# zhangrengang/SubPhaser

Measured on AMD Instinct MI355X. Metric: genome Gbases/s k-mer+enrichment, wheat k=15 1Mb windows, higher is better.
Workload: dtype u32

## Files before the change

include/subphaser_hip.h:

```cpp
#ifndef SUBPHASER_HIP_H
#define SUBPHASER_HIP_H
#include <stdint.h>
#ifdef __cplusplus
extern "C" {
#endif

#define SP_OK 0
#define SP_EINVAL (-1)
#define SP_EUNSUP (-2)
#define SP_ENOMEM (-3)
#define SP_EHIP (-4)
#define SP_ENODEV (-5)
#define SP_ESTATE (-6)
#define SP_EIO (-7)

typedef struct sp_ctx sp_ctx;

int sp_version(void);
const char *sp_last_error(const sp_ctx *ctx);

int sp_ctx_create(int device, void *stream, sp_ctx **out);
int sp_ctx_destroy(sp_ctx *ctx);
int sp_sync(sp_ctx *ctx);
void *sp_stream(sp_ctx *ctx);

int sp_genome_reset(sp_ctx *ctx, int n_chrom);
int sp_genome_add(sp_ctx *ctx, int chrom, const uint8_t *ascii, int64_t len);
int sp_genome_add_device(sp_ctx *ctx, int chrom, const uint8_t *d_ascii, int64_t len);
int sp_genome_len(sp_ctx *ctx, int chrom, int64_t *len);
int sp_genome_unpack(sp_ctx *ctx, int chrom, uint8_t *ascii_out, int64_t len);

int sp_count(sp_ctx *ctx, int k, int lower_count, int engine);
int sp_count_range(sp_ctx *ctx, int k, int lower_count, int engine, int first, int last);
int sp_count_recounts(sp_ctx *ctx, int64_t *recounts);
int sp_nslots(sp_ctx *ctx, int k, int64_t *nslots);
int sp_tables_bind(sp_ctx *ctx, int chrom, void *d_table);
int sp_table_overflow(sp_ctx *ctx, int chrom, void *d_pairs, int64_t cap, int64_t *n_pairs);
int sp_table_merge(sp_ctx *ctx, void *d_dst_u8, const void *d_dst_ovf, int64_t n_dst_ovf, const void *d_src_u8,
                   const void *d_src_ovf, int64_t n_src_ovf, int64_t slot_base, int64_t n, void *d_out_ovf, int64_t cap,
                   int64_t *n_out);
int sp_table_lengths(sp_ctx *ctx, const void *d_tab_u8, const void *d_ovf, int64_t n_ovf, int64_t slot_base, int64_t n,
                     int lower_count, int64_t *sum, int64_t *n_dump);
int sp_lengths(sp_ctx *ctx, int64_t *lengths );
int sp_dump_size(sp_ctx *ctx, int chrom, int64_t *n);
int sp_dump(sp_ctx *ctx, int chrom, uint64_t *keys, uint32_t *counts, int64_t cap, int64_t *n);

int sp_filter_view(sp_ctx *ctx, int C, const void *const *d_tabs, int64_t slot_base,
                   int64_t nslots_view, const int64_t *lengths, int k, int lower_count,
                   const void *const *d_ovf, const int64_t *n_ovf);
int sp_filter(sp_ctx *ctx, int n_sets, const int32_t *set_off, const int32_t *unit_off,
              const int32_t *unit_chrom, double min_fold, int baseline, double min_freq,
              double max_freq, double ratio, int64_t *n_union, int64_t *n_rows, int64_t *n_hist);
int sp_filter_fetch(sp_ctx *ctx, uint64_t *keys, uint32_t *counts, double *freqs, uint64_t *tot,
                    int64_t cap_rows);
int sp_filter_fetch_async(sp_ctx *ctx, uint64_t *keys, uint32_t *counts, uint64_t *tot, int64_t cap_rows);
int sp_filter_fetch_wait(sp_ctx *ctx);
int sp_filter_fetch_device(sp_ctx *ctx, void *d_keys, void *d_counts, void *d_tot, int64_t cap_rows);
int sp_filter_hist(sp_ctx *ctx, uint64_t *tot, int64_t cap);

int sp_labels_set(sp_ctx *ctx, const uint64_t *keys, const uint8_t *sg, int64_t n, int n_sg);
int sp_labels_set_device(sp_ctx *ctx, const uint64_t *d_keys, const uint8_t *d_sg, int64_t n, int n_sg);
int sp_map_nslots(sp_ctx *ctx, int chrom, int64_t bin_size, int64_t chunk_size, int64_t *nslots);
int sp_map_bins(sp_ctx *ctx, int chrom, int64_t bin_size, int64_t chunk_size, int32_t *slot_counts,
                int64_t nslots, int64_t *n_mapped);
int sp_map_bins_all(sp_ctx *ctx, int64_t bin_size, int64_t chunk_size, const int64_t *slot_off,
                    int32_t *slot_counts, int64_t *n_mapped);
int sp_stack_windows(sp_ctx *ctx, int64_t bin_size, int64_t chunk_size, int64_t window_size,
                     const int64_t *slot_off, const int64_t *win_off, int64_t *win_counts);
int sp_stack_windows_dev(sp_ctx *ctx, int64_t bin_size, int64_t chunk_size, int64_t window_size,
                         const int64_t *slot_off, const int64_t *win_off, const int64_t *seg_start, void *d_win);
int sp_map_features(sp_ctx *ctx, const uint8_t *ascii, const int64_t *off, int64_t n_feat,
                    int64_t *counts);
int sp_map_intervals(sp_ctx *ctx, const int32_t *chrom, const int64_t *start, const int64_t *end, int64_t n,
                     int64_t *counts);
int sp_labels_hit(sp_ctx *ctx, int64_t *n_hit);

int sp_enrich(sp_ctx *ctx, const int64_t *counts, int64_t W, int S, double max_pval,
              double min_ratio, double *pvals, int32_t *argmin, uint8_t *sig, double *ratios);
int sp_enrich_dev(sp_ctx *ctx, const void *d_counts, int64_t W, int S, double max_pval, double min_ratio,
                  double *pvals, int32_t *argmin, uint8_t *sig, double *ratios);
int sp_stack_enrich(sp_ctx *ctx, int64_t bin_size, int64_t chunk_size, int64_t window_size, const int64_t *slot_off,
                    const int64_t *win_off, double max_pval, double min_ratio, int64_t *win_counts, double *pvals,
                    int32_t *argmin, uint8_t *sig, double *ratios);

int sp_kmer_ttest(sp_ctx *ctx, const uint32_t *counts, int64_t M, int C, const int64_t *lengths, int n_groups,
                  const int32_t *group_off, const int32_t *group_chrom, int32_t *top, int32_t *second,
                  double *pvals, double *means);
int sp_kmer_ttest_wide(sp_ctx *ctx, const uint32_t *counts, int64_t M, int C, const int64_t *lengths, int n_groups,
                       const int32_t *group_off, const int32_t *group_chrom, int32_t *top, int32_t *second,
                       double *pvals, double *means);
int sp_kmer_ranktest(sp_ctx *ctx, const uint32_t *counts , int64_t M, int C, const int64_t *lengths,
                     int n_groups, const int32_t *group_off, const int32_t *group_chrom,
                     int method , int32_t *top, int32_t *second, double *pvals,
                     double *means , double *stat );
int sp_kmer_wilcoxon(sp_ctx *ctx, const uint32_t *counts , int64_t M, int C, const int64_t *lengths,
                     int n_groups, const int32_t *group_off, const int32_t *group_chrom, int32_t *top, int32_t *second,
                     double *pvals, double *means , double *stat );

int sp_kmeans_bootstrap(sp_ctx *ctx, const double *z , int C, int64_t M, const int64_t *cols , int R,
                        int n, int K, uint64_t seed, int32_t *labels , int32_t *iters ,
                        double *gram );

int sp_kmer_pca_gram(sp_ctx *ctx, const uint32_t *counts , int64_t M, int C,
                     const int64_t *lengths, double *gram , int64_t *n_bad, double *stats );
int sp_kmer_pca_signs(sp_ctx *ctx, const uint32_t *counts, int64_t M, int C, const int64_t *lengths,
                      const double *U , int n_comp, int64_t *rows , double *vals );

int sp_hclust_complete(sp_ctx *ctx, const double *pts , int P, int D, double *merges ,
                       double *dist );

int sp_sparse_sizes(sp_ctx *ctx, int64_t *n);
int sp_sparse_sample(sp_ctx *ctx, int chrom, int64_t n_samples, uint64_t *keys, int64_t *n_out);
int sp_sparse_split(sp_ctx *ctx, int chrom, const uint64_t *splitters, int n_split, int64_t *bounds);
int sp_sparse_export(sp_ctx *ctx, int chrom, int64_t first, int64_t count, void *d_keys, void *d_counts);
int sp_sparse_view(sp_ctx *ctx, int C, const void *const *d_keys, const void *const *d_counts, const int64_t *n,
                   const int64_t *lengths, int k, int lower_count);

int sp_prof_enable(sp_ctx *ctx, int on);
int sp_prof_reset(sp_ctx *ctx);
int sp_prof_report(sp_ctx *ctx, char *buf, int64_t cap);

int sp_synth_chrom(sp_ctx *ctx, uint8_t *d_out, int64_t len, uint64_t seed, int set_id,
                   int sg_id, int n_sg, int chrom_id, int exchange);
int sp_synth_chrom_range(sp_ctx *ctx, uint8_t *d_out, int64_t len, int64_t start, int64_t n, uint64_t seed, int set_id,
                         int sg_id, int n_sg, int chrom_id, int exchange);
int sp_host_alloc(sp_ctx *ctx, int64_t bytes, void **h_ptr);
int sp_host_free(sp_ctx *ctx, void *h_ptr);
int sp_host_register(sp_ctx *ctx, void *h_ptr, int64_t bytes);
int sp_host_unregister(sp_ctx *ctx, void *h_ptr);
int sp_dev_alloc(sp_ctx *ctx, int64_t bytes, void **d_ptr);
int sp_dev_free(sp_ctx *ctx, void *d_ptr);
int sp_dev_copy_to_host(sp_ctx *ctx, void *dst, const void *d_src, int64_t bytes);
int sp_dev_copy_from_host(sp_ctx *ctx, void *d_dst, const void *src, int64_t bytes);


typedef struct sp_fasta sp_fasta;
int sp_fasta_open(const void *data, int64_t n, int threads, sp_fasta **out);
int sp_fasta_counts(const sp_fasta *h, int64_t *n_records, int64_t *n_bases);
int sp_fasta_fetch(const sp_fasta *h, int64_t *hdr_start, int64_t *hdr_end, int64_t *seq_off, void *cat);
void sp_fasta_close(sp_fasta *h);

// ... 27 lines not shown
```

subphaser_amd/_native.py:

```python
import ctypes as C
import json
import os

import numpy as np

_HERE = os.path.dirname(os.path.abspath(__file__))
LIB_PATH = os.environ.get("SUBPHASER_HIP_LIB") or os.path.join(_HERE, "lib", "libsubphaser_hip.so")

SP_OK, SP_EINVAL, SP_EUNSUP, SP_ENOMEM, SP_EHIP, SP_ENODEV, SP_ESTATE, SP_EIO = 0, -1, -2, -3, -4, -5, -6, -7
KBOOT_MAX_POINTS, KBOOT_MAX_CLUSTERS = 128, 32
KPCA_MAX_CHROM, KPCA_MAX_COMP = 1024, 32
HCLUST_MAX_POINTS = 16384
RANKTEST_MAX_GROUP = 64
RANKTEST_METHODS = ("kruskal", "mannwhitneyu")
WILCOXON_MAX_GROUP = 64

SYMBOLS = [
    "sp_version", "sp_last_error", "sp_ctx_create", "sp_ctx_destroy", "sp_sync", "sp_stream",
    "sp_genome_reset", "sp_genome_add", "sp_genome_add_device", "sp_genome_len", "sp_genome_unpack",
    "sp_count", "sp_count_range", "sp_count_recounts", "sp_nslots", "sp_tables_bind", "sp_table_overflow", "sp_table_merge", "sp_table_lengths", "sp_lengths", "sp_dump_size", "sp_dump",
    "sp_filter_view", "sp_filter", "sp_filter_fetch", "sp_filter_fetch_async", "sp_filter_fetch_wait", "sp_filter_fetch_device", "sp_filter_hist",
    "sp_labels_set", "sp_labels_set_device", "sp_map_nslots", "sp_map_bins", "sp_map_bins_all", "sp_stack_windows", "sp_stack_windows_dev", "sp_stack_enrich", "sp_map_features", "sp_map_intervals", "sp_labels_hit",
    "sp_enrich", "sp_enrich_dev", "sp_kmer_ttest", "sp_kmer_ttest_wide", "sp_kmer_ranktest", "sp_kmer_wilcoxon", "sp_kmeans_bootstrap", "sp_kmer_pca_gram", "sp_kmer_pca_signs", "sp_hclust_complete",
    "sp_sparse_sizes", "sp_sparse_sample", "sp_sparse_split", "sp_sparse_export", "sp_sparse_view",
    "sp_prof_enable", "sp_prof_reset", "sp_prof_report",
    "sp_synth_chrom", "sp_synth_chrom_range", "sp_host_alloc", "sp_host_free", "sp_host_register", "sp_host_unregister", "sp_dev_alloc", "sp_dev_free", "sp_dev_copy_to_host", "sp_dev_copy_from_host",
    "sp_fasta_open", "sp_fasta_counts", "sp_fasta_fetch", "sp_fasta_close",
    "sp_text_kmer_matrix", "sp_text_sig_kmers", "sp_text_repr", "sp_text_table",
]


def csrc_fingerprint():
    import glob
    import hashlib
    h = hashlib.sha256()
    files = sorted(glob.glob(os.path.join(_HERE, "csrc", "*.hip")) + glob.glob(os.path.join(_HERE, "csrc", "*.h")))
    for f in files:
        h.update(os.path.basename(f).encode())
        h.update(open(f, "rb").read())
    return h.hexdigest()[:16]


class NativeError(RuntimeError):
    """HIP/runtime failure inside libsubphaser_hip.so."""


_lib = None


def load():
    global _lib
    if _lib is not None:
        return _lib
    if not os.path.exists(LIB_PATH):
        raise NativeError(
            "libsubphaser_hip.so is not built (%s). Run `python -c 'import __graft_entry__ as g; g.build()'` "
            "or `make -C subphaser_amd/csrc`. There is no CPU fallback." % LIB_PATH)
    L = C.CDLL(LIB_PATH)
    vp, i64, i32, dbl, ci = C.c_void_p, C.c_int64, C.c_int32, C.c_double, C.c_int
    P = C.POINTER
    L.sp_version.restype = ci
    L.sp_last_error.restype = C.c_char_p
    L.sp_last_error.argtypes = [vp]
    L.sp_ctx_create.argtypes = [ci, vp, P(vp)]
    L.sp_ctx_destroy.argtypes = [vp]
    L.sp_sync.argtypes = [vp]
    L.sp_stream.restype = vp
    L.sp_stream.argtypes = [vp]
    L.sp_genome_reset.argtypes = [vp, ci]
    L.sp_genome_add.argtypes = [vp, ci, vp, i64]
    L.sp_genome_add_device.argtypes = [vp, ci, vp, i64]
    L.sp_genome_len.argtypes = [vp, ci, P(i64)]
    L.sp_genome_unpack.argtypes = [vp, ci, vp, i64]
    L.sp_count.argtypes = [vp, ci, ci, ci]
    L.sp_count_range.argtypes = [vp, ci, ci, ci, ci, ci]
    L.sp_nslots.argtypes = [vp, ci, P(i64)]
    L.sp_count_recounts.argtypes = [vp, P(i64)]
    L.sp_tables_bind.argtypes = [vp, ci, vp]
    L.sp_table_overflow.argtypes = [vp, ci, vp, i64, P(i64)]
    L.sp_table_merge.argtypes = [vp, vp, vp, i64, vp, vp, i64, i64, i64, vp, i64, P(i64)]
    L.sp_table_lengths.argtypes = [vp, vp, vp, i64, i64, i64, ci, P(i64), P(i64)]
    L.sp_filter_view.argtypes = [vp, ci, vp, i64, i64, vp, ci, ci, vp, vp]
    L.sp_lengths.argtypes = [vp, vp]
    L.sp_dump_size.argtypes = [vp, ci, P(i64)]
    L.sp_dump.argtypes = [vp, ci, vp, vp, i64, P(i64)]
    L.sp_filter.argtypes = [vp, ci, vp, vp, vp, dbl, ci, dbl, dbl, dbl, P(i64), P(i64), P(i64)]
    L.sp_filter_fetch.argtypes = [vp, vp, vp, vp, vp, i64]
    L.sp_filter_fetch_device.argtypes = [vp, vp, vp, vp, i64]
    L.sp_filter_fetch_async.argtypes = [vp, vp, vp, vp, i64]
    L.sp_filter_fetch_wait.argtypes = [vp]
    L.sp_filter_hist.argtypes = [vp, vp, i64]
    L.sp_labels_set.argtypes = [vp, vp, vp, i64, ci]
    L.sp_labels_set_device.argtypes = [vp, vp, vp, i64, ci]
    L.sp_map_nslots.argtypes = [vp, ci, i64, i64, P(i64)]
    L.sp_map_bins.argtypes = [vp, ci, i64, i64, vp, i64, P(i64)]
    L.sp_map_bins_all.argtypes = [vp, i64, i64, vp, vp, vp]
    L.sp_stack_windows.argtypes = [vp, i64, i64, i64, vp, vp, vp]
    L.sp_stack_windows_dev.argtypes = [vp, i64, i64, i64, vp, vp, vp, vp]
    L.sp_stack_enrich.argtypes = [vp, i64, i64, i64, vp, vp, dbl, dbl, vp, vp, vp, vp, vp]
    L.sp_map_features.argtypes = [vp, vp, vp, i64, vp]
    L.sp_map_intervals.argtypes = [vp, vp, vp, vp, i64, vp]
    L.sp_host_alloc.argtypes = [vp, i64, P(vp)]
    L.sp_host_free.argtypes = [vp, vp]
    L.sp_labels_hit.argtypes = [vp, P(i64)]
    L.sp_enrich.argtypes = [vp, vp, i64, ci, dbl, dbl, vp, vp, vp, vp]
    L.sp_enrich_dev.argtypes = [vp, vp, i64, ci, dbl, dbl, vp, vp, vp, vp]
    L.sp_kmer_ttest.argtypes = [vp, vp, i64, ci, vp, ci, vp, vp, vp, vp, vp, vp]
    L.sp_kmer_ttest_wide.argtypes = [vp, vp, i64, ci, vp, ci, vp, vp, vp, vp, vp, vp]
    L.sp_kmer_ranktest.argtypes = [vp, vp, i64, ci, vp, ci, vp, vp, ci, vp, vp, vp, vp, vp]
    L.sp_kmer_wilcoxon.argtypes = [vp, vp, i64, ci, vp, ci, vp, vp, vp, vp, vp, vp, vp]
    L.sp_kmeans_bootstrap.argtypes = [vp, vp, ci, i64, vp, ci, ci, ci, C.c_uint64, vp, vp, vp]
    L.sp_kmer_pca_gram.argtypes = [vp, vp, i64, ci, vp, vp, P(i64), vp]
    L.sp_kmer_pca_signs.argtypes = [vp, vp, i64, ci, vp, vp, ci, vp, vp]
    L.sp_hclust_complete.argtypes = [vp, vp, ci, ci, vp, vp]
    L.sp_sparse_sizes.argtypes = [vp, vp]
    L.sp_sparse_sample.argtypes = [vp, ci, i64, vp, P(i64)]
    L.sp_sparse_split.argtypes = [vp, ci, vp, ci, vp]
    L.sp_sparse_export.argtypes = [vp, ci, i64, i64, vp, vp]
    L.sp_sparse_view.argtypes = [vp, ci, vp, vp, vp, vp, ci, ci]
    L.sp_prof_enable.argtypes = [vp, ci]
    L.sp_prof_reset.argtypes = [vp]
    L.sp_prof_report.argtypes = [vp, C.c_char_p, i64]
    L.sp_synth_chrom.argtypes = [vp, vp, i64, C.c_uint64, ci, ci, ci, ci, ci]
    L.sp_synth_chrom_range.argtypes = [vp, vp, i64, i64, i64, C.c_uint64, ci, ci, ci, ci, ci]
    L.sp_dev_alloc.argtypes = [vp, i64, P(vp)]
    L.sp_dev_free.argtypes = [vp, vp]
    L.sp_dev_copy_to_host.argtypes = [vp, vp, vp, i64]
    L.sp_host_register.argtypes = [vp, vp, i64]
    L.sp_host_unregister.argtypes = [vp, vp]
    L.sp_dev_copy_from_host.argtypes = [vp, vp, vp, i64]
    L.sp_fasta_open.argtypes = [vp, i64, ci, P(vp)]
    L.sp_fasta_counts.argtypes = [vp, P(i64), P(i64)]
    L.sp_fasta_fetch.argtypes = [vp, vp, vp, vp, vp]
    L.sp_fasta_close.argtypes = [vp]
    L.sp_fasta_close.restype = None
    L.sp_text_kmer_matrix.argtypes = [vp, ci, vp, i64, ci, ci, ci, P(i64)]
    L.sp_text_sig_kmers.argtypes = [vp, ci, vp, C.c_char_p, ci, vp, vp, ci, i64, ci, ci, P(i64)]
    L.sp_text_repr.argtypes = [vp, i64, vp, vp]
    L.sp_text_table.argtypes = [vp, ci, i64, ci, ci, P(i64)]
    for name in SYMBOLS:
        if name not in ("sp_last_error", "sp_stream", "sp_fasta_close"):
            getattr(L, name).restype = ci
    _lib = L
    return L


def _p(a):
    return a.ctypes.data_as(C.c_void_p) if a is not None else None


def fasta_scan(data, threads=None, out=None):
    L = load()
    data = np.frombuffer(data, np.uint8) if isinstance(data, (bytes, bytearray, memoryview)) else data
    if data.dtype != np.uint8 or not data.flags.c_contiguous:
        data = np.ascontiguousarray(data, np.uint8)
    n = int(data.size)
    if threads is None:
        threads = min(32, len(os.sched_getaffinity(0)))
    h = C.c_void_p()
    rc = L.sp_fasta_open(C.c_void_p(data.ctypes.data) if n else None, n, int(threads), C.byref(h))
    if rc == SP_ENOMEM:
        raise MemoryError("sp_fasta_open")
    if rc:
        raise ValueError("sp_fasta_open: bad arguments")
    try:
        nr, nb = C.c_int64(), C.c_int64()
        L.sp_fasta_counts(h, C.byref(nr), C.byref(nb))
        nr, nb = nr.value, nb.value
        hs, he, off = np.empty(nr, np.int64), np.empty(nr, np.int64), np.empty(nr + 1, np.int64)
        cat = out(nb) if out is not None else np.empty(nb, np.uint8)
        if L.sp_fasta_fetch(h, _p(hs), _p(he), _p(off), _p(cat) if nb else None):
            raise ValueError("sp_fasta_fetch: bad arguments")
    finally:
        L.sp_fasta_close(h)
    ids = []
    for a, b in zip(hs.tolist(), he.tolist()):
        t = bytes(data[a:b]).split()
        ids.append(t[0].decode() if t else "")
    return ids, cat, off


def _fd_of(fout):
    try:
        fd = fout.fileno()
        fout.flush()
        return fd
    except Exception:
        return None


def _text_threads():
    return min(64, len(os.sched_getaffinity(0)))


def _text_fail(name, rc):
    msg = load().sp_last_error(None).decode(errors="replace")
    if rc == SP_ENOMEM:
        raise MemoryError("%s: %s" % (name, msg or "out of memory"))
    raise OSError("%s failed (%d): %s" % (name, rc, msg))


def text_kmer_matrix(fout, keys, k, freqs):
    fd = _fd_of(fout)
    if fd is None:
        return False
    keys = np.ascontiguousarray(keys, np.uint64)
    freqs = np.ascontiguousarray(freqs, np.float64)
    M, Cn = freqs.shape
    rc = load().sp_text_kmer_matrix(_p(keys), int(k), _p(freqs), M, Cn, _text_threads(), fd, None)
    if rc:
        _text_fail("sp_text_kmer_matrix", rc)
    return True


def text_sig_kmers(fout, keys, k, top, names, pvals, means):
    fd = _fd_of(fout)
    if fd is None:
        return False
    keys = np.ascontiguousarray(keys, np.uint64)
    top = np.ascontiguousarray(top, np.int32)
    pvals = np.ascontiguousarray(pvals, np.float64)
    means = np.ascontiguousarray(means, np.float64)
    blob = b"".join(n.encode() + b"\0" for n in names)
# ... 248 lines not shown
    def sparse_view(self, d_keys, d_counts, n, lengths, k, lower_count):
        if d_keys is None:
            self._ck(self.L.sp_sparse_view(self.h, 0, None, None, None, None, 0, 0))
            self._view_C = None
            return
        ka = (C.c_void_p * len(d_keys))(*[int(p) for p in d_keys])
        ca = (C.c_void_p * len(d_counts))(*[int(p) for p in d_counts])
        n = np.ascontiguousarray(n, np.int64)
        lengths = np.ascontiguousarray(lengths, np.int64)
        self._ck(self.L.sp_sparse_view(self.h, len(d_keys), ka, ca, _p(n), _p(lengths), int(k), int(lower_count)))
        self._view_C = len(d_keys)
        self.k = int(k)

    def lengths(self):
        out = np.zeros(self.n_chrom, np.int64)
        self._ck(self.L.sp_lengths(self.h, _p(out)))
        return out

    def dump_size(self, chrom):
        n = C.c_int64()
        self._ck(self.L.sp_dump_size(self.h, int(chrom), C.byref(n)))
        return n.value

    def dump(self, chrom, sort=True):
        n = C.c_int64()
        self._ck(self.L.sp_dump_size(self.h, int(chrom), C.byref(n)))
        keys = np.empty(n.value, np.uint64)
        cnts = np.empty(n.value, np.uint32)
        self._ck(self.L.sp_dump(self.h, int(chrom), _p(keys), _p(cnts), n.value, C.byref(n)))
        if sort and keys.size:
            o = np.argsort(keys, kind="stable")
            keys, cnts = keys[o], cnts[o]
        return keys, cnts

    def filter(self, set_off, unit_off, unit_chrom, min_fold, baseline, min_freq, max_freq, ratio):
        set_off = np.ascontiguousarray(set_off, np.int32)
        unit_off = np.ascontiguousarray(unit_off, np.int32)
        unit_chrom = np.ascontiguousarray(unit_chrom, np.int32)
        nu, nr, nh = C.c_int64(), C.c_int64(), C.c_int64()
        self._ck(self.L.sp_filter(self.h, len(set_off) - 1, _p(set_off), _p(unit_off), _p(unit_chrom),
                                  float(min_fold), int(baseline), float(min_freq), float(max_freq),
                                  float(ratio), C.byref(nu), C.byref(nr), C.byref(nh)))
        return nu.value, nr.value, nh.value

    def filter_fetch(self, n_rows, want_freqs=True, sort=True, pinned=False):
        Cn = getattr(self, "_view_C", None) or self.n_chrom
        if pinned and not sort:
            keys = self.pinned_empty("ff_keys", (n_rows,), np.uint64)
            counts = self.pinned_empty("ff_counts", (n_rows, Cn), np.uint32)
            tot = self.pinned_empty("ff_tot", (n_rows,), np.uint64)
            freqs = self.pinned_empty("ff_freqs", (n_rows, Cn), np.float64) if want_freqs else None
        else:
            keys = np.empty(n_rows, np.uint64)
            counts = np.empty((n_rows, Cn), np.uint32)
            tot = np.empty(n_rows, np.uint64)
            freqs = np.empty((n_rows, Cn), np.float64) if want_freqs else None
        self._ck(self.L.sp_filter_fetch(self.h, _p(keys), _p(counts), _p(freqs), _p(tot), n_rows))
        if sort and n_rows:
            o = np.argsort(keys, kind="stable")
            keys, counts, tot = keys[o], counts[o], tot[o]
            if freqs is not None:
                freqs = freqs[o]
        return keys, counts, freqs, tot

    def filter_fetch_async(self, n_rows):
        Cn = getattr(self, "_view_C", None) or self.n_chrom
        keys = self.pinned_empty("ff_keys", (n_rows,), np.uint64)
        counts = self.pinned_empty("ff_counts", (n_rows, Cn), np.uint32)
        tot = self.pinned_empty("ff_tot", (n_rows,), np.uint64)
        self._ck(self.L.sp_filter_fetch_async(self.h, _p(keys), _p(counts), _p(tot), n_rows))
        return keys, counts, tot

    def filter_fetch_async_ptr(self, h_keys, h_counts, n_rows):
        tot = self.pinned_empty("ff_tot", (max(int(n_rows), 1),), np.uint64)
        self._ck(self.L.sp_filter_fetch_async(self.h, C.c_void_p(int(h_keys)), C.c_void_p(int(h_counts)), _p(tot), int(n_rows)))

    def filter_fetch_wait(self):
        self._ck(self.L.sp_filter_fetch_wait(self.h))

    def filter_fetch_device(self, d_keys, d_counts, d_tot, n_rows):
        v = lambda p: C.c_void_p(int(p)) if p else None
        self._ck(self.L.sp_filter_fetch_device(self.h, v(d_keys), v(d_counts), v(d_tot), int(n_rows)))

    def filter_hist(self, n_hist):
        tot = np.empty(n_hist, np.uint64)
        self._ck(self.L.sp_filter_hist(self.h, _p(tot), n_hist))
        return tot

    def labels_set(self, keys, sg, n_sg):
        keys = np.ascontiguousarray(keys, np.uint64)
        sg = np.ascontiguousarray(sg, np.uint8)
        assert keys.size == sg.size
        self._ck(self.L.sp_labels_set(self.h, _p(keys), _p(sg), keys.size, int(n_sg)))
        self.n_sg = int(n_sg)

    def labels_set_device(self, d_keys, d_sg, n, n_sg):
        self._ck(self.L.sp_labels_set_device(self.h, C.c_void_p(int(d_keys)), C.c_void_p(int(d_sg)), int(n), int(n_sg)))
        self.n_sg = int(n_sg)

    def labels_set_from(self, labels, n_sg):
        if hasattr(labels, "on_device"):
            d_keys, d_sg = labels.on_device(self)
            self.labels_set_device(d_keys, d_sg, len(labels.keys), n_sg)
        else:
            self.labels_set(labels.keys, labels.sg_idx, n_sg)

    def map_nslots(self, chrom, bin_size, chunk_size):
        n = C.c_int64()
        self._ck(self.L.sp_map_nslots(self.h, int(chrom), int(bin_size), int(chunk_size), C.byref(n)))
        return n.value

    def map_bins(self, chrom, bin_size=10000, chunk_size=10_000_000):
        ns = self.map_nslots(chrom, bin_size, chunk_size)
        out = np.empty((ns, self.n_sg), np.int32)
        n = C.c_int64()
        self._ck(self.L.sp_map_bins(self.h, int(chrom), int(bin_size), int(chunk_size), _p(out), ns,
                                    C.byref(n)))
        return out, n.value

    def map_bins_all(self, bin_size=10000, chunk_size=10_000_000):
        off = np.zeros(self.n_chrom + 1, np.int64)
        for i in range(self.n_chrom):
            off[i + 1] = off[i] + self.map_nslots(i, bin_size, chunk_size)
        out = self.pinned_empty("map_all", (int(off[-1]), self.n_sg), np.int32)
        nm = np.zeros(self.n_chrom, np.int64)
        self._ck(self.L.sp_map_bins_all(self.h, int(bin_size), int(chunk_size), _p(off), _p(out), _p(nm)))
        self.last_map = (out, off)
        return [out[off[i]:off[i + 1]] for i in range(self.n_chrom)], nm

    def stack_windows(self, bin_size, chunk_size, window_size, lengths):
        out, off = self.last_map
        woff = np.zeros(self.n_chrom + 1, np.int64)
        for i, n in enumerate(lengths):
            woff[i + 1] = woff[i] + (int(n) + int(window_size) - 1) // int(window_size) + 1
        win = self.pinned_empty("win_all", (int(woff[-1]), self.n_sg), np.int64)
        self._ck(self.L.sp_stack_windows(self.h, int(bin_size), int(chunk_size), int(window_size), _p(off),
                                         _p(woff), _p(win)))
        return win, woff

    def stack_windows_dev(self, bin_size, chunk_size, window_size, win_off, seg_start, d_win):
        out, off = self.last_map
        win_off = np.ascontiguousarray(win_off, np.int64)
        seg = np.ascontiguousarray(seg_start, np.int64) if seg_start is not None else None
        self._ck(self.L.sp_stack_windows_dev(self.h, int(bin_size), int(chunk_size), int(window_size), _p(off),
                                             _p(win_off), _p(seg) if seg is not None else None, C.c_void_p(int(d_win))))

    def stack_enrich(self, bin_size, chunk_size, window_size, lengths, max_pval=0.05, min_ratio=0.5):
        out, off = self.last_map
        woff = np.zeros(self.n_chrom + 1, np.int64)
        for i, n in enumerate(lengths):
            woff[i + 1] = woff[i] + (int(n) + int(window_size) - 1) // int(window_size) + 1
        W, S = int(woff[-1]), self.n_sg
        win = self.pinned_empty("win_all", (W, S), np.int64)
        pvals = self.pinned_empty("enr_p", (W, S), np.float64)
        ratios = self.pinned_empty("enr_q", (W, S), np.float64)
        argmin = self.pinned_empty("enr_a", (W,), np.int32)
        sig = self.pinned_empty("enr_s", (W,), np.uint8)
        self._ck(self.L.sp_stack_enrich(self.h, int(bin_size), int(chunk_size), int(window_size), _p(off), _p(woff),
                                        float(max_pval), float(min_ratio), _p(win), _p(pvals), _p(argmin), _p(sig),
                                        _p(ratios)))
        return win, woff, pvals, argmin, sig, ratios

    def enrich_dev(self, d_counts, W, S, max_pval=0.05, min_ratio=0.5):
        pvals = np.empty((W, S), np.float64)
        ratios = np.empty((W, S), np.float64)
        argmin = np.empty(W, np.int32)
# ... 211 lines not shown
```

subphaser_amd/csrc/sp_common.h:

```cpp
#pragma once
#include <hip/hip_runtime.h>
#include <stdint.h>
#include <stdio.h>
#include <string.h>

#include <map>
#include <string>
#include <vector>

#include "../../include/subphaser_hip.h"
#include "sp_carve.h"

#define SP_WAVE 64

struct sp_chrom {
    bool tab_external = false;
    int64_t len = 0;
    int64_t nw = 0;
    int64_t cap_mw = 0;
    uint32_t *d_pk = nullptr;
    uint32_t *d_pm = nullptr;
    uint32_t *d_nm = nullptr;
    uint8_t *d_tab = nullptr;
    uint2 *d_ovf = nullptr;
    int64_t n_ovf = 0, cap_ovf = 0;
    uint32_t *d_ovf_idx = nullptr;
    int64_t ovf_idx_n = 0, ovf_idx_cap = 0;
    int64_t length_sum = 0;
    int64_t n_dump = 0;
    hipEvent_t ev_packed = nullptr;
};
#define SP_PAD_WORDS 8
#define SP_LIST_MAXC 1024
#define SP_TABLE_LDS (140 * 1024)
#define SP_TABLE_MIN_TILE 256
#define SP_TABLE_MAXC (SP_TABLE_LDS / SP_TABLE_MIN_TILE)
#ifndef SP_DERIVE_PM
#define SP_DERIVE_PM 1
#endif

struct sp_buf {
    void *p = nullptr;
    int64_t cap = 0;
};

template <typename T>
struct sp_tmp {
    T *p = nullptr;
    sp_tmp() = default;
    sp_tmp(const sp_tmp &) = delete;
    sp_tmp &operator=(const sp_tmp &) = delete;
    ~sp_tmp() {
        if (p) hipFree(p);
    }
    hipError_t alloc(size_t n_elems) { return hipMalloc((void **)&p, (n_elems ? n_elems : 1) * sizeof(T)); }
    operator T *() const { return p; }
};

struct sp_sparse_chrom {
    uint64_t *d_keys = nullptr;
    uint32_t *d_cnts = nullptr;
    int64_t n = 0, cap = 0, length_sum = 0;
};

struct sp_tabref {
    const uint8_t *tab;
    const uint2 *ovf;
    int64_t n_ovf;
    const uint32_t *ovf_idx = nullptr;
};

struct sp_prof_entry {
    std::string name;
    hipEvent_t e0, e1;
};

struct sp_ctx {
    int device = 0;
    hipStream_t stream = nullptr;
    hipStream_t copy_stream = nullptr;
    hipEvent_t copy_event = nullptr;
    bool own_stream = false;
    int n_cu = 256;
    std::string err;
    std::vector<sp_chrom> chroms;
    int k = 0;
    int lower = 0;
    int64_t nslots = 0;
    bool counted = false;
    int64_t c2_recounts = 0;
    bool fv_on = false;
    std::vector<sp_tabref> fv_tabs;
    std::vector<int64_t> fv_lengths;
    int64_t fv_slot_base = 0, fv_nslots = 0;
    bool sv_on = false;
    std::vector<const uint64_t *> sv_keys;
    std::vector<const uint32_t *> sv_cnts;
    std::vector<int64_t> sv_n;
    bool filtered = false;
    int64_t n_union = 0, n_rows = 0, n_hist = 0;
    uint32_t *d_flag_row = nullptr;
    uint32_t *d_flag_hist = nullptr;
    uint64_t *d_blk_row = nullptr;
    uint64_t *d_blk_hist = nullptr;
    int64_t n_fblocks = 0;
    uint8_t *d_label = nullptr;
    sp_buf b_ptab, b_labkeys;
    int ptab_k = 0;
    int64_t ptab_n = 0;
    unsigned long long *h_lflags = nullptr;
    sp_buf b_lflags;
    int64_t bloom_last_n = -1;
    int bloom_last_bits = 0, bloom_last_k = 0;
    sp_buf b_ctab, b_covf;
    int ct_bb = 0;
    uint32_t ct_ovf_mask = 0;
    int sq_bb = 0;
    uint64_t sq_ovf_mask = 0;
    int map_engine = 0;
    bool labels_ready = false;
    uint32_t *d_bloom = nullptr;
    int bloom_bits = 0;
    int n_sg = 0;
    int64_t n_labels = 0;
    void *d_scratch = nullptr;
    int64_t scratch_bytes = 0;
    void *d_ws2 = nullptr;
    int64_t ws2_bytes = 0;
    sp_buf b_cntlen;
    sp_buf b_tab32, b_ovfw;
    struct lane_t {
        hipStream_t stream = nullptr;
        hipEvent_t done = nullptr;
        void *d_ws2 = nullptr;
        int64_t ws2_bytes = 0;
        sp_buf b_ovfw;
        void *h_desc = nullptr;
        int64_t h_desc_cap = 0;
        sp_buf b_sp_a, b_sp_b, b_sp_c, b_sp_tmp, b_s3_small;
        hipEvent_t ev_a = nullptr, ev_b = nullptr;
    };
#define SP_MAX_LANES 7
    lane_t lanes[SP_MAX_LANES];
    lane_t *lane = nullptr;
    void *h_desc = nullptr;
    int64_t h_desc_cap = 0;
    hipEvent_t lane_go = nullptr;
    struct lane_scope {
        sp_ctx *ctx;
        hipStream_t saved;
        lane_scope(sp_ctx *c, lane_t *ln) : ctx(c), saved(c->stream) {
            if (ln) {
                ctx->lane = ln;
                ctx->stream = ln->stream;
            }
        }
        lane_scope(const lane_scope &) = delete;
        lane_scope &operator=(const lane_scope &) = delete;
        ~lane_scope() {
            ctx->lane = nullptr;
            ctx->stream = saved;
        }
    };
    bool sparse_mode = false;
    bool list_mode = false;
    std::vector<sp_sparse_chrom> sparse;
    sp_buf b_sp_a, b_sp_b, b_sp_c, b_sp_tmp, b_sf_keys, b_sf_counts, b_sf_tot, b_sf_hist, b_s3_small, b_slots;
    unsigned long long *h_s3 = nullptr;
    hipEvent_t s3_ev[2] = {nullptr, nullptr};
    int64_t sf_n = 0;
    uint64_t *d_hkeys = nullptr;
    int64_t hcap = 0;
    sp_buf b_tt;
    sp_buf b_kb;
    sp_buf b_kp;
    sp_buf b_hc;
    sp_buf b_wtab, b_enr;
    sp_buf b_fq;
    sp_buf b_fflat;
    sp_buf b_map, b_mapdesc, b_ival, b_emit, b_fpar, b_win;
    bool map_all_valid = false;
    bool prof = false;
    std::vector<sp_prof_entry> prof_pending;
    std::map<std::string, std::pair<int64_t, double>> prof_acc;
};

extern thread_local std::string g_sp_err;

int sp_fail(sp_ctx *ctx, int code, const char *fmt, ...);
int sp_scratch(sp_ctx *ctx, int64_t bytes, void **out);
struct sp_ctx;
int sp_buf_ensure(sp_ctx *ctx, sp_buf &b, int64_t bytes);
void sp_buf_free(sp_buf &b);
bool sp_on_device(sp_ctx *ctx, const void *p);
void sp_prof_begin(sp_ctx *ctx, const char *name);
void sp_prof_end(sp_ctx *ctx);
void sp_prof_flush(sp_ctx *ctx);

#define SP_HIP(ctx, call)                                                                  \
    do {                                                                                   \
        hipError_t e__ = (call);                                                           \
        if (e__ != hipSuccess)                                                             \
            return sp_fail(ctx, e__ == hipErrorOutOfMemory ? SP_ENOMEM : SP_EHIP,          \
                           "%s failed: %s (%s:%d)", #call, hipGetErrorString(e__), __FILE__, \
                           __LINE__);                                                      \
    } while (0)

#define SP_LAUNCH(ctx, name, kernel, grid, block, shmem, ...)                       \
    do {                                                                            \
        sp_prof_begin(ctx, name);                                                   \
        hipLaunchKernelGGL(kernel, grid, block, shmem, (ctx)->stream, __VA_ARGS__); \
        sp_prof_end(ctx);                                                           \
        SP_HIP(ctx, hipGetLastError());                                             \
    } while (0)

struct sp_kparams {
    int k;
    int odd;
    uint64_t kmask;
    int rcshift;
};

__host__ __device__ inline sp_kparams sp_make_kparams(int k) {
    sp_kparams p;
    p.k = k;
    p.odd = k & 1;
    p.kmask = (k == 32) ? ~0ULL : ((1ULL << (2 * k)) - 1ULL);
    p.rcshift = 2 * (k - 1);
    return p;
}

__host__ __device__ inline int64_t sp_dense_slots(int k) {
    return (k & 1) ? (1LL << (2 * k - 1)) : (1LL << (2 * k));
}

__host__ __device__ inline uint64_t sp_slot_of(uint64_t fwd, uint64_t rc, const sp_kparams &p) {
    if (p.odd) {
        uint64_t rep = ((fwd >> p.k) & 1ULL) ? rc : fwd;
        uint64_t lowmask = (1ULL << p.k) - 1ULL;
        return (rep & lowmask) | ((rep >> (p.k + 1)) << p.k);
    }
    return fwd < rc ? fwd : rc;
}

__host__ __device__ inline uint64_t sp_revcomp(uint64_t x, int k) {
    x = ~x;
    x = ((x >> 2) & 0x3333333333333333ULL) | ((x & 0x3333333333333333ULL) << 2);
    x = ((x >> 4) & 0x0F0F0F0F0F0F0F0FULL) | ((x & 0x0F0F0F0F0F0F0F0FULL) << 4);
    x = ((x >> 8) & 0x00FF00FF00FF00FFULL) | ((x & 0x00FF00FF00FF00FFULL) << 8);
    x = ((x >> 16) & 0x0000FFFF0000FFFFULL) | ((x & 0x0000FFFF0000FFFFULL) << 16);
    x = (x >> 32) | (x << 32);
    return x >> (64 - 2 * k);
}

__host__ __device__ inline uint64_t sp_key_of_slot(uint64_t slot, const sp_kparams &p) {
    if (p.odd) {
        uint64_t lowmask = (1ULL << p.k) - 1ULL;
        uint64_t rep = (slot & lowmask) | ((slot >> p.k) << (p.k + 1));
        uint64_t r = sp_revcomp(rep, p.k);
        return rep < r ? rep : r;
    }
    return slot;
}

__host__ __device__ inline uint64_t sp_slot_of_key(uint64_t key, const sp_kparams &p) {
    return sp_slot_of(key, sp_revcomp(key, p.k), p);
}
```

subphaser_amd/csrc/sp_count.hip:

```cpp
#include "sp_device.h"
#include "sp_c2batch.h"
#include "sp_c2plan.h"
#include "sp_internal.h"

__global__ void __launch_bounds__(256)
k1_count_atomic(const uint32_t *__restrict__ pk, const uint32_t *__restrict__ nm, int64_t n_units,
                sp_kparams32 kp, uint32_t *__restrict__ tab) {
    int64_t u = (int64_t)blockIdx.x * blockDim.x + threadIdx.x;
    const int64_t stride = (int64_t)gridDim.x * blockDim.x;
    for (; u < n_units; u += stride) {
        uint32_t last = 0xFFFFFFFFu;
        uint32_t acc = 0;
        sp_scan_unit32<SP_UNIT>(pk, nm, u * SP_UNIT, kp, [&](int64_t, uint32_t fwd, uint32_t rc) {
            const uint32_t slot = sp_slot_of32(fwd, rc, kp);
            if (slot == last) {
                acc++;
            } else {
                if (acc) atomicAdd(&tab[last], acc);
                last = slot;
                acc = 1;
            }
        });
        if (acc) atomicAdd(&tab[last], acc);
    }
// ... 377 lines not shown
    if (hipMemGetInfo(&free_b, &total_b) == hipSuccess) {
        int64_t need[SP_MAX_LANES];
        for (int l = 0; l < n_lanes; l++) need[l] = ctx->lanes[l].ws2_bytes >= per_lane ? 0 : per_lane;
        const int fit = sp_lanes_fit(need, n_lanes, (int64_t)free_b, (int64_t)total_b);
        if (fit < n_lanes) {
            if (getenv("SP_DEBUG_COUNT")) fprintf(stderr, "[sp] count: %d of %d lanes fit the free device memory\n", fit, n_lanes);
            n_lanes = (dense_lanes && fit == 1) ? 0 : fit;
        }
    }
    const int rc = sp_lanes_open(ctx, n_lanes);
    if (rc) return rc;
    if (n_lanes && J.list_mode) {
        SP_HIP(ctx, hipEventRecord(ctx->lane_go, ctx->stream));
        for (int l = 0; l < n_lanes; l++) SP_HIP(ctx, hipStreamWaitEvent(ctx->lanes[l].stream, ctx->lane_go, 0));
    }
    J.n_lanes = n_lanes;
    return SP_OK;
}

static int list_reserve(sp_ctx *ctx, sp_sparse_chrom &o, int64_t need) {
    if (need <= o.cap) return SP_OK;
    SP_HIP(ctx, hipStreamSynchronize(ctx->stream));
    if (o.d_keys) hipFree(o.d_keys);
    if (o.d_cnts) hipFree(o.d_cnts);
    o = sp_sparse_chrom();
    SP_HIP(ctx, hipMalloc(&o.d_keys, (size_t)(need + 1) * 8));
    SP_HIP(ctx, hipMalloc(&o.d_cnts, (size_t)(need + 1) * 4));
    o.cap = need;
    return SP_OK;
}
static int list_begin(sp_ctx *ctx, const count_job &J, size_t ci) {
    sp_sparse_chrom &o = ctx->sparse[ci];
    o.n = 0;
    o.length_sum = 0;
    int64_t need = ctx->chroms[ci].len / J.lower + 16;
    if (need > J.nslots) need = J.nslots;
    return list_reserve(ctx, o, need);
}

static int count_batch(sp_ctx *ctx, count_job &J) {
    for (size_t ci = (size_t)J.first; ci < (size_t)J.last; ci++) {
        if (!ctx->chroms[ci].d_pk && ctx->chroms[ci].len > 0) return sp_fail(ctx, SP_EINVAL, "chromosome %zu not loaded", ci);
        const int rc = list_begin(ctx, J, ci);
        if (rc) return rc;
        J.by_engine2[ci] = 1;
    }
    SP_HIP(ctx, hipMemsetAsync(J.d_len + 4 * (size_t)J.first, 0, 4 * (size_t)(J.last - J.first) * sizeof(unsigned long long), ctx->stream));
    const int G = J.n_lanes + 1;
    if (J.n_lanes) {
        SP_HIP(ctx, hipEventRecord(ctx->lane_go, ctx->stream));
        for (int l = 0; l < J.n_lanes; l++) SP_HIP(ctx, hipStreamWaitEvent(ctx->lanes[l].stream, ctx->lane_go, 0));
    }
    for (int g = 0; g < G; g++) {
        std::vector<int> idx;
        for (int ci = J.first + g; ci < J.last; ci += G) idx.push_back(ci);
        if (idx.empty()) continue;
        sp_ctx::lane_scope on(ctx, g ? &ctx->lanes[g - 1] : nullptr);
        const int rc = sp_count_engine3_batch(ctx, idx.data(), (int)idx.size(), J.kp, J.lower, J.d_len);
        if (rc) return rc;
    }
    return SP_OK;
}

static int count_chrom_chain(sp_ctx *ctx, count_job &J, size_t ci, sp_ctx::lane_t *ln) {
    SP_HIP(ctx, hipMemsetAsync(J.d_len + 4 * ci, 0, 4 * sizeof(unsigned long long), ln ? ln->stream : ctx->stream));
    sp_ctx::lane_scope on(ctx, ln);
    const int rc = sp_count_engine2(ctx, ctx->chroms[ci], J.kp, J.lower, J.d_len + 4 * ci, !J.sized_by_sample,
                                    J.list_mode ? &ctx->sparse[ci] : nullptr);
    if (!rc) J.by_engine2[ci] = 1;
    return rc;
}

static int count_chrom_list(sp_ctx *ctx, count_job &J, size_t ci) {
    const int rc = list_begin(ctx, J, ci);
    if (rc) return rc;
    const size_t G = (size_t)(J.n_lanes + 1);
    return count_chrom_chain(ctx, J, ci, (J.n_lanes > 0 && ci % G) ? &ctx->lanes[ci % G - 1] : nullptr);
}

static int count_chrom_table(sp_ctx *ctx, count_job &J, size_t ci) {
    sp_chrom &c = ctx->chroms[ci];
    sp_ctx::lane_t *ln = J.n_lanes > 0 ? &ctx->lanes[ci % (size_t)J.n_lanes] : nullptr;
    if (ln && c.ev_packed) SP_HIP(ctx, hipStreamWaitEvent(ln->stream, c.ev_packed, 0));
    if (ln && ctx->copy_event) SP_HIP(ctx, hipStreamWaitEvent(ln->stream, ctx->copy_event, 0));
    return count_chrom_chain(ctx, J, ci, ln);
}

static int count_chrom_atomic(sp_ctx *ctx, const count_job &J, size_t ci, int64_t need_ovf) {
    sp_chrom &c = ctx->chroms[ci];
    const int64_t nslots = J.nslots;
    SP_HIP(ctx, hipMemsetAsync(J.d_len + 4 * ci, 0, 4 * sizeof(unsigned long long), ctx->stream));
    const int64_t n_buckets = (nslots + (1LL << SP_OVF_SHIFT) - 1) >> SP_OVF_SHIFT;
    int rc = sp_buf_ensure(ctx, ctx->b_tab32, nslots * 4);
    if (rc) return rc;
    rc = sp_buf_ensure(ctx, ctx->b_ovfw, need_ovf * 8 + (3 * n_buckets + 1) * 4 + 256);
    if (rc) return rc;
    uint32_t *tab32 = (uint32_t *)ctx->b_tab32.p;
    uint2 *ovf_tmp = (uint2 *)ctx->b_ovfw.p;
    uint32_t *seg_base = (uint32_t *)(ovf_tmp + need_ovf), *seg_cnt = seg_base + n_buckets, *seg_off = seg_cnt + n_buckets;
    SP_HIP(ctx, hipMemsetAsync(tab32, 0, (size_t)nslots * sizeof(uint32_t), ctx->stream));
    int64_t n_units = (c.len + SP_UNIT - 1) / SP_UNIT;
    if (n_units > 0) {
        int grid = grid_for(ctx, n_units, 256, 16);
        SP_LAUNCH(ctx, "k1_count_atomic", k1_count_atomic, dim3(grid), dim3(256), 0, c.d_pk, c.d_nm,
                  n_units, sp_make_kparams32(J.kp.k), tab32);
    }
    int grid2 = (int)(n_buckets < (int64_t)ctx->n_cu * 8 ? n_buckets : (int64_t)ctx->n_cu * 8);
    SP_LAUNCH(ctx, "k1_narrow", k1_narrow, dim3(grid2), dim3(256), 0, (const uint32_t *)tab32, nslots,
              (uint32_t)J.lower, c.d_tab, J.d_len + 4 * ci, ovf_tmp, (unsigned long long)need_ovf, seg_base, seg_cnt,
              n_buckets);
    return sp_ovf_finalize(ctx, c, ovf_tmp, seg_base, seg_cnt, seg_off, n_buckets, nullptr);
}

static int count_all(sp_ctx *ctx, count_job &J) {
    if (J.batch) return count_batch(ctx, J);
    for (size_t ci = (size_t)J.first; ci < (size_t)J.last; ci++) {
        sp_chrom &c = ctx->chroms[ci];
        if (!c.d_pk && c.len > 0) return sp_fail(ctx, SP_EINVAL, "chromosome %zu not loaded", ci);
        int rc;
        if (J.list_mode) {
            rc = count_chrom_list(ctx, J, ci);
        } else {
            if (!c.d_tab) SP_HIP(ctx, hipMalloc(&c.d_tab, (size_t)J.nslots));
            const int64_t need_ovf = c.len / 255 + 16;
            if (need_ovf > c.cap_ovf) {
                if (c.d_ovf) {
                    SP_HIP(ctx, hipStreamSynchronize(ctx->stream));
                    hipFree(c.d_ovf);
                    c.d_ovf = nullptr;
                }
                SP_HIP(ctx, hipMalloc(&c.d_ovf, (size_t)need_ovf * sizeof(uint2)));
                c.cap_ovf = need_ovf;
            }
            int eng = J.engine;
            if (eng == 0) eng = (sp_engine2_supported(J.nslots) && c.len >= (1 << 22)) ? 2 : 1;
            rc = eng == 2 ? count_chrom_table(ctx, J, ci) : count_chrom_atomic(ctx, J, ci, need_ovf);
        }
        if (rc) return rc;
    }
    return SP_OK;
}

extern "C" {

static int count_impl(sp_ctx *ctx, int k, int lower_count, int engine, int first, int last) {
    if (!ctx) return SP_EINVAL;
    if (k < 1 || k > 32) return sp_fail(ctx, SP_EUNSUP, "k=%d unsupported (1..32)", k);
    if (lower_count < 1) lower_count = 1;
    if (ctx->chroms.empty()) return sp_fail(ctx, SP_EINVAL, "sp_count: no chromosomes loaded");
    SP_HIP(ctx, hipSetDevice(ctx->device));
    if (first < 0 || last > (int)ctx->chroms.size() || first > last)
        return sp_fail(ctx, SP_EINVAL, "sp_count_range: bad chromosome range [%d, %d)", first, last);
    if (k > 15) {
        if (first != 0 || last != (int)ctx->chroms.size())
            return sp_fail(ctx, SP_EUNSUP, "sp_count_range: k > 15 counts all chromosomes at once");
        for (auto &c : ctx->chroms)
            if (!c.d_pk && c.len > 0) return sp_fail(ctx, SP_EINVAL, "a chromosome is not loaded");
        ctx->counted = false;
        ctx->filtered = false;
        if (ctx->d_label && ctx->k != k) {
            hipFree(ctx->d_label);
            ctx->d_label = nullptr;
        }
        if (ctx->k != k) ctx->labels_ready = false;
        ctx->k = k;
        ctx->lower = lower_count;
        ctx->nslots = 0;
        ctx->sparse_mode = true;
        ctx->list_mode = false;
        int rcs = (engine == 1) ? sp_sparse_count(ctx, k, lower_count) : sp_sparse_count3(ctx, k, lower_count);
        if (rcs) return rcs;
        ctx->counted = true;
        return SP_OK;
    }
    ctx->sparse_mode = false;
    const size_t C = ctx->chroms.size();
    const bool whole = first == 0 && last == (int)C;
    count_job J{sp_make_kparams(k), sp_dense_slots(k), lower_count, engine, first, last};
    for (size_t ci = (size_t)first; ci < (size_t)last; ci++) {
        J.longest = ctx->chroms[ci].len > J.longest ? ctx->chroms[ci].len : J.longest;
        J.total_len += ctx->chroms[ci].len;
    }
    const int64_t nslots = J.nslots;
    int rc = count_list_mode(ctx, J, whole);
    if (rc) return rc;
    const bool list_mode = J.list_mode;
    if (ctx->k != k || ctx->nslots != nslots) {
        SP_HIP(ctx, hipStreamSynchronize(ctx->stream));
        for (auto &c : ctx->chroms)
            if (c.d_tab && !c.tab_external) {
                hipFree(c.d_tab);
                c.d_tab = nullptr;
            }
        if (ctx->d_label) {
            hipFree(ctx->d_label);
            ctx->d_label = nullptr;
        }
        ctx->labels_ready = false;
    }
    ctx->k = k;
    ctx->lower = lower_count;
    ctx->nslots = nslots;
    ctx->counted = false;
    ctx->filtered = false;
    ctx->list_mode = list_mode;
    if (list_mode && ctx->sparse.size() != C) {
        sp_sparse_release(ctx);
        ctx->sparse.assign(C, sp_sparse_chrom());
    }
    rc = sp_buf_ensure(ctx, ctx->b_cntlen, (int64_t)(4 * C * sizeof(unsigned long long)));
    if (rc) return rc;
    unsigned long long *d_len = J.d_len = (unsigned long long *)ctx->b_cntlen.p;
    const char *env_exact = getenv("SP_C2_EXACT");
    const bool sized_by_sample = J.sized_by_sample = !(env_exact && env_exact[0] == '1');
    J.by_engine2.assign(C, 0);
    const char *env_batch = getenv("SP_C2_BATCH");
    J.batch = list_mode && last - first > 1 && sized_by_sample && !(env_batch && env_batch[0] == '0') &&
              (J.longest < (1LL << 26) || (env_batch && env_batch[0] == '1'));
    const bool dense_lanes = !list_mode && C > 1 && whole && engine != 1;
    if ((list_mode && C > 1) || dense_lanes) {
        rc = count_open_lanes(ctx, J, dense_lanes);
        if (rc) return rc;
    }
    rc = count_all(ctx, J);
    if (rc) {
        sp_lanes_drain(ctx, J.n_lanes);
        return rc;
    }
    rc = sp_lanes_join(ctx, J.n_lanes);
    if (rc) return rc;
    std::vector<unsigned long long> h(4 * C);
    SP_HIP(ctx, hipMemcpyAsync(h.data(), d_len, 4 * C * sizeof(unsigned long long), hipMemcpyDeviceToHost,
                              ctx->stream));
    SP_HIP(ctx, hipStreamSynchronize(ctx->stream));
    int redone = 0;
    for (size_t ci = (size_t)first; ci < (size_t)last; ci++) {
        if (!J.by_engine2[ci] || !sized_by_sample || h[4 * ci + 3] == 0) continue;
        SP_HIP(ctx, hipMemsetAsync(d_len + 4 * ci, 0, 4 * sizeof(unsigned long long), ctx->stream));
        rc = sp_count_engine2(ctx, ctx->chroms[ci], J.kp, lower_count, d_len + 4 * ci, true,
                              list_mode ? &ctx->sparse[ci] : nullptr);
        if (rc) return rc;
        redone++;
    }
    if (redone) {
        if (getenv("SP_DEBUG_COUNT")) fprintf(stderr, "[sp] engine 2: %d chromosome(s) recounted with exact bucket sizes\n", redone);
        SP_HIP(ctx, hipMemcpyAsync(h.data(), d_len, 4 * C * sizeof(unsigned long long), hipMemcpyDeviceToHost, ctx->stream));
        SP_HIP(ctx, hipStreamSynchronize(ctx->stream));
    }
    ctx->c2_recounts += redone;
    for (size_t ci = (size_t)first; ci < (size_t)last; ci++) {
        if (J.by_engine2[ci] && h[4 * ci + 3] != 0)
            return sp_fail(ctx, SP_ESTATE, "count engine 2: chromosome %zu overran its bucket regions with exact sizes", ci);
        ctx->chroms[ci].length_sum = (int64_t)h[4 * ci];
        ctx->chroms[ci].n_dump = (int64_t)h[4 * ci + 1];
        ctx->chroms[ci].n_ovf = (int64_t)h[4 * ci + 2];
        if (list_mode) {
            sp_sparse_chrom &o = ctx->sparse[ci];
            if (ctx->chroms[ci].n_ovf > o.cap || ctx->chroms[ci].n_dump > o.cap)
                return sp_fail(ctx, SP_ESTATE, "count engine 3: chromosome %zu reserved %lld pairs for %lld dump k-mers (capacity %lld)",
                               ci, (long long)ctx->chroms[ci].n_ovf, (long long)ctx->chroms[ci].n_dump, (long long)o.cap);
            o.n = ctx->chroms[ci].n_dump;
            o.length_sum = ctx->chroms[ci].length_sum;
            ctx->chroms[ci].n_ovf = 0;
            continue;
        }
        if (ctx->chroms[ci].n_ovf > ctx->chroms[ci].cap_ovf)
            return sp_fail(ctx, SP_ESTATE, "overflow list of chromosome %zu: %lld pairs exceed the capacity %lld", ci,
                           (long long)ctx->chroms[ci].n_ovf, (long long)ctx->chroms[ci].cap_ovf);
    }
    ctx->counted = true;
    return SP_OK;
}

int sp_count(sp_ctx *ctx, int k, int lower_count, int engine) {
    return count_impl(ctx, k, lower_count, engine, 0, ctx ? (int)ctx->chroms.size() : 0);
}

int sp_count_range(sp_ctx *ctx, int k, int lower_count, int engine, int first, int last) {
    return count_impl(ctx, k, lower_count, engine, first, last);
}

int sp_count_recounts(sp_ctx *ctx, int64_t *recounts) {
    if (!ctx || !recounts) return sp_fail(ctx, SP_EINVAL, "sp_count_recounts: bad arguments");
    *recounts = ctx->c2_recounts;
    return SP_OK;
}

int sp_nslots(sp_ctx *ctx, int k, int64_t *nslots) {
    (void)ctx;
    if (!nslots || k < 1 || k > 15) return sp_fail(ctx, SP_EUNSUP, "sp_nslots: dense tables exist for k = 1..15");
    *nslots = sp_dense_slots(k);
    return SP_OK;
}

int sp_tables_bind(sp_ctx *ctx, int chrom, void *d_table) {
    if (!ctx || chrom < 0 || chrom >= (int)ctx->chroms.size())
        return sp_fail(ctx, SP_EINVAL, "sp_tables_bind: bad arguments");
    SP_HIP(ctx, hipSetDevice(ctx->device));
    sp_chrom &c = ctx->chroms[(size_t)chrom];
    if (c.d_tab && !c.tab_external) {
        SP_HIP(ctx, hipStreamSynchronize(ctx->stream));
        hipFree(c.d_tab);
    }
    c.d_tab = (uint8_t *)d_table;
    c.tab_external = d_table != nullptr;
    ctx->counted = false;
    return SP_OK;
}

int sp_table_overflow(sp_ctx *ctx, int chrom, void *d_pairs, int64_t cap, int64_t *n_pairs) {
    if (!ctx || !n_pairs || cap < 0 || chrom < 0 || chrom >= (int)ctx->chroms.size())
        return sp_fail(ctx, SP_EINVAL, "sp_table_overflow: bad arguments");
    if (ctx->sparse_mode || ctx->list_mode || !ctx->counted)
        return sp_fail(ctx, SP_EINVAL, "sp_table_overflow: call sp_count (k <= 15, byte-table engines 1 / 2) first");
    sp_chrom &c = ctx->chroms[(size_t)chrom];
    *n_pairs = c.n_ovf;
    if (!d_pairs) return SP_OK;
    if (cap < c.n_ovf) return sp_fail(ctx, SP_EINVAL, "sp_table_overflow: capacity %lld < %lld", (long long)cap, (long long)c.n_ovf);
    SP_HIP(ctx, hipSetDevice(ctx->device));
    if (c.n_ovf)
        SP_HIP(ctx, hipMemcpyAsync(d_pairs, c.d_ovf, (size_t)c.n_ovf * sizeof(uint2), hipMemcpyDeviceToDevice, ctx->stream));
    return SP_OK;
}

int sp_table_merge(sp_ctx *ctx, void *d_dst_u8, const void *d_dst_ovf, int64_t n_dst_ovf, const void *d_src_u8,
                   const void *d_src_ovf, int64_t n_src_ovf, int64_t slot_base, int64_t n, void *d_out_ovf, int64_t cap,
                   int64_t *n_out) {
    if (!ctx || !d_dst_u8 || !d_src_u8 || !n_out || n < 0 || slot_base < 0 || cap < 0 || n_dst_ovf < 0 || n_src_ovf < 0 ||
        (n_dst_ovf > 0 && !d_dst_ovf) || (n_src_ovf > 0 && !d_src_ovf) || (cap > 0 && !d_out_ovf) ||
        (d_out_ovf && (d_out_ovf == d_dst_ovf || d_out_ovf == d_src_ovf)))
        return sp_fail(ctx, SP_EINVAL, "sp_table_merge: bad arguments");
    *n_out = 0;
    if (n == 0) return SP_OK;
    SP_HIP(ctx, hipSetDevice(ctx->device));
    const int64_t n_buckets = (n + (1LL << SP_OVF_SHIFT) - 1) >> SP_OVF_SHIFT;
    int rc = sp_buf_ensure(ctx, ctx->b_ovfw, (cap + 1) * 8 + (3 * n_buckets + 1) * 4 + 256);
    if (rc) return rc;
    unsigned long long *d_cur = (unsigned long long *)ctx->b_ovfw.p;
    uint2 *tmp = (uint2 *)(d_cur + 1);
    uint32_t *seg_base = (uint32_t *)(tmp + cap), *seg_cnt = seg_base + n_buckets, *seg_off = seg_cnt + n_buckets;
    SP_HIP(ctx, hipMemsetAsync(d_cur, 0, 8, ctx->stream));
    sp_tabref A, B;
    A.tab = (const uint8_t *)d_dst_u8; A.ovf = (const uint2 *)d_dst_ovf; A.n_ovf = n_dst_ovf;
    B.tab = (const uint8_t *)d_src_u8; B.ovf = (const uint2 *)d_src_ovf; B.n_ovf = n_src_ovf;
    int grid = (int)(n_buckets < (int64_t)ctx->n_cu * 8 ? n_buckets : (int64_t)ctx->n_cu * 8);
    SP_LAUNCH(ctx, "kx_merge", kx_merge, dim3(grid), dim3(256), 0, (uint8_t *)d_dst_u8, A, B, slot_base, n, d_cur, tmp,
              (unsigned long long)cap, seg_base, seg_cnt, n_buckets);
    unsigned long long h = 0;
    SP_HIP(ctx, hipMemcpyAsync(&h, d_cur, 8, hipMemcpyDeviceToHost, ctx->stream));
    SP_HIP(ctx, hipStreamSynchronize(ctx->stream));
    *n_out = (int64_t)h;
    if ((int64_t)h > cap)
        return sp_fail(ctx, SP_ENOMEM, "sp_table_merge: %lld overflow pairs exceed the capacity %lld (the tables are now "
                       "inconsistent: merge again from fresh inputs)", (long long)h, (long long)cap);
    if (h) return ovf_finalize_to(ctx, (uint2 *)d_out_ovf, tmp, seg_base, seg_cnt, seg_off, n_buckets, nullptr, slot_base);
    return SP_OK;
}

int sp_table_lengths(sp_ctx *ctx, const void *d_tab_u8, const void *d_ovf, int64_t n_ovf, int64_t slot_base, int64_t n,
                     int lower_count, int64_t *sum, int64_t *n_dump) {
    if (!ctx || !d_tab_u8 || !sum || !n_dump || n < 0 || n_ovf < 0 || (n_ovf > 0 && !d_ovf))
        return sp_fail(ctx, SP_EINVAL, "sp_table_lengths: bad arguments");
    *sum = *n_dump = 0;
    if (n == 0) return SP_OK;
    SP_HIP(ctx, hipSetDevice(ctx->device));
    void *scr = nullptr;
    int rc = sp_scratch(ctx, 256, &scr);
    if (rc) return rc;
    unsigned long long *d2 = (unsigned long long *)scr, h[2] = {0, 0};
    SP_HIP(ctx, hipMemsetAsync(d2, 0, 16, ctx->stream));
    sp_tabref T;
    T.tab = (const uint8_t *)d_tab_u8; T.ovf = (const uint2 *)d_ovf; T.n_ovf = n_ovf;
    SP_LAUNCH(ctx, "kx_lengths", kx_lengths, dim3((unsigned)(ctx->n_cu * 4)), dim3(256), 0, T, slot_base, n,
              (uint32_t)(lower_count < 1 ? 1 : lower_count), d2);
    SP_HIP(ctx, hipMemcpyAsync(h, d2, 16, hipMemcpyDeviceToHost, ctx->stream));
    SP_HIP(ctx, hipStreamSynchronize(ctx->stream));
    *sum = (int64_t)h[0];
    *n_dump = (int64_t)h[1];
    return SP_OK;
}

int sp_lengths(sp_ctx *ctx, int64_t *lengths) {
    if (!ctx || !lengths) return sp_fail(ctx, SP_EINVAL, "sp_lengths: bad arguments");
    if (!ctx->counted) return sp_fail(ctx, SP_EINVAL, "sp_lengths: call sp_count first");
    for (size_t i = 0; i < ctx->chroms.size(); i++) lengths[i] = ctx->chroms[i].length_sum;
    return SP_OK;
}

int sp_dump_size(sp_ctx *ctx, int chrom, int64_t *n) {
    if (!ctx || !n || chrom < 0 || chrom >= (int)ctx->chroms.size())
        return sp_fail(ctx, SP_EINVAL, "sp_dump_size: bad arguments");
    if (!ctx->counted) return sp_fail(ctx, SP_EINVAL, "sp_dump_size: call sp_count first");
    *n = ctx->chroms[(size_t)chrom].n_dump;
    return SP_OK;
}

int sp_dump(sp_ctx *ctx, int chrom, uint64_t *keys, uint32_t *counts, int64_t cap, int64_t *n) {
    if (!ctx || !n || chrom < 0 || chrom >= (int)ctx->chroms.size())
        return sp_fail(ctx, SP_EINVAL, "sp_dump: bad arguments");
    if (!ctx->counted) return sp_fail(ctx, SP_EINVAL, "sp_dump: call sp_count first");
    SP_HIP(ctx, hipSetDevice(ctx->device));
    sp_chrom &c = ctx->chroms[(size_t)chrom];
    *n = c.n_dump;
    if (cap < c.n_dump) return sp_fail(ctx, SP_EINVAL, "sp_dump: capacity %lld < %lld", (long long)cap,
                                       (long long)c.n_dump);
    if (c.n_dump == 0) return SP_OK;
    if (ctx->sparse_mode || ctx->list_mode) return sp_sparse_dump(ctx, chrom, keys, counts);
    const sp_kparams kp = sp_make_kparams(ctx->k);
    int64_t nblk = (ctx->nslots + DUMP_SLOTS - 1) / DUMP_SLOTS;
    sp_tmp<unsigned long long> d_blk, d_keys;
    sp_tmp<uint32_t> d_cnt;
    SP_HIP(ctx, d_blk.alloc((size_t)nblk));
    SP_HIP(ctx, d_keys.alloc((size_t)c.n_dump));
    SP_HIP(ctx, d_cnt.alloc((size_t)c.n_dump));
    sp_tabref T;
    T.tab = c.d_tab;
    T.ovf = c.d_ovf;
    T.n_ovf = c.n_ovf;
    SP_LAUNCH(ctx, "dump_count", dump_count, dim3((unsigned)nblk), dim3(DUMP_BLOCK), 0, T,
              ctx->nslots, (uint32_t)ctx->lower, d_blk.p);
    SP_LAUNCH(ctx, "scan_excl_u64", scan_excl_u64, dim3(1), dim3(1024), 0, d_blk.p, nblk,
              (unsigned long long *)nullptr);
    SP_LAUNCH(ctx, "dump_write", dump_write, dim3((unsigned)nblk), dim3(DUMP_BLOCK), 0, T,
              ctx->nslots, (uint32_t)ctx->lower, d_blk.p, kp, d_keys.p, d_cnt.p);
    SP_HIP(ctx, hipMemcpyAsync(keys, d_keys, (size_t)c.n_dump * sizeof(uint64_t), hipMemcpyDeviceToHost,
                              ctx->stream));
    SP_HIP(ctx, hipMemcpyAsync(counts, d_cnt, (size_t)c.n_dump * sizeof(uint32_t), hipMemcpyDeviceToHost,
                              ctx->stream));
    SP_HIP(ctx, hipStreamSynchronize(ctx->stream));
    return SP_OK;
}
}
```

subphaser_amd/csrc/sp_ctx.hip:

```cpp
#include <stdarg.h>

#include "sp_common.h"
#include "sp_internal.h"

thread_local std::string g_sp_err;

int sp_fail(sp_ctx *ctx, int code, const char *fmt, ...) {
    char buf[1024];
    va_list ap;
    va_start(ap, fmt);
    vsnprintf(buf, sizeof buf, fmt, ap);
    va_end(ap);
    if (ctx) ctx->err = buf;
    g_sp_err = buf;
    return code;
}

int sp_scratch(sp_ctx *ctx, int64_t bytes, void **out) {
    if (bytes > ctx->scratch_bytes) {
        if (ctx->d_scratch) {
            SP_HIP(ctx, hipStreamSynchronize(ctx->stream));
            SP_HIP(ctx, hipFree(ctx->d_scratch));
            ctx->d_scratch = nullptr;
            ctx->scratch_bytes = 0;
        }
        SP_HIP(ctx, hipMalloc(&ctx->d_scratch, (size_t)bytes));
        ctx->scratch_bytes = bytes;
    }
    *out = ctx->d_scratch;
    return SP_OK;
}

bool sp_on_device(sp_ctx *ctx, const void *p) {
    hipPointerAttribute_t at;
    if (hipPointerGetAttributes(&at, p) == hipSuccess) return at.type == hipMemoryTypeDevice && at.device == ctx->device;
    (void)hipGetLastError();
    return false;
}

int sp_buf_ensure(sp_ctx *ctx, sp_buf &b, int64_t bytes) {
    if (bytes <= b.cap) return SP_OK;
    if (b.p) {
        SP_HIP(ctx, hipStreamSynchronize(ctx->stream));
        SP_HIP(ctx, hipFree(b.p));
        b.p = nullptr;
        b.cap = 0;
    }
    int64_t want = bytes + bytes / 8 + 4096;
    SP_HIP(ctx, hipMalloc(&b.p, (size_t)want));
    b.cap = want;
    return SP_OK;
}
void sp_buf_free(sp_buf &b) {
    if (b.p) hipFree(b.p);
    b.p = nullptr;
    b.cap = 0;
}

void sp_prof_begin(sp_ctx *ctx, const char *name) {
    if (!ctx->prof) return;
    sp_prof_entry e;
    e.name = name;
    hipEventCreate(&e.e0);
    hipEventCreate(&e.e1);
    hipEventRecord(e.e0, ctx->stream);
    ctx->prof_pending.push_back(e);
}
void sp_prof_end(sp_ctx *ctx) {
    if (!ctx->prof) return;
    hipEventRecord(ctx->prof_pending.back().e1, ctx->stream);
}
void sp_prof_flush(sp_ctx *ctx) {
    if (ctx->prof_pending.empty()) return;
    hipStreamSynchronize(ctx->stream);
    for (auto &e : ctx->prof_pending) {
        float ms = 0.f;
        hipEventElapsedTime(&ms, e.e0, e.e1);
        auto &acc = ctx->prof_acc[e.name];
        acc.first += 1;
        acc.second += ms;
        hipEventDestroy(e.e0);
        hipEventDestroy(e.e1);
    }
    ctx->prof_pending.clear();
}


extern "C" {

int sp_version(void) { return 100; }

const char *sp_last_error(const sp_ctx *ctx) { return ctx ? ctx->err.c_str() : g_sp_err.c_str(); }

int sp_ctx_create(int device, void *stream, sp_ctx **out) {
    if (!out) return sp_fail(nullptr, SP_EINVAL, "sp_ctx_create: out is NULL");
    int n = 0;
    if (hipGetDeviceCount(&n) != hipSuccess || n <= 0)
        return sp_fail(nullptr, SP_ENODEV, "no HIP device visible (libsubphaser_hip needs an MI355X)");
    if (device < 0 || device >= n)
        return sp_fail(nullptr, SP_EINVAL, "device %d out of range (0..%d)", device, n - 1);
    sp_ctx *ctx = new sp_ctx();
    ctx->device = device;
    SP_HIP(ctx, hipSetDevice(device));
    hipDeviceProp_t prop;
    SP_HIP(ctx, hipGetDeviceProperties(&prop, device));
    ctx->n_cu = prop.multiProcessorCount;
    if (stream) {
        ctx->stream = (hipStream_t)stream;
    } else {
        SP_HIP(ctx, hipStreamCreateWithFlags(&ctx->stream, hipStreamNonBlocking));
        ctx->own_stream = true;
    }
    *out = ctx;
    return SP_OK;
}

static void free_chrom(sp_chrom &c) {
    if (c.d_pk) hipFree(c.d_pk);
    if (c.d_nm) hipFree(c.d_nm);
    if (c.d_tab && !c.tab_external) hipFree(c.d_tab);
    if (c.d_ovf) hipFree(c.d_ovf);
    if (c.d_ovf_idx) hipFree(c.d_ovf_idx);
    c.d_ovf_idx = nullptr;
    c.ovf_idx_n = c.ovf_idx_cap = 0;
    if (c.ev_packed) hipEventDestroy(c.ev_packed);
    c = sp_chrom();
}

static void free_filter(sp_ctx *ctx) {
    if (ctx->d_flag_row) hipFree(ctx->d_flag_row);
    if (ctx->d_flag_hist) hipFree(ctx->d_flag_hist);
    if (ctx->d_blk_row) hipFree(ctx->d_blk_row);
    if (ctx->d_blk_hist) hipFree(ctx->d_blk_hist);
    ctx->d_flag_row = ctx->d_flag_hist = nullptr;
    ctx->d_blk_row = ctx->d_blk_hist = nullptr;
    ctx->filtered = false;
}

int sp_ctx_destroy(sp_ctx *ctx) {
    if (!ctx) return SP_OK;
    hipSetDevice(ctx->device);
    hipStreamSynchronize(ctx->stream);
    sp_prof_flush(ctx);
    for (auto &c : ctx->chroms) free_chrom(c);
    free_filter(ctx);
    sp_sparse_release(ctx);
    if (ctx->d_label) hipFree(ctx->d_label);
    if (ctx->d_bloom) hipFree(ctx->d_bloom);
    if (ctx->d_scratch) hipFree(ctx->d_scratch);
    if (ctx->d_ws2) hipFree(ctx->d_ws2);
    for (auto &ln : ctx->lanes) {
        if (ln.d_ws2) hipFree(ln.d_ws2);
        sp_buf_free(ln.b_ovfw);
        if (ln.h_desc) hipHostFree(ln.h_desc);
        sp_buf_free(ln.b_sp_a);
        sp_buf_free(ln.b_sp_b);
        sp_buf_free(ln.b_sp_c);
        sp_buf_free(ln.b_sp_tmp);
        sp_buf_free(ln.b_s3_small);
        if (ln.ev_a) hipEventDestroy(ln.ev_a);
        if (ln.ev_b) hipEventDestroy(ln.ev_b);
        if (ln.done) hipEventDestroy(ln.done);
        if (ln.stream) hipStreamDestroy(ln.stream);
    }
    if (ctx->lane_go) hipEventDestroy(ctx->lane_go);
    if (ctx->h_s3) hipHostFree(ctx->h_s3);
    if (ctx->h_desc) hipHostFree(ctx->h_desc);
    for (auto &e : ctx->s3_ev)
        if (e) hipEventDestroy(e);
    sp_buf_free(ctx->b_map);
    sp_buf_free(ctx->b_mapdesc);
    sp_buf_free(ctx->b_ival);
    sp_buf_free(ctx->b_ptab);
    sp_buf_free(ctx->b_lflags);
    if (ctx->h_lflags) hipHostFree(ctx->h_lflags);
    sp_buf_free(ctx->b_cntlen);
    sp_buf_free(ctx->b_ctab);
    sp_buf_free(ctx->b_covf);
    sp_buf_free(ctx->b_tab32);
    sp_buf_free(ctx->b_ovfw);
    sp_buf_free(ctx->b_labkeys);
    sp_buf_free(ctx->b_emit);
    sp_buf_free(ctx->b_slots);
    sp_buf_free(ctx->b_fpar);
    sp_buf_free(ctx->b_fflat);
    sp_buf_free(ctx->b_fq);
    sp_buf_free(ctx->b_wtab);
    sp_buf_free(ctx->b_enr);
    sp_buf_free(ctx->b_tt);
    sp_buf_free(ctx->b_kb);
    sp_buf_free(ctx->b_kp);
    sp_buf_free(ctx->b_hc);
    sp_buf_free(ctx->b_win);
    if (ctx->copy_stream) {
        hipStreamSynchronize(ctx->copy_stream);
        hipStreamDestroy(ctx->copy_stream);
        hipEventDestroy(ctx->copy_event);
    }
    if (ctx->own_stream) hipStreamDestroy(ctx->stream);
    delete ctx;
    return SP_OK;
}

int sp_sync(sp_ctx *ctx) {
    SP_HIP(ctx, hipStreamSynchronize(ctx->stream));
    return SP_OK;
}

void *sp_stream(sp_ctx *ctx) { return (void *)ctx->stream; }

int sp_genome_reset(sp_ctx *ctx, int n_chrom) {
    if (!ctx || n_chrom < 0) return sp_fail(ctx, SP_EINVAL, "sp_genome_reset: bad arguments");
    SP_HIP(ctx, hipSetDevice(ctx->device));
    SP_HIP(ctx, hipStreamSynchronize(ctx->stream));
    if ((size_t)n_chrom == ctx->chroms.size()) {
        for (auto &c : ctx->chroms) {
            c.len = 0;
            c.nw = 0;
            c.length_sum = 0;
            c.n_dump = 0;
            c.n_ovf = 0;
            c.ovf_idx_n = 0;
        }
    } else {
        for (auto &c : ctx->chroms) free_chrom(c);
        ctx->chroms.assign((size_t)n_chrom, sp_chrom());
    }
    ctx->counted = false;
    ctx->filtered = false;
    return SP_OK;
}
}

__device__ __forceinline__ void pack_byte(uint32_t b, uint32_t &code, uint32_t &inv) {
    uint32_t u = b & 0xDFu;
    code = ((b >> 1) ^ (b >> 2)) & 3u;
    inv = !(u == 'A' || u == 'C' || u == 'G' || u == 'T');
}

__device__ __forceinline__ void pack_word4(uint32_t w, uint32_t &c8, uint32_t &inv4) {
    uint32_t t = ((w >> 1) ^ (w >> 2)) & 0x03030303u;
    const uint32_t letters = __builtin_amdgcn_perm(0u, 0x54474341u, t);
    const uint32_t x = letters ^ (w & 0xDFDFDFDFu);
    const uint32_t f = ((((x & 0x7F7F7F7Fu) + 0x7F7F7F7Fu) | x) & 0x80808080u) >> 7;
    t &= ~(f * 3u);
    t |= t >> 6;
    t |= t >> 12;
    c8 = t & 0xFFu;
    inv4 = ((f * 0x00204081u) >> 21) & 0xFu;
}
__device__ __forceinline__ uint32_t pack_msb_first(uint32_t w) {
    const uint32_t r = __brev(w);
    return ((r & 0x55555555u) << 1) | ((r >> 1) & 0x55555555u);
}

__global__ void __launch_bounds__(256)
k0_pack(const uint8_t *__restrict__ ascii, int64_t len, uint32_t *__restrict__ pk, uint32_t *__restrict__ pm,
        uint32_t *__restrict__ nm, int64_t n_mask_words) {
    int64_t t = (int64_t)blockIdx.x * blockDim.x + threadIdx.x;
    int64_t stride = (int64_t)gridDim.x * blockDim.x;
    const bool aligned = (((uintptr_t)ascii) & 15) == 0;
    for (; t < n_mask_words; t += stride) {
        int64_t base = t * 32;
        uint32_t w0 = 0, w1 = 0, m = 0, r0 = 0, r1 = 0;
        if (base + 32 <= len && aligned) {
            const uint4 *p = reinterpret_cast<const uint4 *>(ascii + base);
            uint4 a = p[0], b = p[1];
            uint32_t v[8] = {a.x, a.y, a.z, a.w, b.x, b.y, b.z, b.w};
#pragma unroll
            for (int q = 0; q < 8; q++) {
                uint32_t c8, inv4;
                pack_word4(v[q], c8, inv4);
                if (q < 4) w0 |= c8 << (8 * q);
                else w1 |= c8 << (8 * (q - 4));
                m |= inv4 << (4 * q);
            }
            r0 = pack_msb_first(w0);
            r1 = pack_msb_first(w1);
        } else {
            for (int i = 0; i < 32; i++) {
                uint32_t c = 0, iv = 1;
                if (base + i < len) pack_byte(ascii[base + i], c, iv);
                if (iv) c = 0;
                if (i < 16) { w0 |= c << (2 * i); r0 |= c << (30 - 2 * i); }
                else { w1 |= c << (2 * (i - 16)); r1 |= c << (30 - 2 * (i - 16)); }
                m |= iv << i;
            }
        }
        *reinterpret_cast<uint2 *>(pk + 2 * t) = make_uint2(w0, w1);
#if !SP_DERIVE_PM
        *reinterpret_cast<uint2 *>(pm + 2 * t) = make_uint2(r0, r1);
#else
        (void)r0; (void)r1; (void)pm;
#endif
        nm[t] = m;
    }
}

__global__ void __launch_bounds__(256)
k0_unpack(const uint32_t *__restrict__ pk, const uint32_t *__restrict__ nm, int64_t len,
          uint8_t *__restrict__ out) {
    int64_t i = (int64_t)blockIdx.x * blockDim.x + threadIdx.x;
    int64_t stride = (int64_t)gridDim.x * blockDim.x;
    for (; i < len; i += stride) {
        uint32_t c = (pk[i >> 4] >> (2 * (i & 15))) & 3u;
        uint32_t iv = (nm[i >> 5] >> (i & 31)) & 1u;
        out[i] = iv ? 'N' : "ACGT"[c];
    }
}

static int genome_add_impl(sp_ctx *ctx, int chrom, const uint8_t *d_ascii, int64_t len) {
    sp_chrom &c = ctx->chroms[(size_t)chrom];
    c.len = len;
    c.length_sum = 0;
    c.n_dump = 0;
    int64_t nmw = (len + 31) / 32 + SP_PAD_WORDS;
    c.nw = (len + 15) / 16;
    if (nmw > c.cap_mw) {
        if (c.d_pk) hipFree(c.d_pk);
        if (c.d_nm) hipFree(c.d_nm);
        c.d_pk = c.d_pm = c.d_nm = nullptr;
        c.cap_mw = 0;
#if SP_DERIVE_PM
        SP_HIP(ctx, hipMalloc(&c.d_pk, (size_t)(2 * nmw) * sizeof(uint32_t)));
        c.d_pm = c.d_pk;
#else
        SP_HIP(ctx, hipMalloc(&c.d_pk, (size_t)(4 * nmw) * sizeof(uint32_t)));
        c.d_pm = c.d_pk + 2 * nmw;
#endif
        SP_HIP(ctx, hipMalloc(&c.d_nm, (size_t)nmw * sizeof(uint32_t)));
        c.cap_mw = nmw;
    }
    int64_t blocks = (nmw + 255) / 256;
    if (blocks > 8LL * ctx->n_cu * 8) blocks = 8LL * ctx->n_cu * 8;
    if (blocks < 1) blocks = 1;
    SP_LAUNCH(ctx, "k0_pack", k0_pack, dim3((unsigned)blocks), dim3(256), 0, d_ascii, len, c.d_pk,
              c.d_pm, c.d_nm, nmw);
    if (!c.ev_packed) SP_HIP(ctx, hipEventCreateWithFlags(&c.ev_packed, hipEventDisableTiming));
    SP_HIP(ctx, hipEventRecord(c.ev_packed, ctx->stream));
    ctx->counted = false;
    return SP_OK;
}

extern "C" {

int sp_genome_add_device(sp_ctx *ctx, int chrom, const uint8_t *d_ascii, int64_t len) {
    if (!ctx || chrom < 0 || chrom >= (int)ctx->chroms.size() || len < 0 || (!d_ascii && len > 0))
        return sp_fail(ctx, SP_EINVAL, "sp_genome_add_device: bad arguments (chrom=%d len=%lld)", chrom,
                       (long long)len);
    SP_HIP(ctx, hipSetDevice(ctx->device));
    return genome_add_impl(ctx, chrom, d_ascii, len);
}

int sp_genome_add(sp_ctx *ctx, int chrom, const uint8_t *ascii, int64_t len) {
    if (!ctx || chrom < 0 || chrom >= (int)ctx->chroms.size() || len < 0 || (!ascii && len > 0))
        return sp_fail(ctx, SP_EINVAL, "sp_genome_add: bad arguments (chrom=%d len=%lld)", chrom,
                       (long long)len);
    SP_HIP(ctx, hipSetDevice(ctx->device));
    uint8_t *d = nullptr;
    SP_HIP(ctx, hipMalloc(&d, (size_t)(len > 0 ? len : 1)));
    hipError_t e = hipMemcpyAsync(d, ascii, (size_t)len, hipMemcpyHostToDevice, ctx->stream);
    int rc = SP_OK;
    if (e != hipSuccess) rc = sp_fail(ctx, SP_EHIP, "H2D copy failed: %s", hipGetErrorString(e));
    if (rc == SP_OK) rc = genome_add_impl(ctx, chrom, d, len);
    hipStreamSynchronize(ctx->stream);
    hipFree(d);
    return rc;
}

int sp_genome_len(sp_ctx *ctx, int chrom, int64_t *len) {
    if (!ctx || !len || chrom < 0 || chrom >= (int)ctx->chroms.size())
        return sp_fail(ctx, SP_EINVAL, "sp_genome_len: bad arguments");
    *len = ctx->chroms[(size_t)chrom].len;
    return SP_OK;
}

int sp_genome_unpack(sp_ctx *ctx, int chrom, uint8_t *ascii_out, int64_t len) {
    if (!ctx || chrom < 0 || chrom >= (int)ctx->chroms.size() || !ascii_out)
        return sp_fail(ctx, SP_EINVAL, "sp_genome_unpack: bad arguments");
    sp_chrom &c = ctx->chroms[(size_t)chrom];
    if (len != c.len) return sp_fail(ctx, SP_EINVAL, "sp_genome_unpack: len mismatch");
    if (len == 0) return SP_OK;
    SP_HIP(ctx, hipSetDevice(ctx->device));
    uint8_t *d = nullptr;
    SP_HIP(ctx, hipMalloc(&d, (size_t)len));
    int64_t blocks = (len + 255) / 256;
    if (blocks > 65536) blocks = 65536;
    SP_LAUNCH(ctx, "k0_unpack", k0_unpack, dim3((unsigned)blocks), dim3(256), 0, c.d_pk, c.d_nm, len, d);
    SP_HIP(ctx, hipMemcpyAsync(ascii_out, d, (size_t)len, hipMemcpyDeviceToHost, ctx->stream));
    SP_HIP(ctx, hipStreamSynchronize(ctx->stream));
    hipFree(d);
    return SP_OK;
}

int sp_prof_enable(sp_ctx *ctx, int on) {
    if (!ctx) return SP_EINVAL;
    if (!on) sp_prof_flush(ctx);
    ctx->prof = on != 0;
    return SP_OK;
}
int sp_prof_reset(sp_ctx *ctx) {
    if (!ctx) return SP_EINVAL;
    sp_prof_flush(ctx);
    ctx->prof_acc.clear();
    return SP_OK;
}
int sp_prof_report(sp_ctx *ctx, char *buf, int64_t cap) {
    if (!ctx || !buf || cap < 3) return SP_EINVAL;
    sp_prof_flush(ctx);
    std::string s = "{";
    bool first = true;
    for (auto &kv : ctx->prof_acc) {
        char tmp[256];
        snprintf(tmp, sizeof tmp, "%s\"%s\": {\"calls\": %lld, \"ms\": %.6f}", first ? "" : ", ",
                 kv.first.c_str(), (long long)kv.second.first, kv.second.second);
        s += tmp;
        first = false;
    }
    s += "}";
    if ((int64_t)s.size() + 1 > cap) return sp_fail(ctx, SP_EINVAL, "sp_prof_report: buffer too small");
    memcpy(buf, s.c_str(), s.size() + 1);
    return SP_OK;
}

int sp_host_alloc(sp_ctx *ctx, int64_t bytes, void **h_ptr) {
    if (!ctx || !h_ptr || bytes < 0) return sp_fail(ctx, SP_EINVAL, "sp_host_alloc: bad arguments");
    SP_HIP(ctx, hipSetDevice(ctx->device));
    SP_HIP(ctx, hipHostMalloc(h_ptr, (size_t)(bytes > 0 ? bytes : 1), hipHostMallocDefault));
    return SP_OK;
}
int sp_host_free(sp_ctx *ctx, void *h_ptr) {
    if (!ctx) return SP_EINVAL;
    SP_HIP(ctx, hipHostFree(h_ptr));
    return SP_OK;
}
int sp_host_register(sp_ctx *ctx, void *h_ptr, int64_t bytes) {
    if (!ctx || !h_ptr || bytes <= 0) return sp_fail(ctx, SP_EINVAL, "sp_host_register: bad arguments");
    SP_HIP(ctx, hipSetDevice(ctx->device));
    SP_HIP(ctx, hipHostRegister(h_ptr, (size_t)bytes, hipHostRegisterPortable));
    return SP_OK;
}
int sp_host_unregister(sp_ctx *ctx, void *h_ptr) {
    if (!ctx || !h_ptr) return SP_EINVAL;
    SP_HIP(ctx, hipHostUnregister(h_ptr));
    return SP_OK;
}
int sp_dev_alloc(sp_ctx *ctx, int64_t bytes, void **d_ptr) {
    if (!ctx || !d_ptr || bytes < 0) return sp_fail(ctx, SP_EINVAL, "sp_dev_alloc: bad arguments");
    SP_HIP(ctx, hipSetDevice(ctx->device));
    SP_HIP(ctx, hipMalloc(d_ptr, (size_t)(bytes > 0 ? bytes : 1)));
    return SP_OK;
}
int sp_dev_free(sp_ctx *ctx, void *d_ptr) {
    if (!ctx) return SP_EINVAL;
    SP_HIP(ctx, hipStreamSynchronize(ctx->stream));
    SP_HIP(ctx, hipFree(d_ptr));
    return SP_OK;
}
int sp_dev_copy_to_host(sp_ctx *ctx, void *dst, const void *d_src, int64_t bytes) {
    if (!ctx || !dst || !d_src || bytes < 0) return sp_fail(ctx, SP_EINVAL, "sp_dev_copy_to_host: bad arguments");
    SP_HIP(ctx, hipMemcpyAsync(dst, d_src, (size_t)bytes, hipMemcpyDeviceToHost, ctx->stream));
    SP_HIP(ctx, hipStreamSynchronize(ctx->stream));
    return SP_OK;
}
int sp_dev_copy_from_host(sp_ctx *ctx, void *d_dst, const void *src, int64_t bytes) {
    if (!ctx || !d_dst || !src || bytes < 0) return sp_fail(ctx, SP_EINVAL, "sp_dev_copy_from_host: bad arguments");
    SP_HIP(ctx, hipMemcpyAsync(d_dst, src, (size_t)bytes, hipMemcpyHostToDevice, ctx->stream));
    SP_HIP(ctx, hipStreamSynchronize(ctx->stream));
    return SP_OK;
}
}
```

subphaser_amd/csrc/sp_filter.hip:

```cpp
#include "sp_device.h"
#include "sp_filter.h"
#include "sp_internal.h"

#ifndef F_BLOCK
#define F_BLOCK 256
#endif
#ifndef F_GROUPS_PER_WAVE
#define F_GROUPS_PER_WAVE 64
#endif
#define F_WAVES (F_BLOCK / 64)
#define F_SLOTS_PER_BLOCK (F_WAVES * F_GROUPS_PER_WAVE * 64)
#ifndef F_TILE_BYTES
#define F_TILE_BYTES (24 * 1024)
#endif

#define F3_CHROM_MASK 0xfffff
#define F3_UNIT_END (1 << 20)
#define F3_SET_END (1 << 21)
#define F3_TOT (1 << 22)
#define F3_BI1 (1 << 23)

struct sp_filter_params {
    int C;
    int n_sets;
// ... 288 lines not shown
                        if (!(t < P.min_freq || t > P.max_freq)) {
                            atomicOr(&bmr[sl >> 5], 1u << (sl & 31));
                            nrow++;
                        }
                    }
                }
            }
            __syncthreads();
        }
        const uint32_t q2n = s_q2n;
        if (q2n) {
            const int EW = 1 + (R + 3) / 4;
            if (threadIdx.x == 0) {
                s_q3n = 0;
                s_gq0 = (P.gq && q2n) ? atomicAdd(P.gq_n, (unsigned long long)q2n) : ~0ULL;
            }
            __syncthreads();
            const unsigned long long gq0 = s_gq0;
            for (uint32_t q = threadIdx.x; q < q2n; q += F_BLOCK) {
                const int sl = (int)queue2[q];
                const unsigned long long pos = gq0 == ~0ULL ? ~0ULL : gq0 + q;
                if (pos < P.gq_cap) {
                    uint32_t *e = P.gq + pos * EW;
                    e[0] = (uint32_t)(base + sl);
                    for (int r0 = 0; r0 < R; r0 += 4) {
                        uint32_t w = 0;
                        for (int i = 0; i < 4 && r0 + i < R; i++) w |= (uint32_t)tile[(size_t)(r0 + i) * TS + sl] << (8 * i);
                        e[1 + r0 / 4] = w;
                    }
                } else {
                    queue[atomicAdd(&s_q3n, 1u)] = (uint16_t)sl;
                }
            }
            __syncthreads();
            const uint32_t q3n = s_q3n;
            const int wave = threadIdx.x >> 6;
            uint32_t *mine = resolved + (size_t)wave * R;
            for (uint32_t q = wave; q < q3n; q += F_BLOCK / 64) {
                const int sl = (int)queue[q];
                for (int r = lane; r < R; r += 64) {
                    uint32_t y = tile[(size_t)r * TS + sl];
                    if (y == 255u) y = sp_ovf_lookup(l_ovf[r], (int64_t)l_novf[r], (uint32_t)(P.slot_base + base + sl));
                    mine[r] = y >= P.lower ? y : 0u;
                }
                __builtin_amdgcn_wave_barrier();
                __threadfence_block();
                if (lane == 0) {
                    auto cnt_chrom = [&](int c) -> uint32_t { return mine[P.row_of_chrom[c]]; };
                    unsigned long long tot = 0;
                    for (int r = 0; r < R; r++)
                        if (rowdesc[r] & F3_TOT) tot += mine[r];
                    if (tot) {
                        if (!SWAR) nuni++;
                        bool is_row = false, is_hist = false;
                        sp_filter_decide(cnt_chrom, tot, F, is_row, is_hist);
                        if (is_row) { atomicOr(&bmr[sl >> 5], 1u << (sl & 31)); nrow++; }
                        if (is_hist) { atomicOr(&bmh[sl >> 5], 1u << (sl & 31)); nhist++; }
                    }
                }
                __builtin_amdgcn_wave_barrier();
            }
        }
        __syncthreads();
        for (int i = threadIdx.x; i < TS / 64; i += F_BLOCK) {
            const int64_t g = (base >> 6) + i;
            if ((g << 6) < P.nslots) {
                bm_row[g] = (unsigned long long)bmr[2 * i] | ((unsigned long long)bmr[2 * i + 1] << 32);
                bm_hist[g] = (unsigned long long)bmh[2 * i] | ((unsigned long long)bmh[2 * i + 1] << 32);
            }
        }
        __syncthreads();
    }
    unsigned long long t_row = sp_block_sum_u64(nrow, red);
    unsigned long long t_hist = sp_block_sum_u64(nhist, red);
    unsigned long long t_uni = sp_block_sum_u64(nuni, red);
    if (threadIdx.x == 0) {
        blk_row[blockIdx.x] = t_row;
        blk_hist[blockIdx.x] = t_hist;
        if (t_uni) atomicAdd(n_union, t_uni);
    }
}

__global__ void __launch_bounds__(256)
k3_slow(const sp_tabref *__restrict__ tabs, sp_filter_params P, unsigned long long n_entries,
        const int32_t *__restrict__ set_off, const int32_t *__restrict__ unit_off,
        const int32_t *__restrict__ unit_chrom, const double *__restrict__ unit_den,
        unsigned long long *__restrict__ bm_row, unsigned long long *__restrict__ bm_hist,
        unsigned long long *__restrict__ blk_row, unsigned long long *__restrict__ blk_hist,
        unsigned long long *__restrict__ n_union, int count_union) {
    extern __shared__ uint32_t res[];
    const int R = P.R, EW = 1 + (R + 3) / 4, lane = threadIdx.x & 63, wave = threadIdx.x >> 6;
    uint32_t *mine = res + (size_t)wave * R;
    sp_fsets F;
    F.n_sets = P.n_sets;
    F.n_multi = P.n_multi;
    F.baseline = P.baseline;
    F.set_off = set_off;
    F.unit_off = unit_off;
    F.unit_chrom = unit_chrom;
    F.unit_den = unit_den;
    F.unit_inv = unit_den + set_off[P.n_sets];
    F.min_fold = P.min_fold;
    F.min_freq = P.min_freq;
    F.max_freq = P.max_freq;
    F.ratio = P.ratio;
    for (unsigned long long q = (unsigned long long)blockIdx.x * 4 + wave; q < n_entries; q += (unsigned long long)gridDim.x * 4) {
        const uint32_t *e = P.gq + q * EW;
        const uint32_t sl = e[0];
        for (int r = lane; r < R; r += 64) {
            uint32_t y = (e[1 + r / 4] >> (8 * (r & 3))) & 255u;
            if (y == 255u) {
                const sp_tabref t = tabs[P.rowdesc[r] & F3_CHROM_MASK];
                y = sp_ovf_lookup_t(t, (uint32_t)(P.slot_base + sl));
            }
            mine[r] = y >= P.lower ? y : 0u;
        }
        __builtin_amdgcn_wave_barrier();
        __threadfence_block();
        if (lane == 0) {
            auto cnt_chrom = [&](int c) -> uint32_t { return mine[P.row_of_chrom[c]]; };
            unsigned long long tot = 0;
            for (int r = 0; r < R; r++)
                if (P.rowdesc[r] & F3_TOT) tot += mine[r];
            if (tot) {
                if (count_union) atomicAdd(n_union, 1ULL);
                bool is_row = false, is_hist = false;
                sp_filter_decide(cnt_chrom, tot, F, is_row, is_hist);
                if (is_row) {
                    atomicOr(&bm_row[sl >> 6], 1ULL << (sl & 63));
                    atomicAdd(&blk_row[sl / F_SLOTS_PER_BLOCK], 1ULL);
                }
                if (is_hist) {
                    atomicOr(&bm_hist[sl >> 6], 1ULL << (sl & 63));
                    atomicAdd(&blk_hist[sl / F_SLOTS_PER_BLOCK], 1ULL);
                }
            }
        }
        __builtin_amdgcn_wave_barrier();
    }
}

__global__ void __launch_bounds__(F_BLOCK)
k3_emit_slots(int64_t nslots, const unsigned long long *__restrict__ bm, const unsigned long long *__restrict__ blk_off,
              uint32_t *__restrict__ slots) {
    __shared__ unsigned long long wave_cnt[F_WAVES];
    const int lane = threadIdx.x & 63, wave = threadIdx.x >> 6;
    const int64_t blk_base = (int64_t)blockIdx.x * F_SLOTS_PER_BLOCK;
    const int64_t g0 = (blk_base >> 6) + (int64_t)wave * F_GROUPS_PER_WAVE;
    const int64_t ngroups = (nslots + 63) >> 6;
    unsigned long long mycnt = 0;
    for (int g = lane; g < F_GROUPS_PER_WAVE; g += 64)
        if (g0 + g < ngroups) mycnt += __popcll(bm[g0 + g]);
    for (int o = 32; o > 0; o >>= 1) mycnt += __shfl_down(mycnt, o, 64);
    if (lane == 0) wave_cnt[wave] = mycnt;
    __syncthreads();
    unsigned long long off = blk_off[blockIdx.x];
    for (int w = 0; w < wave; w++) off += wave_cnt[w];
    for (int g = 0; g < F_GROUPS_PER_WAVE; g++) {
        if (g0 + g >= ngroups) break;
        const unsigned long long bits = bm[g0 + g];
        if (bits == 0) continue;
        if ((bits >> lane) & 1ULL)
            slots[off + __popcll(bits & ((1ULL << lane) - 1ULL))] = (uint32_t)(((g0 + g) << 6) + lane);
        off += __popcll(bits);
    }
}

__global__ void __launch_bounds__(256)
k3_emit(const sp_tabref *__restrict__ tabs, int C, uint32_t lower, int64_t M, int64_t slot_base, sp_kparams kp,
        const uint32_t *__restrict__ slots, const double *__restrict__ chrom_len,
        unsigned long long *__restrict__ keys, uint32_t *__restrict__ counts,
        double *__restrict__ freqs, unsigned long long *__restrict__ tots) {
    const int64_t r = (int64_t)blockIdx.x * blockDim.x + threadIdx.x;
    if (r >= M) return;
    const int64_t slot = slots[r];
    unsigned long long tot = 0;
    for (int c = 0; c < C; c++) {
        uint32_t v = sp_tab_count(tabs[c], slot, slot_base);
        v = v >= lower ? v : 0u;
        tot += v;
        if (counts) counts[r * C + c] = v;
        if (freqs) freqs[r * C + c] = (double)v / chrom_len[c];
    }
    if (keys) keys[r] = sp_key_of_slot((uint64_t)(slot_base + slot), kp);
    if (tots) tots[r] = tot;
}

static void free_filter_buffers(sp_ctx *ctx) {
    if (ctx->d_flag_row) hipFree(ctx->d_flag_row);
    if (ctx->d_flag_hist) hipFree(ctx->d_flag_hist);
    if (ctx->d_blk_row) hipFree(ctx->d_blk_row);
    if (ctx->d_blk_hist) hipFree(ctx->d_blk_hist);
    ctx->d_flag_row = ctx->d_flag_hist = nullptr;
    ctx->d_blk_row = ctx->d_blk_hist = nullptr;
    ctx->filtered = false;
}


static int filter_C(sp_ctx *ctx) {
    return ctx->sv_on ? (int)ctx->sv_keys.size() : ctx->fv_on ? (int)ctx->fv_tabs.size() : (int)ctx->chroms.size();
}
static sp_tabref filter_tab(sp_ctx *ctx, int i) {
    if (ctx->fv_on) return ctx->fv_tabs[(size_t)i];
    const sp_chrom &c = ctx->chroms[(size_t)i];
    sp_tabref t;
    t.tab = c.d_tab;
    t.ovf = c.d_ovf;
    t.n_ovf = c.n_ovf;
    t.ovf_idx = (c.ovf_idx_n > 0 && c.ovf_idx_n == ((ctx->nslots + (1LL << SP_OVF_SHIFT) - 1) >> SP_OVF_SHIFT) + 1) ? c.d_ovf_idx : nullptr;
    return t;
}
static int64_t filter_len(sp_ctx *ctx, int i) {
    return (ctx->fv_on || ctx->sv_on) ? ctx->fv_lengths[(size_t)i] : ctx->chroms[(size_t)i].length_sum;
}
static int64_t filter_nslots(sp_ctx *ctx) { return ctx->fv_on ? ctx->fv_nslots : ctx->nslots; }
static int64_t filter_base(sp_ctx *ctx) { return ctx->fv_on ? ctx->fv_slot_base : 0; }

static int upload_tabs(sp_ctx *ctx, const sp_tabref **d_tabs, double **d_len) {
    const size_t C = (size_t)filter_C(ctx);
    size_t bytes = C * sizeof(sp_tabref) + C * sizeof(double);
    void *scr = nullptr;
    int rc = sp_scratch(ctx, (int64_t)bytes + 4096, &scr);
    if (rc) return rc;
    std::vector<sp_tabref> h(C);
    std::vector<double> hl(C);
    for (size_t i = 0; i < C; i++) {
        h[i] = filter_tab(ctx, (int)i);
        hl[i] = (double)filter_len(ctx, (int)i);
    }
    SP_HIP(ctx, hipMemcpyAsync(scr, h.data(), C * sizeof(sp_tabref), hipMemcpyHostToDevice, ctx->stream));
    SP_HIP(ctx, hipMemcpyAsync((char *)scr + C * sizeof(sp_tabref), hl.data(), C * sizeof(double),
                              hipMemcpyHostToDevice, ctx->stream));
    SP_HIP(ctx, hipStreamSynchronize(ctx->stream));
    *d_tabs = (const sp_tabref *)scr;
    *d_len = (double *)((char *)scr + C * sizeof(sp_tabref));
    return SP_OK;
}

extern "C" {

int sp_filter_view(sp_ctx *ctx, int C, const void *const *d_tabs, int64_t slot_base, int64_t nslots_view,
                   const int64_t *lengths, int k, int lower_count, const void *const *d_ovf, const int64_t *n_ovf) {
    if (!ctx) return SP_EINVAL;
    if (d_tabs && C > SP_LIST_MAXC)
        return sp_fail(ctx, SP_EUNSUP, "sp_filter_view: a view takes at most %d chromosomes (got %d); more chromosomes are "
                                       "filtered on one GPU", SP_LIST_MAXC, C);
    if (d_tabs && (ctx->sparse_mode || ctx->list_mode)) return sp_fail(ctx, SP_EUNSUP, "sp_filter_view: byte-table engines (k <= 15) only");
    if (!d_tabs) {
        ctx->fv_on = false;
        ctx->fv_tabs.clear();
        ctx->fv_lengths.clear();
        ctx->filtered = false;
        return SP_OK;
    }
    if (C <= 0 || !lengths || slot_base < 0 || nslots_view <= 0 || (slot_base % 64) != 0 || k < 1 || k > 15)
        return sp_fail(ctx, SP_EINVAL, "sp_filter_view: bad arguments (slot_base must be a multiple of 64)");
    ctx->fv_tabs.assign((size_t)C, sp_tabref());
    ctx->fv_lengths.assign((size_t)C, 0);
    for (int i = 0; i < C; i++) {
        if (!d_tabs[i]) return sp_fail(ctx, SP_EINVAL, "sp_filter_view: table %d is NULL", i);
        if ((uintptr_t)d_tabs[i] & 15) return sp_fail(ctx, SP_EINVAL, "sp_filter_view: table %d is not 16-byte aligned", i);
        sp_tabref t;
        t.tab = (const uint8_t *)d_tabs[i];
        t.ovf = (d_ovf && n_ovf && n_ovf[i] > 0) ? (const uint2 *)d_ovf[i] : nullptr;
        t.n_ovf = (d_ovf && n_ovf && n_ovf[i] > 0) ? n_ovf[i] : 0;
        if (t.n_ovf && !t.ovf) return sp_fail(ctx, SP_EINVAL, "sp_filter_view: overflow list %d is NULL", i);
        ctx->fv_tabs[(size_t)i] = t;
        ctx->fv_lengths[(size_t)i] = lengths[i];
    }
    ctx->fv_slot_base = slot_base;
    ctx->fv_nslots = nslots_view;
    ctx->fv_on = true;
    ctx->filtered = false;
    if (ctx->k == 0) {
        ctx->k = k;
        ctx->nslots = sp_dense_slots(k);
    }
    if (ctx->k != k) return sp_fail(ctx, SP_EINVAL, "sp_filter_view: k=%d but the context counted with k=%d", k, ctx->k);
    ctx->lower = lower_count < 1 ? 1 : lower_count;
    return SP_OK;
}

int sp_filter(sp_ctx *ctx, int n_sets, const int32_t *set_off, const int32_t *unit_off,
              const int32_t *unit_chrom, double min_fold, int baseline, double min_freq,
              double max_freq, double ratio, int64_t *n_union, int64_t *n_rows, int64_t *n_hist) {
    if (!ctx || !set_off || !unit_off || !unit_chrom || n_sets <= 0)
        return sp_fail(ctx, SP_EINVAL, "sp_filter: bad arguments");
    if (!ctx->counted && !ctx->fv_on && !ctx->sv_on) return sp_fail(ctx, SP_EINVAL, "sp_filter: call sp_count first");
    SP_HIP(ctx, hipSetDevice(ctx->device));
    if (ctx->copy_stream) SP_HIP(ctx, hipStreamSynchronize(ctx->copy_stream));
    const int C = filter_C(ctx);
    if (min_freq > max_freq)
        return sp_fail(ctx, SP_ESTATE, "`min_freq` (%g) should be lower than `max_freq` (%g)", min_freq,
                       max_freq);
    int n_single = 0, n_units = set_off[n_sets];
    for (int s = 0; s < n_sets; s++) {
        int nu = set_off[s + 1] - set_off[s];
        if (nu == 1) n_single++;
        if (nu > F_MAXU)
            return sp_fail(ctx, SP_EUNSUP, "a homoeologous set has %d subgenome columns; this build supports <= %d",
                           nu, F_MAXU);
        if (nu > 1) {
            int bi = baseline < 0 ? nu + baseline : baseline;
            if (bi < 0 || bi >= nu) return sp_fail(ctx, SP_ESTATE, "list index out of range (baseline=%d)", baseline);
        }
    }
    if (n_single == n_sets) return sp_fail(ctx, SP_ESTATE, "All singletons are not allowed");
    for (int i = 0; i < C; i++)
        if (filter_len(ctx, i) == 0)
            return sp_fail(ctx, SP_ESTATE, "Chromosomes `[%d]` have only 0 kmers", i);
    const int n_uc = unit_off[n_units];
    for (int j = 0; j < n_uc; j++)
        if (unit_chrom[j] < 0 || unit_chrom[j] >= C)
            return sp_fail(ctx, SP_EINVAL, "sp_filter: chromosome index %d out of range", unit_chrom[j]);

    if (ctx->sparse_mode || ctx->list_mode) {
        std::vector<double> den_s((size_t)n_units * 2);
        for (int u = 0; u < n_units; u++) {
            int64_t d = 0;
            for (int j = unit_off[u]; j < unit_off[u + 1]; j++) d += filter_len(ctx, unit_chrom[j]);
            den_s[(size_t)u] = (double)d;
            den_s[(size_t)(n_units + u)] = 1.0 / (double)d;
        }
        int rcs = sp_sparse_filter(ctx, n_sets, set_off, unit_off, unit_chrom, den_s, min_fold, baseline, min_freq,
                                   max_freq, ratio);
        if (rcs) return rcs;
        if (n_union) *n_union = ctx->n_union;
        if (n_rows) *n_rows = ctx->n_rows;
        if (n_hist) *n_hist = ctx->n_hist;
        return SP_OK;
    }
    if (C > SP_LIST_MAXC)
        return sp_fail(ctx, SP_EUNSUP, "sp_filter: byte tables of %d chromosomes: more than %d chromosomes are filtered as "
                                       "lists only -- k = 9..15, a whole-genome count (engine 0 or 3) into library-owned "
                                       "tables on one GPU; no filter view, bound tables or count engines 1 / 2", C, SP_LIST_MAXC);
    const int64_t nslots = filter_nslots(ctx);
    const int64_t nblk = (nslots + F_SLOTS_PER_BLOCK - 1) / F_SLOTS_PER_BLOCK;
    const int64_t ngroups = (nslots + 63) / 64;
    ctx->filtered = false;
    if (!ctx->d_flag_row || ctx->n_fblocks != nblk) {
        free_filter_buffers(ctx);
        SP_HIP(ctx, hipMalloc(&ctx->d_flag_row, (size_t)ngroups * 8));
        SP_HIP(ctx, hipMalloc(&ctx->d_flag_hist, (size_t)ngroups * 8));
        SP_HIP(ctx, hipMalloc(&ctx->d_blk_row, (size_t)(nblk + 1) * 8));
        SP_HIP(ctx, hipMalloc(&ctx->d_blk_hist, (size_t)(nblk + 1) * 8));
    }
    ctx->n_fblocks = nblk;

    std::vector<double> den((size_t)n_units * 2);
    for (int u = 0; u < n_units; u++) {
        int64_t d = 0;
        for (int j = unit_off[u]; j < unit_off[u + 1]; j++) d += filter_len(ctx, unit_chrom[j]);
        den[(size_t)u] = (double)d;
        den[(size_t)(n_units + u)] = 1.0 / (double)d;
    }
    const size_t uc_room = (size_t)(n_uc > 0 ? n_uc : 1);
    char *d_fs = nullptr;
    sp_tabref *d_tabs = nullptr;
    unsigned long long *d_nuni = nullptr;
    auto lay = [&](sp_carve cv) {
        d_fs = cv.take<char>(sp_fsets_bytes(n_sets, n_units, uc_room));
        d_tabs = cv.take<sp_tabref>((size_t)C);
        d_nuni = cv.take<unsigned long long>(32);
        return cv.off;
    };
    int rcb = sp_buf_ensure(ctx, ctx->b_fpar, (int64_t)lay(sp_carve()));
    if (rcb) return rcb;
    lay(sp_carve(ctx->b_fpar.p));
    std::vector<sp_tabref> htabs((size_t)C);
    for (int i = 0; i < C; i++) htabs[(size_t)i] = filter_tab(ctx, i);
    sp_fsets F;
    hipError_t e = sp_fsets_upload(ctx->stream, d_fs, n_sets, set_off, unit_off, unit_chrom, uc_room, den.data(), min_fold,
                                   baseline, min_freq, max_freq, ratio, F);
    if (e == hipSuccess) e = hipMemcpyAsync(d_tabs, htabs.data(), (size_t)C * sizeof(sp_tabref), hipMemcpyHostToDevice, ctx->stream);
    if (e == hipSuccess) e = hipMemsetAsync(d_nuni, 0, 32, ctx->stream);
    if (e == hipSuccess) e = hipStreamSynchronize(ctx->stream);
    if (e != hipSuccess)
        return sp_fail(ctx, SP_EHIP, "sp_filter: parameter upload failed: %s", hipGetErrorString(e));
    const int32_t *d_set = F.set_off, *d_uo = F.unit_off, *d_uc = F.unit_chrom;
    const double *d_den = F.unit_den;
    sp_filter_params P;
    P.C = C;
    P.n_sets = n_sets;
    P.baseline = baseline;
    P.lower = (uint32_t)ctx->lower;
    P.min_fold = min_fold;
    P.min_freq = min_freq;
    P.max_freq = max_freq;
    P.ratio = ratio;
    P.nslots = nslots;
    P.slot_base = filter_base(ctx);
    int TS = F_SLOTS_PER_BLOCK;
    while (TS > SP_TABLE_MIN_TILE && (size_t)C * TS > F_TILE_BYTES) TS >>= 1;
    if ((size_t)C * TS > SP_TABLE_LDS)
        return sp_fail(ctx, SP_EUNSUP, "sp_filter: %d chromosomes exceed the LDS staging budget (at most %d)", C, SP_TABLE_MAXC);
    P.TS = TS;
    P.n_multi = n_sets - n_single;
    P.need_hist = 0;
    while (P.need_hist <= P.n_multi && (double)P.need_hist / (double)P.n_multi < ratio) P.need_hist++;
    P.need_active = (min_fold > 0 && P.n_multi <= 126) ? P.need_hist : 0;
    std::vector<int32_t> rowdesc, row_of_chrom((size_t)C, -1);
    std::vector<float> rowinv;
    P.fast = 1;
    for (int st = 0; st < n_sets; st++) {
        const int nu = set_off[st + 1] - set_off[st];
        if (nu == 1) continue;
        const int bi = baseline < 0 ? nu + baseline : baseline;
        if (!(bi == 1 || bi == nu - 1)) P.fast = 0;
        for (int u = set_off[st]; u < set_off[st + 1]; u++) {
            if (unit_off[u + 1] == unit_off[u]) P.fast = 0;
            for (int j = unit_off[u]; j < unit_off[u + 1]; j++) {
                const int c = unit_chrom[j];
                int d = c;
                if (row_of_chrom[(size_t)c] < 0) {
                    row_of_chrom[(size_t)c] = (int32_t)rowdesc.size();
                    d |= F3_TOT;
                }
                if (j == unit_off[u + 1] - 1) d |= F3_UNIT_END;
                if (j == unit_off[u + 1] - 1 && u == set_off[st + 1] - 1) d |= F3_SET_END;
                if (bi == 1) d |= F3_BI1;
                rowdesc.push_back(d);
                rowinv.push_back((float)den[(size_t)(n_units + u)]);
            }
        }
    }
    P.R_sets = (int)rowdesc.size();
    for (int c = 0; c < C; c++)
        if (row_of_chrom[(size_t)c] < 0) {
            row_of_chrom[(size_t)c] = (int32_t)rowdesc.size();
            rowdesc.push_back(c | F3_TOT);
            rowinv.push_back(0.0f);
        }
    P.R = (int)rowdesc.size();
    if (C > F3_CHROM_MASK) return sp_fail(ctx, SP_EUNSUP, "sp_filter: too many chromosomes");
    TS = F_SLOTS_PER_BLOCK;
    while (TS > SP_TABLE_MIN_TILE && (size_t)P.R * TS > F_TILE_BYTES) TS >>= 1;
    if ((size_t)P.R * TS > SP_TABLE_LDS)
        return sp_fail(ctx, SP_EUNSUP, "sp_filter: %d chromosome rows exceed the LDS staging budget (at most %d)", P.R,
                       SP_TABLE_MAXC);
    P.TS = TS;
    {
        size_t nR = ((size_t)P.R + 7) & ~(size_t)7;
        if (nR < 32) nR = 32;
        std::vector<int32_t> blob(2 * nR + (size_t)C, 0);
        memcpy(blob.data(), rowdesc.data(), (size_t)P.R * 4);
        memcpy(blob.data() + nR, rowinv.data(), (size_t)P.R * 4);
        memcpy(blob.data() + 2 * nR, row_of_chrom.data(), (size_t)C * 4);
        int rcf = sp_buf_ensure(ctx, ctx->b_fflat, (int64_t)blob.size() * 4 + 64);
        if (rcf) return rcf;
        SP_HIP(ctx, hipMemcpyAsync(ctx->b_fflat.p, blob.data(), blob.size() * 4, hipMemcpyHostToDevice, ctx->stream));
        SP_HIP(ctx, hipStreamSynchronize(ctx->stream));
        P.rowdesc = (const int32_t *)ctx->b_fflat.p;
        P.rowinv = (const float *)(P.rowdesc + nR);
        P.row_of_chrom = P.rowdesc + 2 * nR;
    }
    {
        const int EW = 1 + (P.R + 3) / 4;
        unsigned long long cap = (unsigned long long)(nslots / 64 + 4096);
        int rq = sp_buf_ensure(ctx, ctx->b_fq, (int64_t)(cap * EW * 4 + 64));
        if (rq) return rq;
        P.gq = (uint32_t *)((char *)ctx->b_fq.p + 64);
        P.gq_n = (unsigned long long *)ctx->b_fq.p;
        P.gq_cap = cap;
        SP_HIP(ctx, hipMemsetAsync(ctx->b_fq.p, 0, 64, ctx->stream));
    }
    const size_t shmem = (size_t)P.R * TS + (size_t)TS * 4 + (size_t)TS / 4 + (size_t)P.R * 16 + (size_t)P.R * 4 * F_WAVES;
    const bool swar = ctx->lower >= 1 && ctx->lower <= 128;
    const int nch = (swar && P.fast && P.R <= 32) ? 1 : 0;
#define K3_LAUNCH(SW, N)                                                                                          \
    do {                                                                                                          \
        SP_HIP(ctx, hipFuncSetAttribute((const void *)k3_eval<SW, N>, hipFuncAttributeMaxDynamicSharedMemorySize, \
                                        (int)shmem));                                                             \
        SP_LAUNCH(ctx, "k3_eval", (k3_eval<SW, N>), dim3((unsigned)nblk), dim3(F_BLOCK), shmem,                   \
                  (const sp_tabref *)d_tabs, P, d_set, d_uo, d_uc, d_den, (unsigned long long *)ctx->d_flag_row,  \
                  (unsigned long long *)ctx->d_flag_hist, (unsigned long long *)ctx->d_blk_row,                   \
                  (unsigned long long *)ctx->d_blk_hist, d_nuni);                                                 \
    } while (0)
    if (!swar) K3_LAUNCH(false, 0);
    else if (nch == 1) K3_LAUNCH(true, 1);
    else K3_LAUNCH(true, 0);
#undef K3_LAUNCH
    {
        unsigned long long hq = 0;
        SP_HIP(ctx, hipMemcpyAsync(&hq, P.gq_n, 8, hipMemcpyDeviceToHost, ctx->stream));
        SP_HIP(ctx, hipStreamSynchronize(ctx->stream));
        if (hq > P.gq_cap) hq = P.gq_cap;
        if (hq > 0) {
            unsigned long long nb = (hq + 3) / 4;
            if (nb > (unsigned long long)ctx->n_cu * 32) nb = (unsigned long long)ctx->n_cu * 32;
            SP_LAUNCH(ctx, "k3_slow", k3_slow, dim3((unsigned)nb), dim3(256), (size_t)P.R * 16, (const sp_tabref *)d_tabs, P, hq,
                      d_set, d_uo, d_uc, d_den, (unsigned long long *)ctx->d_flag_row, (unsigned long long *)ctx->d_flag_hist,
                      (unsigned long long *)ctx->d_blk_row, (unsigned long long *)ctx->d_blk_hist, d_nuni, swar ? 0 : 1);
        }
    }
    unsigned long long *d_tot = d_nuni + 1;
    SP_LAUNCH(ctx, "scan_excl_u64", scan_excl_u64, dim3(1), dim3(1024), 0,
              (unsigned long long *)ctx->d_blk_row, nblk, d_tot);
    SP_LAUNCH(ctx, "scan_excl_u64", scan_excl_u64, dim3(1), dim3(1024), 0,
              (unsigned long long *)ctx->d_blk_hist, nblk, d_tot + 1);
    unsigned long long h[3] = {0, 0, 0};
    SP_HIP(ctx, hipMemcpyAsync(h, d_tot, 16, hipMemcpyDeviceToHost, ctx->stream));
    SP_HIP(ctx, hipMemcpyAsync(h + 2, d_nuni, 8, hipMemcpyDeviceToHost, ctx->stream));
    SP_HIP(ctx, hipStreamSynchronize(ctx->stream));
    ctx->n_rows = (int64_t)h[0];
    ctx->n_hist = (int64_t)h[1];
    ctx->n_union = (int64_t)h[2];
    ctx->filtered = true;
    if (n_union) *n_union = ctx->n_union;
    if (n_rows) *n_rows = ctx->n_rows;
    if (n_hist) *n_hist = ctx->n_hist;
    return SP_OK;
}

static int emit_common(sp_ctx *ctx, bool hist, uint64_t *keys, uint32_t *counts, double *freqs,
                       uint64_t *tot, int64_t cap, bool async = false) {
    if (!ctx->filtered) return sp_fail(ctx, SP_EINVAL, "call sp_filter first");
    SP_HIP(ctx, hipSetDevice(ctx->device));
    const int64_t M = hist ? ctx->n_hist : ctx->n_rows;
    if (cap < M) return sp_fail(ctx, SP_EINVAL, "capacity %lld < %lld rows", (long long)cap, (long long)M);
    if (M == 0) return SP_OK;
    if (ctx->sparse_mode || ctx->list_mode) return sp_sparse_fetch(ctx, hist, keys, counts, freqs, tot, async);
    const int C = filter_C(ctx);
    const sp_tabref *d_tabs = nullptr;
    double *d_len = nullptr;
    int rc = upload_tabs(ctx, &d_tabs, &d_len);
    if (rc) return rc;
    unsigned long long *d_keys = nullptr, *d_tot = nullptr;
    uint32_t *d_counts = nullptr;
    double *d_freqs = nullptr;
    auto al = [](size_t x) { return (x + 255) & ~(size_t)255; };
    size_t need = (keys ? al((size_t)M * 8) : 0) + (tot ? al((size_t)M * 8) : 0) +
                  (counts ? al((size_t)M * C * 4) : 0) + (freqs ? al((size_t)M * C * 8) : 0);
    rc = sp_buf_ensure(ctx, ctx->b_emit, (int64_t)need);
    if (rc) return rc;
    {
        char *q = (char *)ctx->b_emit.p;
        if (keys) { d_keys = (unsigned long long *)q; q += al((size_t)M * 8); }
        if (tot) { d_tot = (unsigned long long *)q; q += al((size_t)M * 8); }
        if (counts) { d_counts = (uint32_t *)q; q += al((size_t)M * C * 4); }
        if (freqs) { d_freqs = (double *)q; q += al((size_t)M * C * 8); }
    }
    const sp_kparams kp = sp_make_kparams(ctx->k);
    rc = sp_buf_ensure(ctx, ctx->b_slots, M * 4 + 64);
    if (rc) return rc;
    uint32_t *d_slots = (uint32_t *)ctx->b_slots.p;
    SP_LAUNCH(ctx, "k3_emit_slots", k3_emit_slots, dim3((unsigned)ctx->n_fblocks), dim3(F_BLOCK), 0, filter_nslots(ctx),
              (const unsigned long long *)(hist ? ctx->d_flag_hist : ctx->d_flag_row),
              (const unsigned long long *)(hist ? ctx->d_blk_hist : ctx->d_blk_row), d_slots);
    SP_LAUNCH(ctx, hist ? "k3_emit_hist" : "k3_emit", k3_emit, dim3((unsigned)((M + 255) / 256)), dim3(256), 0, d_tabs, C,
              (uint32_t)ctx->lower, M, filter_base(ctx), kp, (const uint32_t *)d_slots, (const double *)d_len, d_keys,
              d_counts, d_freqs, d_tot);
    hipStream_t cs = ctx->stream;
    if (async) {
        if (!ctx->copy_stream) {
            SP_HIP(ctx, hipStreamCreateWithFlags(&ctx->copy_stream, hipStreamNonBlocking));
            SP_HIP(ctx, hipEventCreateWithFlags(&ctx->copy_event, hipEventDisableTiming));
        }
        SP_HIP(ctx, hipEventRecord(ctx->copy_event, ctx->stream));
        SP_HIP(ctx, hipStreamWaitEvent(ctx->copy_stream, ctx->copy_event, 0));
        cs = ctx->copy_stream;
    }
    if (keys) SP_HIP(ctx, hipMemcpyAsync(keys, d_keys, (size_t)M * 8, hipMemcpyDeviceToHost, cs));
    if (tot) SP_HIP(ctx, hipMemcpyAsync(tot, d_tot, (size_t)M * 8, hipMemcpyDeviceToHost, cs));
    if (counts) SP_HIP(ctx, hipMemcpyAsync(counts, d_counts, (size_t)M * C * 4, hipMemcpyDeviceToHost, cs));
    if (freqs) SP_HIP(ctx, hipMemcpyAsync(freqs, d_freqs, (size_t)M * C * 8, hipMemcpyDeviceToHost, cs));
    if (!async) SP_HIP(ctx, hipStreamSynchronize(ctx->stream));
    return SP_OK;
}

int sp_filter_fetch(sp_ctx *ctx, uint64_t *keys, uint32_t *counts, double *freqs, uint64_t *tot,
                    int64_t cap_rows) {
    if (!ctx) return SP_EINVAL;
    return emit_common(ctx, false, keys, counts, freqs, tot, cap_rows);
}

int sp_filter_fetch_async(sp_ctx *ctx, uint64_t *keys, uint32_t *counts, uint64_t *tot, int64_t cap_rows) {
    if (!ctx) return SP_EINVAL;
    return emit_common(ctx, false, keys, counts, nullptr, tot, cap_rows, true);
}

int sp_filter_fetch_wait(sp_ctx *ctx) {
    if (!ctx) return SP_EINVAL;
    if (ctx->copy_stream) SP_HIP(ctx, hipStreamSynchronize(ctx->copy_stream));
    return SP_OK;
}

int sp_filter_fetch_device(sp_ctx *ctx, void *d_keys, void *d_counts, void *d_tot, int64_t cap_rows) {
    if (!ctx) return SP_EINVAL;
    if (!ctx->filtered) return sp_fail(ctx, SP_EINVAL, "call sp_filter first");
    SP_HIP(ctx, hipSetDevice(ctx->device));
    const int64_t M = ctx->n_rows;
    if (cap_rows < M) return sp_fail(ctx, SP_EINVAL, "capacity %lld < %lld rows", (long long)cap_rows, (long long)M);
    if (M == 0) return SP_OK;
    const int C = filter_C(ctx);
    if (ctx->sparse_mode || ctx->list_mode) {
        if (d_keys) SP_HIP(ctx, hipMemcpyAsync(d_keys, ctx->b_sf_keys.p, (size_t)M * 8, hipMemcpyDeviceToDevice, ctx->stream));
        if (d_counts) SP_HIP(ctx, hipMemcpyAsync(d_counts, ctx->b_sf_counts.p, (size_t)M * C * 4, hipMemcpyDeviceToDevice, ctx->stream));
        if (d_tot) SP_HIP(ctx, hipMemcpyAsync(d_tot, ctx->b_sf_tot.p, (size_t)M * 8, hipMemcpyDeviceToDevice, ctx->stream));
        SP_HIP(ctx, hipStreamSynchronize(ctx->stream));
        return SP_OK;
    }
    const sp_tabref *d_tabs = nullptr;
    double *d_len = nullptr;
    int rc = upload_tabs(ctx, &d_tabs, &d_len);
    if (rc) return rc;
    const sp_kparams kp = sp_make_kparams(ctx->k);
    rc = sp_buf_ensure(ctx, ctx->b_slots, M * 4 + 64);
    if (rc) return rc;
    uint32_t *d_slots = (uint32_t *)ctx->b_slots.p;
    SP_LAUNCH(ctx, "k3_emit_slots", k3_emit_slots, dim3((unsigned)ctx->n_fblocks), dim3(F_BLOCK), 0, filter_nslots(ctx),
              (const unsigned long long *)ctx->d_flag_row, (const unsigned long long *)ctx->d_blk_row, d_slots);
    SP_LAUNCH(ctx, "k3_emit", k3_emit, dim3((unsigned)((M + 255) / 256)), dim3(256), 0, d_tabs, C, (uint32_t)ctx->lower, M,
              filter_base(ctx), kp, (const uint32_t *)d_slots, (const double *)d_len, (unsigned long long *)d_keys,
              (uint32_t *)d_counts, (double *)nullptr, (unsigned long long *)d_tot);
    SP_HIP(ctx, hipStreamSynchronize(ctx->stream));
    return SP_OK;
}

int sp_filter_hist(sp_ctx *ctx, uint64_t *tot, int64_t cap) {
    if (!ctx || !tot) return sp_fail(ctx, SP_EINVAL, "sp_filter_hist: bad arguments");
    return emit_common(ctx, true, nullptr, nullptr, nullptr, tot, cap);
}
}
```

subphaser_amd/csrc/sp_hclust.hip:

```cpp
#include "sp_common.h"
#include "sp_hclust.h"

#include <limits.h>

#define SP_HC_DTHREADS 256
#define SP_HC_T 32
#define SP_HC_DB 32
#define SP_HC_LD (SP_HC_DB + 1)
#define SP_HC_THREADS 1024
#define SP_HC_WAVES (SP_HC_THREADS / SP_WAVE)

__global__ void __launch_bounds__(SP_HC_DTHREADS)
hc_dist(const double *__restrict__ pts, int P, int D, double *__restrict__ dist) {
    __shared__ double s_p[2][SP_HC_T * SP_HC_LD];
    const int tid = threadIdx.x, tx = tid & 15, ty = tid >> 4;
    const int i0 = blockIdx.y * SP_HC_T, j0 = blockIdx.x * SP_HC_T;
    const int ni = min(SP_HC_T, P - i0), nj = min(SP_HC_T, P - j0);
    const bool diag = i0 == j0;
    const double *A = s_p[0], *B = diag ? s_p[0] : s_p[1];
    double acc[2][2] = {{0.0, 0.0}, {0.0, 0.0}};
    for (int d0 = 0; d0 < D; d0 += SP_HC_DB) {
        const int nd = min(SP_HC_DB, D - d0);
        __syncthreads();
        for (int e = tid; e < SP_HC_T * SP_HC_DB; e += SP_HC_DTHREADS) {
// ... 68 lines not shown
            }
        }
        for (int off = 32; off; off >>= 1) {
            const double ov = __shfl_down(bv, off);
            const int oi = __shfl_down(bi, off);
            if (sp_hc_less(ov, oi, bv, bi)) {
                bv = ov;
                bi = oi;
            }
        }
        if ((tid & 63) == 0) {
            s_rv[tid >> 6] = bv;
            s_ri[tid >> 6] = bi;
        }
        __syncthreads();
        if (tid == 0) {
            for (int w = 1; w < SP_HC_WAVES; w++)
                if (sp_hc_less(s_rv[w], s_ri[w], bv, bi)) {
                    bv = s_rv[w];
                    bi = s_ri[w];
                }
            const double cur = prev >= 0 ? s_cur : INFINITY;
            int op;
            scans++;
            const bool push = bi != INT_MAX && bv < cur;
            if (scans > sp_hc_max_scans(P) || (push && len >= P)) {
                status[0] = SP_HC_SCANS;
                op = HC_STOP;
            } else if (push) {
                chain[len++] = bi;
                op = HC_PUSH;
            } else if (prev < 0) {
                status[0] = SP_HC_NONE;
                op = HC_STOP;
            } else {
                len -= 2;
                const int a = min(x, prev), b = max(x, prev);
                const int na = size[a], nb = size[b];
                double *m = merges + 4 * (long long)done;
                m[0] = (double)a;
                m[1] = (double)b;
                m[2] = cur;
                m[3] = (double)(na + nb);
                size[a] = 0;
                size[b] = na + nb;
                s_live[a >> 5] &= ~(1u << (a & 31));
                s_mx = a;
                s_my = b;
                done++;
                op = done == P - 1 ? HC_STOP : HC_MERGE;
            }
            if (op == HC_STOP) status[1] = scans;
            s_op = op;
        }
        __syncthreads();
        const int op = s_op;
        if (op == HC_STOP) break;
        if (op == HC_MERGE) {
            const int mx = s_mx, my = s_my;
            const double *rx = D + (long long)mx * P;
            double *ry = D + (long long)my * P;
            for (int i = tid; i < P; i += SP_HC_THREADS) {
                const double v = sp_hc_max(rx[i], ry[i]);
                if (((s_live[i >> 5] >> (i & 31)) & 1u) && i != my) {
                    ry[i] = v;
                    D[(long long)i * P + my] = v;
                }
            }
        }
    }
}

extern "C" int sp_hclust_complete(sp_ctx *ctx, const double *pts, int P, int D, double *merges, double *dist) {
    if (!ctx || !pts || !merges) return sp_fail(ctx, SP_EINVAL, "sp_hclust_complete: bad arguments");
    if (P < 2 || D < 1) return sp_fail(ctx, SP_EINVAL, "sp_hclust_complete: %d points in %d dimensions (2 and 1 at least)", P, D);
    if (P > SP_HC_MAXP)
        return sp_fail(ctx, SP_EUNSUP, "sp_hclust_complete: %d points (up to %d supported)", P, SP_HC_MAXP);
    const size_t n_pts = (size_t)P * (size_t)D;
    for (size_t i = 0; i < n_pts; i++)
        if (!isfinite(pts[i]))
            return sp_fail(ctx, SP_EINVAL, "sp_hclust_complete: coordinate %d of point %lld is not finite", (int)(i % (size_t)D),
                           (long long)(i / (size_t)D));
    SP_HIP(ctx, hipSetDevice(ctx->device));
    auto layout = [&](sp_carve &cv, double *&d_pts, double *&d_dist, double *&d_merges, int *&d_size, int *&d_chain, long long *&d_status) {
        d_pts = cv.take<double>(n_pts);
        d_dist = cv.take<double>((size_t)P * (size_t)P);
        d_merges = cv.take<double>((size_t)(P - 1) * 4);
        d_size = cv.take<int>((size_t)P);
        d_chain = cv.take<int>((size_t)P);
        d_status = cv.take<long long>(2);
    };
    double *d_pts, *d_dist, *d_merges;
    int *d_size, *d_chain;
    long long *d_status;
    sp_carve sizes;
    layout(sizes, d_pts, d_dist, d_merges, d_size, d_chain, d_status);
    int rc = sp_buf_ensure(ctx, ctx->b_hc, (int64_t)sizes.off);
    if (rc == SP_ENOMEM)
        return sp_fail(ctx, SP_ENOMEM, "sp_hclust_complete: a workspace of %lld bytes (the %d x %d distance matrix and %d x %d points) does not fit on the device",
                       (long long)sizes.off, P, P, P, D);
    if (rc) return rc;
    sp_carve cv(ctx->b_hc.p);
    layout(cv, d_pts, d_dist, d_merges, d_size, d_chain, d_status);
    SP_HIP(ctx, hipMemcpyAsync(d_pts, pts, n_pts * 8, hipMemcpyHostToDevice, ctx->stream));
    SP_HIP(ctx, hipMemsetAsync(d_status, 0, 16, ctx->stream));
    const unsigned n_tiles = (unsigned)((P + SP_HC_T - 1) / SP_HC_T);
    SP_LAUNCH(ctx, "hc_dist", hc_dist, dim3(n_tiles, n_tiles), dim3(SP_HC_DTHREADS), 0, (const double *)d_pts, P, D, d_dist);
    if (dist) SP_HIP(ctx, hipMemcpyAsync(dist, d_dist, (size_t)P * (size_t)P * 8, hipMemcpyDeviceToHost, ctx->stream));
    SP_LAUNCH(ctx, "hc_chain", hc_chain, dim3(1), dim3(SP_HC_THREADS), 0, d_dist, P, d_size, d_chain, d_merges, d_status);
    long long h_status[2] = {0, 0};
    SP_HIP(ctx, hipMemcpyAsync(h_status, d_status, 16, hipMemcpyDeviceToHost, ctx->stream));
    SP_HIP(ctx, hipMemcpyAsync(merges, d_merges, (size_t)(P - 1) * 32, hipMemcpyDeviceToHost, ctx->stream));
    SP_HIP(ctx, hipStreamSynchronize(ctx->stream));
    if (h_status[0] == SP_HC_SCANS)
        return sp_fail(ctx, SP_ESTATE, "sp_hclust_complete: the chain ran %lld scans for %d points (at most %lld expected)",
                       h_status[1], P, (long long)sp_hc_max_scans(P));
    if (h_status[0] != SP_HC_OK)
        return sp_fail(ctx, SP_ESTATE, "sp_hclust_complete: a point has no neighbour at a finite distance (the squared differences overflow)");
    return SP_OK;
}
```

subphaser_amd/csrc/sp_kboot.hip:

```cpp
#include "sp_common.h"
#include "sp_kboot.h"

#define SP_KB_THREADS 256
#define SP_KB_LD (SP_KB_TILE + 1)

template <int MAXC>
__global__ void __launch_bounds__(SP_KB_THREADS)
kb_bootstrap(const double *__restrict__ z, int C, long long M, const long long *__restrict__ cols, int n, int K,
             unsigned long long seed, int *__restrict__ labels, int *__restrict__ iters, double *__restrict__ gram) {
    static_assert(MAXC * SP_KB_LD >= SP_KB_MAXK * MAXC, "the member sums reuse the tile");
    __shared__ double s_g[MAXC * (MAXC + 1) / 2];
    __shared__ double s_tile[MAXC * SP_KB_LD];
    __shared__ double s_closest[MAXC], s_T[SP_KB_MAXK], s_newpot[SP_KB_MAXTRIALS], s_pot;
    __shared__ int s_lab[MAXC], s_centre[SP_KB_MAXK], s_cnt[SP_KB_MAXK], s_cand[SP_KB_MAXTRIALS], s_changed;
    const int tid = threadIdx.x;
    const unsigned long long rep = blockIdx.x;
    const long long *mycols = cols + rep * (unsigned long long)n;
    const int P = C * (C + 1) / 2;

    for (int t0 = 0; t0 < n; t0 += SP_KB_TILE) {
        const int nt = min(SP_KB_TILE, n - t0);
        __syncthreads();
        for (int e = tid; e < C * nt; e += SP_KB_THREADS) {
            const int c = e / nt, t = e - c * nt;
            s_tile[c * SP_KB_LD + t] = z[(long long)c * M + mycols[t0 + t]];
        }
        __syncthreads();
        for (int p = tid; p < P; p += SP_KB_THREADS) {
            int a = (int)((sqrtf(8.0f * (float)p + 1.0f) - 1.0f) * 0.5f);
            while (a * (a + 1) / 2 > p) a--;
            while ((a + 1) * (a + 2) / 2 <= p) a++;
            const int b = p - a * (a + 1) / 2;
            const double *za = s_tile + a * SP_KB_LD, *zb = s_tile + b * SP_KB_LD;
            double acc = t0 ? s_g[p] : 0.0;
            for (int t = 0; t < nt; t++) acc += za[t] * zb[t];
            s_g[p] = acc;
        }
    }
    __syncthreads();
    const sp_kb_half G{s_g};
    if (gram)
        for (int e = tid; e < C * C; e += SP_KB_THREADS) gram[rep * (unsigned long long)(C * C) + e] = G(e / C, e % C);

    double *s_S = s_tile;
    const int trials = sp_kb_trials(K);
    if (tid == 0) s_centre[0] = sp_kb_first_centre(seed, rep, C);
    __syncthreads();
    if (tid < C) s_closest[tid] = sp_kb_d2(G, s_centre[0], tid);
    __syncthreads();
    if (tid == 0) s_pot = sp_kb_potential(s_closest, C);
    __syncthreads();
    for (int c = 1; c < K; c++) {
        if (tid < trials)
            sp_kb_trial(G, C, s_closest, s_pot, sp_kb_u(seed, rep, 1 + (unsigned long long)(c - 1) * trials + tid),
                        &s_cand[tid], &s_newpot[tid]);
        __syncthreads();
        if (tid == 0) {
            const int b = sp_kb_best_trial(s_newpot, trials);
            s_centre[c] = s_cand[b];
            s_pot = s_newpot[b];
        }
        __syncthreads();
        if (tid < C) s_closest[tid] = sp_kb_closer(G, s_centre[c], tid, s_closest[tid]);
        __syncthreads();
    }
    if (tid < C) s_lab[tid] = sp_kb_nearest_centre(G, K, s_centre, tid);
    __syncthreads();

    int it = 0;
    for (;;) {
        it++;
        if (tid == 0) s_changed = 0;
        if (tid < C) sp_kb_point_sums(G, C, K, s_lab, tid, s_S, C);
        __syncthreads();
        if (tid < K) s_cnt[tid] = sp_kb_cluster_total(C, s_lab, tid, s_S, C, &s_T[tid]);
        __syncthreads();
        int next = 0;
        if (tid < C) {
            next = sp_kb_point_assign(G, K, tid, s_S, C, s_T, s_cnt);
            if (next != s_lab[tid]) s_changed = 1;
        }
        __syncthreads();
        if (tid < C) s_lab[tid] = next;
        const int changed = s_changed;
        __syncthreads();
        if (!changed || it >= SP_KB_MAXIT) break;
    }
    if (tid < C) labels[rep * (unsigned long long)C + tid] = s_lab[tid];
    if (tid == 0) iters[rep] = it;
}

extern "C" int sp_kmeans_bootstrap(sp_ctx *ctx, const double *z, int C, int64_t M, const int64_t *cols, int R, int n,
                                   int K, uint64_t seed, int32_t *labels, int32_t *iters, double *gram) {
    if (!ctx || !z || !cols || !labels || !iters || C < 1 || M < 1 || R < 0)
        return sp_fail(ctx, SP_EINVAL, "sp_kmeans_bootstrap: bad arguments");
    if (K < 1 || K > C) return sp_fail(ctx, SP_EINVAL, "sp_kmeans_bootstrap: %d clusters for %d points", K, C);
    if (n < 1) return sp_fail(ctx, SP_EINVAL, "sp_kmeans_bootstrap: %d columns per replicate", n);
    if (C > SP_KB_MAXC || K > SP_KB_MAXK)
        return sp_fail(ctx, SP_EUNSUP, "sp_kmeans_bootstrap: %d points in %d clusters (up to %d in %d supported)", C, K,
                       SP_KB_MAXC, SP_KB_MAXK);
    const size_t ncols = (size_t)R * (size_t)n;
    for (size_t i = 0; i < ncols; i++)
        if (cols[i] < 0 || cols[i] >= M)
            return sp_fail(ctx, SP_EINVAL, "sp_kmeans_bootstrap: column index %lld of replicate %lld outside [0, %lld)",
                           (long long)cols[i], (long long)(i / (size_t)n), (long long)M);
    if (R == 0) return SP_OK;
    SP_HIP(ctx, hipSetDevice(ctx->device));
    const bool on_device = sp_on_device(ctx, z);
    sp_carve sizes;
    auto layout = [&](sp_carve &cv, long long *&d_cols, int *&d_lab, int *&d_it, double *&d_gram) {
        d_cols = cv.take<long long>(ncols);
        d_lab = cv.take<int>((size_t)R * C);
        d_it = cv.take<int>((size_t)R);
        d_gram = gram ? cv.take<double>((size_t)R * C * C) : nullptr;
    };
    long long *d_cols;
    int *d_lab, *d_it;
    double *d_gram;
    layout(sizes, d_cols, d_lab, d_it, d_gram);
    int rc = sp_buf_ensure(ctx, ctx->b_kb, (int64_t)sizes.off);
    if (rc == SP_ENOMEM)
        return sp_fail(ctx, SP_ENOMEM, "sp_kmeans_bootstrap: a workspace of %lld bytes (%d replicates of %d columns) does not fit on the device",
                       (long long)sizes.off, R, n);
    if (rc) return rc;
    sp_carve cv(ctx->b_kb.p);
    layout(cv, d_cols, d_lab, d_it, d_gram);
    const size_t zbytes = (size_t)C * (size_t)M * 8;
    sp_tmp<double> d_z;
    if (!on_device) {
        const hipError_t e = d_z.alloc((size_t)C * (size_t)M);
        if (e != hipSuccess) {
            (void)hipGetLastError();
            return sp_fail(ctx, e == hipErrorOutOfMemory ? SP_ENOMEM : SP_EHIP,
                           "sp_kmeans_bootstrap: the %d x %lld matrix, %lld bytes, does not fit on the device (%s)", C,
                           (long long)M, (long long)zbytes, hipGetErrorString(e));
        }
        SP_HIP(ctx, hipMemcpyAsync(d_z.p, z, zbytes, hipMemcpyHostToDevice, ctx->stream));
    }
    SP_HIP(ctx, hipMemcpyAsync(d_cols, cols, ncols * 8, hipMemcpyHostToDevice, ctx->stream));
    const double *zz = on_device ? z : d_z.p;
    const dim3 grid((unsigned)R), block(SP_KB_THREADS);
    if (C <= 32)
        SP_LAUNCH(ctx, "kb_bootstrap", kb_bootstrap<32>, grid, block, 0, zz, C, (long long)M, (const long long *)d_cols, n, K,
                  (unsigned long long)seed, d_lab, d_it, d_gram);
    else if (C <= 64)
        SP_LAUNCH(ctx, "kb_bootstrap", kb_bootstrap<64>, grid, block, 0, zz, C, (long long)M, (const long long *)d_cols, n, K,
                  (unsigned long long)seed, d_lab, d_it, d_gram);
    else
        SP_LAUNCH(ctx, "kb_bootstrap", kb_bootstrap<SP_KB_MAXC>, grid, block, 0, zz, C, (long long)M,
                  (const long long *)d_cols, n, K, (unsigned long long)seed, d_lab, d_it, d_gram);
    SP_HIP(ctx, hipMemcpyAsync(labels, d_lab, (size_t)R * C * 4, hipMemcpyDeviceToHost, ctx->stream));
    SP_HIP(ctx, hipMemcpyAsync(iters, d_it, (size_t)R * 4, hipMemcpyDeviceToHost, ctx->stream));
    if (gram) SP_HIP(ctx, hipMemcpyAsync(gram, d_gram, (size_t)R * C * C * 8, hipMemcpyDeviceToHost, ctx->stream));
    SP_HIP(ctx, hipStreamSynchronize(ctx->stream));
    return SP_OK;
}
```

subphaser_amd/csrc/sp_kmertest.h:

```cpp
#pragma once
#include <limits.h>

#include "sp_common.h"
#include "sp_ktlayout.h"
#include "sp_ranktest.h"

struct sp_kt_call {
    sp_ctx *ctx;
    const char *who;
    const uint32_t *counts;
    int64_t M;
    int C;
    const int64_t *lengths;
    int n_groups;
    const int32_t *group_off, *group_chrom;
    int32_t *top, *second;
    double *pvals, *means, *stat;
    sp_kt_arrays d;
    const uint32_t *rows;
    std::vector<double> hl;
};
inline int sp_kt_check_groups(const sp_kt_call &k, int max_group, int empty_rc) {
    if (!k.ctx || k.M < 0 || k.C < 1 || k.n_groups < 1 || !k.lengths || !k.group_off || !k.group_chrom ||
        (k.M > 0 && (!k.counts || !k.top || !k.second || !k.pvals || !k.means)))
        return sp_fail(k.ctx, SP_EINVAL, "%s: bad arguments", k.who);
    const sp_kt_verdict v = sp_kt_groups_verdict(k.C, k.n_groups, k.group_off, k.group_chrom, max_group);
    if (v.what == SP_KT_CHROM_RANGE) return sp_fail(k.ctx, SP_EINVAL, "%s: chromosome index out of range", k.who);
    if (v.what == SP_KT_GROUP_BIG || (v.what == SP_KT_GROUP_EMPTY && empty_rc == SP_EUNSUP))
        return sp_fail(k.ctx, SP_EUNSUP, "%s: a subgenome with %d chromosomes (1..%d supported)", k.who, v.n, max_group);
    if (v.what == SP_KT_GROUP_EMPTY) return sp_fail(k.ctx, empty_rc, "%s: subgenome %d has %d chromosomes", k.who, v.g, v.n);
    return SP_OK;
}
inline int sp_kt_check_lengths(const sp_kt_call &k) {
    for (int c = 0; c < k.C; c++)
        if (k.lengths[c] <= 0)
            return sp_fail(k.ctx, SP_EINVAL, "%s: chromosome %d has length %lld", k.who, c, (long long)k.lengths[c]);
    return SP_OK;
}

template <class Extra>
int sp_kt_begin(sp_kt_call &k, bool with_stat, Extra &&extra) {
    sp_ctx *ctx = k.ctx;
    SP_HIP(ctx, hipSetDevice(ctx->device));
    const sp_kt_shape shape{k.M, k.C, k.n_groups, (size_t)k.group_off[k.n_groups], sp_on_device(ctx, k.counts), with_stat};
    sp_carve sizes;
    const size_t need = sp_kt_layout(sizes, shape, k.d, extra);
    const int rc = sp_buf_ensure(ctx, ctx->b_tt, (int64_t)need);
    if (rc == SP_ENOMEM)
        return sp_fail(ctx, SP_ENOMEM, "%s: a workspace of %lld bytes (%lld rows x %d chromosomes%s, %d groups) does not fit on the device",
                       k.who, (long long)need, (long long)k.M, k.C, shape.rows_on_device ? ", read in place" : " and their upload",
                       k.n_groups);
    if (rc) return rc;
    sp_carve cv(ctx->b_tt.p);
    sp_kt_layout(cv, shape, k.d, extra);
    k.rows = shape.rows_on_device ? k.counts : k.d.rows;
    k.hl.assign(k.lengths, k.lengths + k.C);
    if (!shape.rows_on_device)
        SP_HIP(ctx, hipMemcpyAsync(k.d.rows, k.counts, (size_t)k.M * k.C * 4, hipMemcpyHostToDevice, ctx->stream));
    SP_HIP(ctx, hipMemcpyAsync(k.d.len, k.hl.data(), (size_t)k.C * 8, hipMemcpyHostToDevice, ctx->stream));
    SP_HIP(ctx, hipMemcpyAsync(k.d.goff, k.group_off, (size_t)(k.n_groups + 1) * 4, hipMemcpyHostToDevice, ctx->stream));
    SP_HIP(ctx, hipMemcpyAsync(k.d.gch, k.group_chrom, shape.nuc * 4, hipMemcpyHostToDevice, ctx->stream));
    return SP_OK;
}
inline int sp_kt_finish(const sp_kt_call &k) {
    sp_ctx *ctx = k.ctx;
    const size_t M = (size_t)k.M;
    SP_HIP(ctx, hipMemcpyAsync(k.top, k.d.top, M * 4, hipMemcpyDeviceToHost, ctx->stream));
    SP_HIP(ctx, hipMemcpyAsync(k.second, k.d.sec, M * 4, hipMemcpyDeviceToHost, ctx->stream));
    SP_HIP(ctx, hipMemcpyAsync(k.pvals, k.d.p, M * 8, hipMemcpyDeviceToHost, ctx->stream));
    SP_HIP(ctx, hipMemcpyAsync(k.means, k.d.means, M * k.n_groups * 8, hipMemcpyDeviceToHost, ctx->stream));
    if (k.stat) SP_HIP(ctx, hipMemcpyAsync(k.stat, k.d.stat, M * 8, hipMemcpyDeviceToHost, ctx->stream));
    SP_HIP(ctx, hipStreamSynchronize(ctx->stream));
    return SP_OK;
}

struct sp_kt_col {
    double *p;
    int pitch;
    __device__ __forceinline__ double at(int i) const { return p[i * pitch]; }
    __device__ __forceinline__ void set(int i, double x) const { p[i * pitch] = x; }
};
__device__ __forceinline__ double sp_kt_nan() { return __longlong_as_double(0x7ff8000000000000LL); }
struct sp_kt_best {
    int t1 = -1, t2 = -1;
    double k1 = 0, k2 = 0;
};
__device__ __forceinline__ sp_kt_best sp_kt_top2(int g, double key, sp_kt_best b) {
    if (b.t1 < 0 || key > b.k1) { b.t2 = b.t1; b.k2 = b.k1; b.t1 = g; b.k1 = key; }
    else if (b.t2 < 0 || key > b.k2) { b.t2 = g; b.k2 = key; }
    return b;
}
__device__ __forceinline__ void sp_kt_load(const sp_kt_col &col, int at, const uint32_t *__restrict__ row,
                                           const int *__restrict__ gchrom, int o, int n, const double *__restrict__ chrom_len) {
    for (int i = 0; i < n; i++) {
        const int c = gchrom[o + i];
        col.set(at + i, (double)row[c] / chrom_len[c]);
    }
}
struct sp_kt_groups_off {
    const int *__restrict__ goff;
    __device__ __forceinline__ int start(int g) const { return goff[g]; }
    __device__ __forceinline__ int size(int g) const { return goff[g + 1] - goff[g]; }
};
struct sp_kt_groups_even {
    int n;
    __device__ __forceinline__ int start(int g) const { return g * n; }
    __device__ __forceinline__ int size(int) const { return n; }
};
template <class Groups>
__device__ __forceinline__ sp_kt_best sp_kt_means_top2(const sp_kt_col &col, const uint32_t *__restrict__ row,
                                                       const double *__restrict__ chrom_len, int G, const Groups &groups,
                                                       const int *__restrict__ gchrom, double *__restrict__ means_out) {
    sp_kt_best b;
    for (int g = 0; g < G; g++) {
        const int n = groups.size(g);
        sp_kt_load(col, 0, row, gchrom, groups.start(g), n, chrom_len);
        const double mean = sp_rt_np_sum(col, n) / (double)n;
        means_out[g] = mean;
        b = sp_kt_top2(g, mean, b);
    }
    if (b.t2 < 0) b.t2 = b.t1;
    return b;
}
```

subphaser_amd/csrc/sp_kpca.hip:

```cpp
#include "sp_common.h"
#include "sp_kpca.h"

#define SP_KP_THREADS 256
#define SP_KP_COLS 32
#define SP_KP_PITCH (SP_KP_COLS + 1)
#define SP_KP_T 32
#define SP_KP_RB 32
#define SP_KP_LD (SP_KP_T + 1)

__device__ __forceinline__ void kp_stage_counts(const uint32_t *__restrict__ counts, int C, long long row0, int nrows, int c0,
                                                int nc, uint32_t *tile) {
    for (int e = threadIdx.x; e < nrows * nc; e += SP_KP_THREADS) {
        const int r = e / nc, c = e - r * nc;
        tile[r * SP_KP_PITCH + c] = counts[(row0 + r) * (long long)C + c0 + c];
    }
}

__global__ void __launch_bounds__(SP_KP_THREADS)
kp_rowstats(const uint32_t *__restrict__ counts, long long M, int C, const double *__restrict__ len,
            double *__restrict__ stats, unsigned long long *__restrict__ n_bad) {
    __shared__ uint32_t s_tile[SP_KP_THREADS * SP_KP_PITCH];
    __shared__ double s_len[SP_KP_COLS];
    const int tid = threadIdx.x;
    const long long row0 = (long long)blockIdx.x * SP_KP_THREADS;
// ... 157 lines not shown
            const uint32_t *row = s_tile + tid * SP_KP_PITCH;
            for (int c = 0; c < nc; c++) {
                const double z = sp_kp_z(row[c], s_len[c], mean, sd);
#pragma unroll
                for (int j = 0; j < NC; j++) v[j] += s_U[c * NC + j] * z;
            }
        }
    }
#pragma unroll
    for (int j = 0; j < NC; j++) {
        if (j < n_comp) {
            kp_cand x;
            x.ab = good ? fabs(v[j]) : -1.0;
            x.row = good ? row0 + tid : LLONG_MAX;
            x.v = v[j];
            x = kp_block_best(x, s_red);
            if (tid == 0) {
                cand_row[(long long)blockIdx.x * n_comp + j] = x.row;
                cand_val[(long long)blockIdx.x * n_comp + j] = x.ab < 0.0 ? NAN : x.v;
            }
        }
    }
}

__global__ void __launch_bounds__(SP_KP_THREADS)
kp_signs_final(const long long *__restrict__ cand_row, const double *__restrict__ cand_val, long long n_blocks, int n_comp,
               long long *__restrict__ rows, double *__restrict__ vals) {
    __shared__ kp_cand s_red[SP_KP_THREADS / 64];
    const int j = blockIdx.x;
    kp_cand x{-1.0, LLONG_MAX, 0.0};
    for (long long k = threadIdx.x; k < n_blocks; k += SP_KP_THREADS) {
        const double v = cand_val[k * n_comp + j];
        if (v != v) continue;
        kp_take(x, kp_cand{fabs(v), cand_row[k * n_comp + j], v});
    }
    x = kp_block_best(x, s_red);
    if (threadIdx.x == 0) {
        rows[j] = x.ab < 0.0 ? -1 : x.row;
        vals[j] = x.ab < 0.0 ? 0.0 : x.v;
    }
}

namespace {
int kp_check(sp_ctx *ctx, const char *who, const uint32_t *counts, int64_t M, int C, const int64_t *lengths) {
    if (!ctx || !counts || !lengths) return sp_fail(ctx, SP_EINVAL, "%s: bad arguments", who);
    if (M < 1) return sp_fail(ctx, SP_EINVAL, "%s: %lld rows", who, (long long)M);
    if (C < 2) return sp_fail(ctx, SP_EINVAL, "%s: %d chromosomes (a PCA needs two)", who, C);
    if (C > SP_KP_MAXC) return sp_fail(ctx, SP_EUNSUP, "%s: %d chromosomes (up to %d supported)", who, C, SP_KP_MAXC);
    for (int c = 0; c < C; c++)
        if (lengths[c] <= 0) return sp_fail(ctx, SP_EINVAL, "%s: chromosome %d has length %lld", who, c, (long long)lengths[c]);
    return SP_OK;
}
int kp_rows(sp_ctx *ctx, const char *who, const uint32_t *counts, int64_t M, int C, sp_tmp<uint32_t> &up, const uint32_t **out) {
    if (sp_on_device(ctx, counts)) {
        *out = counts;
        return SP_OK;
    }
    const size_t n = (size_t)M * (size_t)C;
    const hipError_t e = up.alloc(n);
    if (e != hipSuccess) {
        (void)hipGetLastError();
        return sp_fail(ctx, e == hipErrorOutOfMemory ? SP_ENOMEM : SP_EHIP, "%s: the %lld x %d rows, %lld bytes, do not fit on the device (%s)",
                       who, (long long)M, C, (long long)(n * 4), hipGetErrorString(e));
    }
    SP_HIP(ctx, hipMemcpyAsync(up.p, counts, n * 4, hipMemcpyHostToDevice, ctx->stream));
    *out = up.p;
    return SP_OK;
}
int kp_launch_stats(sp_ctx *ctx, const uint32_t *d_counts, int64_t M, int C, const double *d_len, double *d_stats,
                    unsigned long long *d_bad) {
    SP_HIP(ctx, hipMemsetAsync(d_bad, 0, 8, ctx->stream));
    SP_LAUNCH(ctx, "kp_rowstats", kp_rowstats, dim3((unsigned)((M + SP_KP_THREADS - 1) / SP_KP_THREADS)), dim3(SP_KP_THREADS), 0,
              d_counts, (long long)M, C, d_len, d_stats, d_bad);
    return SP_OK;
}
}

extern "C" int sp_kmer_pca_gram(sp_ctx *ctx, const uint32_t *counts, int64_t M, int C, const int64_t *lengths, double *gram,
                                int64_t *n_bad, double *stats) {
    int rc = kp_check(ctx, "sp_kmer_pca_gram", counts, M, C, lengths);
    if (rc) return rc;
    if (!gram || !n_bad) return sp_fail(ctx, SP_EINVAL, "sp_kmer_pca_gram: bad arguments");
    SP_HIP(ctx, hipSetDevice(ctx->device));
    const int64_t n_chunks = sp_kp_chunks(M), P = sp_kp_tri(C - 1, C - 1) + 1;
    const int n_tiles = (C + SP_KP_T - 1) / SP_KP_T, n_tpairs = n_tiles * (n_tiles + 1) / 2;
    auto layout = [&](sp_carve &cv, double *&d_len, double *&d_stats, double *&d_part, double *&d_gram, unsigned long long *&d_bad) {
        d_len = cv.take<double>((size_t)C);
        d_stats = cv.take<double>((size_t)M * 2);
        d_part = cv.take<double>((size_t)n_chunks * (size_t)P);
        d_gram = cv.take<double>((size_t)C * C);
        d_bad = cv.take<unsigned long long>(1);
    };
    double *d_len, *d_stats, *d_part, *d_gram;
    unsigned long long *d_bad;
    sp_carve sizes;
    layout(sizes, d_len, d_stats, d_part, d_gram, d_bad);
    rc = sp_buf_ensure(ctx, ctx->b_kp, (int64_t)sizes.off);
    if (rc == SP_ENOMEM)
        return sp_fail(ctx, SP_ENOMEM, "sp_kmer_pca_gram: a workspace of %lld bytes (%lld chunks x %lld pairs x 8 and %lld rows x 16) does not fit on the device",
                       (long long)sizes.off, (long long)n_chunks, (long long)P, (long long)M);
    if (rc) return rc;
    sp_carve cv(ctx->b_kp.p);
    layout(cv, d_len, d_stats, d_part, d_gram, d_bad);
    sp_tmp<uint32_t> up;
    const uint32_t *d_counts;
    rc = kp_rows(ctx, "sp_kmer_pca_gram", counts, M, C, up, &d_counts);
    if (rc) return rc;
    std::vector<double> hl((size_t)C);
    for (int c = 0; c < C; c++) hl[(size_t)c] = (double)lengths[c];
    SP_HIP(ctx, hipMemcpyAsync(d_len, hl.data(), (size_t)C * 8, hipMemcpyHostToDevice, ctx->stream));
    rc = kp_launch_stats(ctx, d_counts, M, C, d_len, d_stats, d_bad);
    if (rc) return rc;
    SP_LAUNCH(ctx, "kp_gram", kp_gram, dim3((unsigned)n_chunks, (unsigned)n_tpairs), dim3(SP_KP_THREADS), 0, d_counts, (long long)M,
              C, (const double *)d_len, (const double *)d_stats, d_part);
    SP_LAUNCH(ctx, "kp_gram_sum", kp_gram_sum, dim3((unsigned)((P + SP_KP_THREADS - 1) / SP_KP_THREADS)), dim3(SP_KP_THREADS), 0,
              (const double *)d_part, (long long)n_chunks, C, d_gram);
    unsigned long long h_bad = 0;
    SP_HIP(ctx, hipMemcpyAsync(gram, d_gram, (size_t)C * C * 8, hipMemcpyDeviceToHost, ctx->stream));
    SP_HIP(ctx, hipMemcpyAsync(&h_bad, d_bad, 8, hipMemcpyDeviceToHost, ctx->stream));
    if (stats) SP_HIP(ctx, hipMemcpyAsync(stats, d_stats, (size_t)M * 16, hipMemcpyDeviceToHost, ctx->stream));
    SP_HIP(ctx, hipStreamSynchronize(ctx->stream));
    *n_bad = (int64_t)h_bad;
    return SP_OK;
}

extern "C" int sp_kmer_pca_signs(sp_ctx *ctx, const uint32_t *counts, int64_t M, int C, const int64_t *lengths, const double *U,
                                 int n_comp, int64_t *rows, double *vals) {
    int rc = kp_check(ctx, "sp_kmer_pca_signs", counts, M, C, lengths);
    if (rc) return rc;
    if (!U || !rows || !vals) return sp_fail(ctx, SP_EINVAL, "sp_kmer_pca_signs: bad arguments");
    if (n_comp < 1 || n_comp > SP_KP_MAXCOMP)
        return sp_fail(ctx, SP_EINVAL, "sp_kmer_pca_signs: %d components (1..%d)", n_comp, SP_KP_MAXCOMP);
    SP_HIP(ctx, hipSetDevice(ctx->device));
    const int64_t n_blocks = (M + SP_KP_THREADS - 1) / SP_KP_THREADS;
    auto layout = [&](sp_carve &cv, double *&d_len, double *&d_stats, double *&d_U, long long *&d_crow, double *&d_cval,
                      long long *&d_rows, double *&d_vals, unsigned long long *&d_bad) {
        d_len = cv.take<double>((size_t)C);
        d_stats = cv.take<double>((size_t)M * 2);
        d_U = cv.take<double>((size_t)C * n_comp);
        d_crow = cv.take<long long>((size_t)n_blocks * n_comp);
        d_cval = cv.take<double>((size_t)n_blocks * n_comp);
        d_rows = cv.take<long long>((size_t)n_comp);
        d_vals = cv.take<double>((size_t)n_comp);
        d_bad = cv.take<unsigned long long>(1);
    };
    double *d_len, *d_stats, *d_U, *d_cval, *d_vals;
    long long *d_crow, *d_rows;
    unsigned long long *d_bad;
    sp_carve sizes;
    layout(sizes, d_len, d_stats, d_U, d_crow, d_cval, d_rows, d_vals, d_bad);
    rc = sp_buf_ensure(ctx, ctx->b_kp, (int64_t)sizes.off);
    if (rc == SP_ENOMEM)
        return sp_fail(ctx, SP_ENOMEM, "sp_kmer_pca_signs: a workspace of %lld bytes (%lld rows, %d components) does not fit on the device",
                       (long long)sizes.off, (long long)M, n_comp);
    if (rc) return rc;
    sp_carve cv(ctx->b_kp.p);
    layout(cv, d_len, d_stats, d_U, d_crow, d_cval, d_rows, d_vals, d_bad);
    sp_tmp<uint32_t> up;
    const uint32_t *d_counts;
    rc = kp_rows(ctx, "sp_kmer_pca_signs", counts, M, C, up, &d_counts);
    if (rc) return rc;
    std::vector<double> hl((size_t)C);
    for (int c = 0; c < C; c++) hl[(size_t)c] = (double)lengths[c];
    SP_HIP(ctx, hipMemcpyAsync(d_len, hl.data(), (size_t)C * 8, hipMemcpyHostToDevice, ctx->stream));
    SP_HIP(ctx, hipMemcpyAsync(d_U, U, (size_t)C * n_comp * 8, hipMemcpyHostToDevice, ctx->stream));
    rc = kp_launch_stats(ctx, d_counts, M, C, d_len, d_stats, d_bad);
    if (rc) return rc;
    const dim3 grid((unsigned)n_blocks), block(SP_KP_THREADS);
    if (n_comp <= 4)
        SP_LAUNCH(ctx, "kp_signs", kp_signs<4>, grid, block, 0, d_counts, (long long)M, C, (const double *)d_len,
                  (const double *)d_stats, (const double *)d_U, n_comp, d_crow, d_cval);
    else
        SP_LAUNCH(ctx, "kp_signs", kp_signs<SP_KP_MAXCOMP>, grid, block, 0, d_counts, (long long)M, C, (const double *)d_len,
                  (const double *)d_stats, (const double *)d_U, n_comp, d_crow, d_cval);
    SP_LAUNCH(ctx, "kp_signs_final", kp_signs_final, dim3((unsigned)n_comp), block, 0, (const long long *)d_crow,
              (const double *)d_cval, (long long)n_blocks, n_comp, d_rows, d_vals);
    static_assert(sizeof(long long) == sizeof(int64_t), "rows are copied out as they are");
    SP_HIP(ctx, hipMemcpyAsync(rows, d_rows, (size_t)n_comp * 8, hipMemcpyDeviceToHost, ctx->stream));
    SP_HIP(ctx, hipMemcpyAsync(vals, d_vals, (size_t)n_comp * 8, hipMemcpyDeviceToHost, ctx->stream));
    SP_HIP(ctx, hipStreamSynchronize(ctx->stream));
    return SP_OK;
}
```

subphaser_amd/csrc/sp_sparse.hip:

```cpp
#include <algorithm>
#include <cstring>
#include <utility>
#include <rocprim/rocprim.hpp>

#include "sp_device.h"
#include "sp_internal.h"
#include "sp_lists.h"
#include "sp_map.h"

__global__ void __launch_bounds__(256)
sps_keygen(const uint32_t *__restrict__ pk, const uint32_t *__restrict__ nm, int64_t n_units, sp_kparams kp,
           unsigned long long *__restrict__ keys ,
           unsigned long long *__restrict__ n_valid) {
    __shared__ unsigned long long red[16];
    unsigned long long nv = 0;
    for (int64_t u = (int64_t)blockIdx.x * blockDim.x + threadIdx.x; u < n_units;
         u += (int64_t)gridDim.x * blockDim.x) {
        sp_scan_unit64<SP_UNIT>(pk, nm, u * SP_UNIT, kp, [&](int64_t start, uint64_t fwd, uint64_t rc) {
            keys[start] = fwd < rc ? fwd : rc;
            nv++;
        });
    }
    unsigned long long t = sp_block_sum_u64(nv, red);
    if (threadIdx.x == 0 && t) atomicAdd(n_valid, t);
// ... 1009 lines not shown
    const int64_t stride = (int64_t)gridDim.x * blockDim.x;
    for (; u < n_units; u += stride) {
        const unsigned long long cv = cov[u];
        if (__all(cv == 0ULL)) continue;
        unsigned long long lab[3] = {0ULL, 0ULL, 0ULL};
        map_unit_scan64_h<TABLE>(pk, pm, nm, u * SP_UNIT, kp, bloom, bloom_bits, htab, hmask, T, lab, ulds, cv);
        for (int sg = 0; sg < S; sg++) {
            const int l = sg + 1;
            masks[u * S + sg] = ((l & 1) ? lab[0] : ~lab[0]) & ((l & 2) ? lab[1] : ~lab[1]) & ((l & 4) ? lab[2] : ~lab[2]) & cv;
        }
    }
}

int sp_sparse_mask_launch(sp_ctx *ctx, sp_chrom &c, int64_t n_units, int S, const unsigned long long *d_cov,
                          unsigned long long *d_masks) {
    const sp_kparams kp = sp_make_kparams(ctx->k);
    int64_t grid = (n_units + MAP_BLOCK - 1) / MAP_BLOCK;
    if (grid > (int64_t)ctx->n_cu * 16) grid = (int64_t)ctx->n_cu * 16;
    if (ctx->map_engine == 0 && S <= 7) {
        const sq_tab T = sq_tab_of(ctx);
        if (T.buckets)
            SP_LAUNCH(ctx, "k5_map_mask_sparse", k5_map_mask_sparse2<1>, dim3((unsigned)grid), dim3(MAP_BLOCK), 0, (const uint32_t *)c.d_pk,
                      (const uint32_t *)c.d_pm, (const uint32_t *)c.d_nm, kp, n_units, S, (unsigned long long *)ctx->d_hkeys,
                      (uint64_t)(ctx->hcap - 1), T, (const uint32_t *)ctx->d_bloom, ctx->bloom_bits, d_cov, d_masks);
        else
            SP_LAUNCH(ctx, "k5_map_mask_sparse", k5_map_mask_sparse2<0>, dim3((unsigned)grid), dim3(MAP_BLOCK), 0, (const uint32_t *)c.d_pk,
                      (const uint32_t *)c.d_pm, (const uint32_t *)c.d_nm, kp, n_units, S, (unsigned long long *)ctx->d_hkeys,
                      (uint64_t)(ctx->hcap - 1), T, (const uint32_t *)ctx->d_bloom, ctx->bloom_bits, d_cov, d_masks);
        return SP_OK;
    }
    if (ctx->map_engine == 0) return sp_fail(ctx, SP_ESTATE, "k > 15 map: the pair-keyed table holds at most 7 subgenomes");
    SP_LAUNCH(ctx, "k5_map_mask_sparse_lab", k5_map_mask_sparse_lab, dim3((unsigned)grid), dim3(MAP_BLOCK), 0, (const uint32_t *)c.d_pk,
              (const uint32_t *)c.d_nm, kp, n_units, S, (unsigned long long *)ctx->d_hkeys, (uint64_t)(ctx->hcap - 1),
              (const uint32_t *)ctx->d_bloom, ctx->bloom_bits, d_cov, d_masks);
    return SP_OK;
}

int sp_sparse_hit(sp_ctx *ctx, unsigned long long *d_n) {
    if (ctx->map_engine == 0 && ctx->sq_bb) {
        if (ctx->n_labels > 0)
            SP_LAUNCH(ctx, "sq_seen", sq_seen, dim3((unsigned)(ctx->n_cu * 4)), dim3(256), 0,
                      (const unsigned long long *)ctx->b_labkeys.p, ctx->n_labels, ctx->k, sq_tab_of(ctx), d_n);
        return SP_OK;
    }
    if (ctx->map_engine == 0) {
        if (ctx->n_labels > 0)
            SP_LAUNCH(ctx, "sps_pair_seen", sps_pair_seen, dim3((unsigned)(ctx->n_cu * 4)), dim3(256), 0,
                      (const unsigned long long *)ctx->b_labkeys.p, ctx->n_labels, ctx->k,
                      (const unsigned long long *)ctx->d_hkeys, (uint64_t)(ctx->hcap - 1), d_n);
        return SP_OK;
    }
    SP_LAUNCH(ctx, "sps_count_seen", sps_count_seen, dim3((unsigned)(ctx->n_cu * 4)), dim3(256), 0,
              (const unsigned long long *)ctx->d_hkeys, ctx->hcap, d_n);
    return SP_OK;
}

__global__ void sps_lower_bound(const unsigned long long *__restrict__ keys, int64_t n,
                                const unsigned long long *__restrict__ q, int nq, long long *__restrict__ out) {
    const int i = blockIdx.x * blockDim.x + threadIdx.x;
    if (i >= nq) return;
    const unsigned long long x = q[i];
    int64_t lo = 0, hi = n;
    while (lo < hi) {
        const int64_t mid = (lo + hi) >> 1;
        if (keys[mid] < x) lo = mid + 1;
        else hi = mid;
    }
    out[i] = lo;
}

extern "C" {

int sp_sparse_sizes(sp_ctx *ctx, int64_t *n) {
    if (!ctx || !n) return sp_fail(ctx, SP_EINVAL, "sp_sparse_sizes: bad arguments");
    if (!ctx->sparse_mode || !ctx->counted) return sp_fail(ctx, SP_EINVAL, "sp_sparse_sizes: call sp_count with k > 15 first");
    for (size_t c = 0; c < ctx->sparse.size(); c++) n[c] = ctx->sparse[c].n;
    return SP_OK;
}

int sp_sparse_sample(sp_ctx *ctx, int chrom, int64_t n_samples, uint64_t *keys, int64_t *n_out) {
    if (!ctx || !keys || !n_out || n_samples < 1 || chrom < 0 || chrom >= (int)ctx->sparse.size())
        return sp_fail(ctx, SP_EINVAL, "sp_sparse_sample: bad arguments");
    SP_HIP(ctx, hipSetDevice(ctx->device));
    const sp_sparse_chrom &o = ctx->sparse[(size_t)chrom];
    const int64_t stride = o.n / n_samples;
    if (stride < 1) {
        if (o.n) SP_HIP(ctx, hipMemcpyAsync(keys, o.d_keys, (size_t)o.n * 8, hipMemcpyDeviceToHost, ctx->stream));
        *n_out = o.n;
    } else {
        SP_HIP(ctx, hipMemcpy2DAsync(keys, 8, o.d_keys, (size_t)stride * 8, 8, (size_t)n_samples, hipMemcpyDeviceToHost,
                                     ctx->stream));
        *n_out = n_samples;
    }
    SP_HIP(ctx, hipStreamSynchronize(ctx->stream));
    return SP_OK;
}

int sp_sparse_split(sp_ctx *ctx, int chrom, const uint64_t *splitters, int n_split, int64_t *bounds) {
    if (!ctx || !bounds || n_split < 0 || (n_split > 0 && !splitters) || n_split > 4096 || chrom < 0 ||
        chrom >= (int)ctx->sparse.size())
        return sp_fail(ctx, SP_EINVAL, "sp_sparse_split: bad arguments");
    SP_HIP(ctx, hipSetDevice(ctx->device));
    const sp_sparse_chrom &o = ctx->sparse[(size_t)chrom];
    bounds[0] = 0;
    bounds[n_split + 1] = o.n;
    if (n_split == 0) return SP_OK;
    void *scr = nullptr;
    int rc = sp_scratch(ctx, (int64_t)n_split * 16 + 256, &scr);
    if (rc) return rc;
    unsigned long long *d_q = (unsigned long long *)scr;
    long long *d_out = (long long *)(d_q + n_split);
    SP_HIP(ctx, hipMemcpyAsync(d_q, splitters, (size_t)n_split * 8, hipMemcpyHostToDevice, ctx->stream));
    SP_LAUNCH(ctx, "sps_lower_bound", sps_lower_bound, dim3((unsigned)((n_split + 63) / 64)), dim3(64), 0,
              (const unsigned long long *)o.d_keys, o.n, (const unsigned long long *)d_q, n_split, d_out);
    SP_HIP(ctx, hipMemcpyAsync(bounds + 1, d_out, (size_t)n_split * 8, hipMemcpyDeviceToHost, ctx->stream));
    SP_HIP(ctx, hipStreamSynchronize(ctx->stream));
    return SP_OK;
}

int sp_sparse_export(sp_ctx *ctx, int chrom, int64_t first, int64_t count, void *d_keys, void *d_counts) {
    if (!ctx || chrom < 0 || chrom >= (int)ctx->sparse.size() || first < 0 || count < 0)
        return sp_fail(ctx, SP_EINVAL, "sp_sparse_export: bad arguments");
    const sp_sparse_chrom &o = ctx->sparse[(size_t)chrom];
    if (first + count > o.n) return sp_fail(ctx, SP_EINVAL, "sp_sparse_export: range exceeds the list (%lld)", (long long)o.n);
    if (count == 0) return SP_OK;
    if (!d_keys || !d_counts) return sp_fail(ctx, SP_EINVAL, "sp_sparse_export: NULL destination");
    SP_HIP(ctx, hipSetDevice(ctx->device));
    SP_HIP(ctx, hipMemcpyAsync(d_keys, o.d_keys + first, (size_t)count * 8, hipMemcpyDeviceToDevice, ctx->stream));
    SP_HIP(ctx, hipMemcpyAsync(d_counts, o.d_cnts + first, (size_t)count * 4, hipMemcpyDeviceToDevice, ctx->stream));
    return SP_OK;
}

int sp_sparse_view(sp_ctx *ctx, int C, const void *const *d_keys, const void *const *d_counts, const int64_t *n,
                   const int64_t *lengths, int k, int lower_count) {
    if (!ctx) return SP_EINVAL;
    if (!d_keys) {
        ctx->sv_on = false;
        ctx->sv_keys.clear();
        ctx->sv_cnts.clear();
        ctx->sv_n.clear();
        ctx->fv_lengths.clear();
        ctx->filtered = false;
        return SP_OK;
    }
    if (C <= 0 || !d_counts || !n || !lengths || k < 16 || k > 32)
        return sp_fail(ctx, SP_EINVAL, "sp_sparse_view: bad arguments (k = 16..32)");
    if (C > SP_LIST_MAXC)
        return sp_fail(ctx, SP_EUNSUP, "sp_sparse_view: a view takes at most %d chromosomes (got %d); more chromosomes are "
                                       "filtered on one GPU", SP_LIST_MAXC, C);
    if (ctx->fv_on) return sp_fail(ctx, SP_EINVAL, "sp_sparse_view: a dense filter view is active");
    if (ctx->k != 0 && ctx->k != k) return sp_fail(ctx, SP_EINVAL, "sp_sparse_view: k=%d but the context counted with k=%d", k, ctx->k);
    for (int i = 0; i < C; i++)
        if (n[i] < 0 || (n[i] > 0 && (!d_keys[i] || !d_counts[i])))
            return sp_fail(ctx, SP_EINVAL, "sp_sparse_view: list %d is NULL", i);
    ctx->sv_keys.assign((size_t)C, nullptr);
    ctx->sv_cnts.assign((size_t)C, nullptr);
    ctx->sv_n.assign((size_t)C, 0);
    ctx->fv_lengths.assign((size_t)C, 0);
    for (int i = 0; i < C; i++) {
        ctx->sv_keys[(size_t)i] = (const uint64_t *)d_keys[i];
        ctx->sv_cnts[(size_t)i] = (const uint32_t *)d_counts[i];
        ctx->sv_n[(size_t)i] = n[i];
        ctx->fv_lengths[(size_t)i] = lengths[i];
    }
    if (ctx->k == 0) {
        ctx->k = k;
        ctx->sparse_mode = true;
    }
    ctx->lower = lower_count < 1 ? 1 : lower_count;
    ctx->sv_on = true;
    ctx->filtered = false;
    return SP_OK;
}

}
```

subphaser_amd/csrc/sp_synth.hip:

```cpp
#include "sp_device.h"

__host__ __device__ inline uint64_t synth_mix(uint64_t x) {
    x += 0x9E3779B97F4A7C15ULL;
    x = (x ^ (x >> 30)) * 0xBF58476D1CE4E5B9ULL;
    x = (x ^ (x >> 27)) * 0x94D049BB133111EBULL;
    return x ^ (x >> 31);
}
__host__ __device__ inline uint64_t synth_h(uint64_t seed, uint64_t stream, uint64_t idx) {
    return synth_mix(synth_mix(seed ^ (stream * 0xD6E8FEB86659FD93ULL)) + idx);
}

#define SYN_SEG 1024
#define SYN_FAMILIES 200

struct sp_synth_params {
    int64_t len;
    int64_t start, n;
    uint64_t seed;
    int set_id, sg_id, n_sg, chrom_id, exchange;
};

__host__ __device__ inline uint8_t synth_base(int64_t p, const sp_synth_params &P) {
    if (p < 100000 || p >= P.len - 100000) return (uint8_t)("TTTAGGG"[p % 7]);
    if (p >= 50000000 && (p % 50000000) < 1000) return (uint8_t)'N';
    const uint64_t q = (uint64_t)(p / SYN_SEG);
    const uint64_t hq = synth_h(P.seed, 100 + (uint64_t)P.chrom_id, q);
    const unsigned cls = (unsigned)(hq % 100);
    unsigned base;
    bool lower = false;
    if (cls < 40) {
        base = (unsigned)(synth_h(P.seed, 1000 + (uint64_t)P.set_id, (uint64_t)p) & 3);
        uint64_t r = synth_h(P.seed, 2000 + (uint64_t)P.set_id * 64 + (uint64_t)P.sg_id, (uint64_t)p);
        if ((r & 0xffff) < 5243) base = (base + 1 + (unsigned)((r >> 16) % 3)) & 3;
    } else {
        unsigned lib;
        if (cls < 65) {
            lib = (unsigned)P.sg_id;
            if (P.exchange && p >= P.len / 10 * 6 && p < P.len / 10 * 7) lib = (unsigned)((P.sg_id + 1) % P.n_sg);
        } else {
            lib = 255;
        }
        const double u = (double)((hq >> 8) & 0xffffff) / 16777216.0;
        unsigned f = (unsigned)(exp(u * 5.303304908059076) ) - 1;
        if (f >= SYN_FAMILIES) f = SYN_FAMILIES - 1;
        const unsigned nblk = 1 + f % 8;
        const unsigned blk = (unsigned)((hq >> 40) % nblk);
        const uint64_t cpos = (uint64_t)blk * SYN_SEG + (uint64_t)(p % SYN_SEG);
        base = (unsigned)(synth_h(P.seed, 5000 + (uint64_t)lib * 1024 + f, cpos) & 3);
        const unsigned div16 = (unsigned)(((hq >> 32) & 0xff) * 3932 / 255);
        uint64_t r = synth_h(P.seed, 3000 + (uint64_t)P.chrom_id, (uint64_t)p);
        if ((r & 0xffff) < div16) base = (base + 1 + (unsigned)((r >> 16) % 3)) & 3;
        lower = ((hq >> 52) % 10) < 3;
    }
    uint8_t ch = (uint8_t)("ACGT"[base]);
    return lower ? (uint8_t)(ch | 0x20) : ch;
}

__global__ void __launch_bounds__(256)
synth_fill(uint8_t *__restrict__ out, sp_synth_params P) {
    int64_t t = (int64_t)blockIdx.x * blockDim.x + threadIdx.x;
    const int64_t stride = (int64_t)gridDim.x * blockDim.x;
    const int64_t n16 = (P.n + 15) / 16;
    const bool aligned = (((uintptr_t)out) & 15) == 0;
    for (; t < n16; t += stride) {
        int64_t p0 = t * 16;
        if (aligned && p0 + 16 <= P.n) {
            uint32_t w[4];
#pragma unroll
            for (int q = 0; q < 4; q++) {
                uint32_t v = 0;
#pragma unroll
                for (int j = 0; j < 4; j++) v |= (uint32_t)synth_base(P.start + p0 + q * 4 + j, P) << (8 * j);
                w[q] = v;
            }
            *reinterpret_cast<uint4 *>(out + p0) = make_uint4(w[0], w[1], w[2], w[3]);
        } else {
            for (int j = 0; j < 16 && p0 + j < P.n; j++) out[p0 + j] = synth_base(P.start + p0 + j, P);
        }
    }
}

extern "C" int sp_synth_chrom_range(sp_ctx *ctx, uint8_t *d_out, int64_t len, int64_t start, int64_t n, uint64_t seed,
                                    int set_id, int sg_id, int n_sg, int chrom_id, int exchange) {
    if (!ctx || !d_out || len <= 0 || n_sg < 1 || start < 0 || n < 0 || start + n > len)
        return sp_fail(ctx, SP_EINVAL, "sp_synth_chrom_range: bad arguments");
    if (n == 0) return SP_OK;
    SP_HIP(ctx, hipSetDevice(ctx->device));
    sp_synth_params P;
    P.len = len;
    P.start = start;
    P.n = n;
    P.seed = seed;
    P.set_id = set_id;
    P.sg_id = sg_id;
    P.n_sg = n_sg;
    P.chrom_id = chrom_id;
    P.exchange = exchange;
    int64_t blocks = ((n + 15) / 16 + 255) / 256;
    if (blocks > (int64_t)ctx->n_cu * 32) blocks = (int64_t)ctx->n_cu * 32;
    SP_LAUNCH(ctx, "synth_fill", synth_fill, dim3((unsigned)blocks), dim3(256), 0, d_out, P);
    return SP_OK;
}

extern "C" int sp_synth_chrom(sp_ctx *ctx, uint8_t *d_out, int64_t len, uint64_t seed, int set_id,
                              int sg_id, int n_sg, int chrom_id, int exchange) {
    if (len <= 0) return sp_fail(ctx, SP_EINVAL, "sp_synth_chrom: bad arguments");
    return sp_synth_chrom_range(ctx, d_out, len, 0, len, seed, set_id, sg_id, n_sg, chrom_id, exchange);
}
```

Baseline: 158.5.

## Remove host sync before k3_slow and overlap async filter fetch with later work

The k3_slow launch no longer reads the queue count back to the host. It now launches at full queue capacity and reads the count on the device, which removes a blocking host-device round trip inside sp_filter. Async fetch now records separate events for when rows are ready and when they have been sent. Other API entry points join on the rows event instead of fully synchronising the copy stream, so host copies can overlap with later compute. The cost is a k3_slow grid sized to capacity rather than actual load, extra join calls throughout the API, and a new queue-stats diagnostic.

```diff
diff --git a/include/subphaser_hip.h b/include/subphaser_hip.h
--- a/include/subphaser_hip.h
+++ b/include/subphaser_hip.h
@@ -57,6 +57,7 @@
 int sp_filter_fetch_wait(sp_ctx *ctx);
 int sp_filter_fetch_device(sp_ctx *ctx, void *d_keys, void *d_counts, void *d_tot, int64_t cap_rows);
 int sp_filter_hist(sp_ctx *ctx, uint64_t *tot, int64_t cap);
+int sp_filter_queue_stats(sp_ctx *ctx, int64_t *pushed, int64_t *cap);
 
 int sp_labels_set(sp_ctx *ctx, const uint64_t *keys, const uint8_t *sg, int64_t n, int n_sg);
 int sp_labels_set_device(sp_ctx *ctx, const uint64_t *d_keys, const uint8_t *d_sg, int64_t n, int n_sg);
diff --git a/subphaser_amd/_native.py b/subphaser_amd/_native.py
--- a/subphaser_amd/_native.py
+++ b/subphaser_amd/_native.py
@@ -19,7 +19,7 @@
     "sp_version", "sp_last_error", "sp_ctx_create", "sp_ctx_destroy", "sp_sync", "sp_stream",
     "sp_genome_reset", "sp_genome_add", "sp_genome_add_device", "sp_genome_len", "sp_genome_unpack",
     "sp_count", "sp_count_range", "sp_count_recounts", "sp_nslots", "sp_tables_bind", "sp_table_overflow", "sp_table_merge", "sp_table_lengths", "sp_lengths", "sp_dump_size", "sp_dump",
-    "sp_filter_view", "sp_filter", "sp_filter_fetch", "sp_filter_fetch_async", "sp_filter_fetch_wait", "sp_filter_fetch_device", "sp_filter_hist",
+    "sp_filter_view", "sp_filter", "sp_filter_fetch", "sp_filter_fetch_async", "sp_filter_fetch_wait", "sp_filter_fetch_device", "sp_filter_hist", "sp_filter_queue_stats",
     "sp_labels_set", "sp_labels_set_device", "sp_map_nslots", "sp_map_bins", "sp_map_bins_all", "sp_stack_windows", "sp_stack_windows_dev", "sp_stack_enrich", "sp_map_features", "sp_map_intervals", "sp_labels_hit",
     "sp_enrich", "sp_enrich_dev", "sp_kmer_ttest", "sp_kmer_ttest_wide", "sp_kmer_ranktest", "sp_kmer_wilcoxon", "sp_kmeans_bootstrap", "sp_kmer_pca_gram", "sp_kmer_pca_signs", "sp_hclust_complete",
     "sp_sparse_sizes", "sp_sparse_sample", "sp_sparse_split", "sp_sparse_export", "sp_sparse_view",
@@ -90,6 +90,8 @@
     L.sp_filter_fetch_async.argtypes = [vp, vp, vp, vp, i64]
     L.sp_filter_fetch_wait.argtypes = [vp]
     L.sp_filter_hist.argtypes = [vp, vp, i64]
+    if hasattr(L, "sp_filter_queue_stats"):
+        L.sp_filter_queue_stats.argtypes = [vp, P(i64), P(i64)]
     L.sp_labels_set.argtypes = [vp, vp, vp, i64, ci]
     L.sp_labels_set_device.argtypes = [vp, vp, vp, i64, ci]
     L.sp_map_nslots.argtypes = [vp, ci, i64, i64, P(i64)]
@@ -139,6 +141,8 @@
     L.sp_text_repr.argtypes = [vp, i64, vp, vp]
     L.sp_text_table.argtypes = [vp, ci, i64, ci, ci, P(i64)]
     for name in SYMBOLS:
+        if name == "sp_filter_queue_stats" and not hasattr(L, name):
+            continue
         if name not in ("sp_last_error", "sp_stream", "sp_fasta_close"):
             getattr(L, name).restype = ci
     _lib = L
@@ -553,6 +557,11 @@
         v = lambda p: C.c_void_p(int(p)) if p else None
         self._ck(self.L.sp_filter_fetch_device(self.h, v(d_keys), v(d_counts), v(d_tot), int(n_rows)))
 
+    def filter_queue_stats(self):
+        n, cap = C.c_int64(), C.c_int64()
+        self._ck(self.L.sp_filter_queue_stats(self.h, C.byref(n), C.byref(cap)))
+        return n.value, cap.value
+
     def filter_hist(self, n_hist):
         tot = np.empty(n_hist, np.uint64)
         self._ck(self.L.sp_filter_hist(self.h, _p(tot), n_hist))
diff --git a/subphaser_amd/csrc/sp_common.h b/subphaser_amd/csrc/sp_common.h
--- a/subphaser_amd/csrc/sp_common.h
+++ b/subphaser_amd/csrc/sp_common.h
@@ -80,6 +80,10 @@
     hipStream_t stream = nullptr;
     hipStream_t copy_stream = nullptr;
     hipEvent_t copy_event = nullptr;
+    hipEvent_t rows_event = nullptr, sent_event = nullptr;
+    bool rows_pending = false;
+    bool sent_pending = false;
+    sp_buf b_ftabs;
     bool own_stream = false;
     int n_cu = 256;
     std::string err;
@@ -99,6 +103,7 @@
     std::vector<int64_t> sv_n;
     bool filtered = false;
     int64_t n_union = 0, n_rows = 0, n_hist = 0;
+    int64_t fq_cap = 0;
     uint32_t *d_flag_row = nullptr;
     uint32_t *d_flag_hist = nullptr;
     uint64_t *d_blk_row = nullptr;
@@ -155,6 +160,9 @@
                 ctx->stream = ln->stream;
             }
         }
+        lane_scope(sp_ctx *c, hipStream_t s) : ctx(c), saved(c->stream) {
+            if (s) ctx->stream = s;
+        }
         lane_scope(const lane_scope &) = delete;
         lane_scope &operator=(const lane_scope &) = delete;
         ~lane_scope() {
@@ -193,6 +201,8 @@
 int sp_buf_ensure(sp_ctx *ctx, sp_buf &b, int64_t bytes);
 void sp_buf_free(sp_buf &b);
 bool sp_on_device(sp_ctx *ctx, const void *p);
+int sp_fetch_join(sp_ctx *ctx);
+int sp_fetch_drain(sp_ctx *ctx);
 void sp_prof_begin(sp_ctx *ctx, const char *name);
 void sp_prof_end(sp_ctx *ctx);
 void sp_prof_flush(sp_ctx *ctx);
diff --git a/subphaser_amd/csrc/sp_count.hip b/subphaser_amd/csrc/sp_count.hip
--- a/subphaser_amd/csrc/sp_count.hip
+++ b/subphaser_amd/csrc/sp_count.hip
@@ -483,7 +483,7 @@
     sp_chrom &c = ctx->chroms[ci];
     sp_ctx::lane_t *ln = J.n_lanes > 0 ? &ctx->lanes[ci % (size_t)J.n_lanes] : nullptr;
     if (ln && c.ev_packed) SP_HIP(ctx, hipStreamWaitEvent(ln->stream, c.ev_packed, 0));
-    if (ln && ctx->copy_event) SP_HIP(ctx, hipStreamWaitEvent(ln->stream, ctx->copy_event, 0));
+    if (ln && ctx->rows_event) SP_HIP(ctx, hipStreamWaitEvent(ln->stream, ctx->rows_event, 0));
     return count_chrom_chain(ctx, J, ci, ln);
 }
 
@@ -550,6 +550,10 @@
     if (lower_count < 1) lower_count = 1;
     if (ctx->chroms.empty()) return sp_fail(ctx, SP_EINVAL, "sp_count: no chromosomes loaded");
     SP_HIP(ctx, hipSetDevice(ctx->device));
+    {
+        const int rcj = sp_fetch_join(ctx);
+        if (rcj) return rcj;
+    }
     if (first < 0 || last > (int)ctx->chroms.size() || first > last)
         return sp_fail(ctx, SP_EINVAL, "sp_count_range: bad chromosome range [%d, %d)", first, last);
     if (k > 15) {
@@ -700,6 +704,8 @@
     SP_HIP(ctx, hipSetDevice(ctx->device));
     sp_chrom &c = ctx->chroms[(size_t)chrom];
     if (c.d_tab && !c.tab_external) {
+        const int rcj = sp_fetch_join(ctx);
+        if (rcj) return rcj;
         SP_HIP(ctx, hipStreamSynchronize(ctx->stream));
         hipFree(c.d_tab);
     }
@@ -719,6 +725,8 @@
     if (!d_pairs) return SP_OK;
     if (cap < c.n_ovf) return sp_fail(ctx, SP_EINVAL, "sp_table_overflow: capacity %lld < %lld", (long long)cap, (long long)c.n_ovf);
     SP_HIP(ctx, hipSetDevice(ctx->device));
+    const int rcj = sp_fetch_join(ctx);
+    if (rcj) return rcj;
     if (c.n_ovf)
         SP_HIP(ctx, hipMemcpyAsync(d_pairs, c.d_ovf, (size_t)c.n_ovf * sizeof(uint2), hipMemcpyDeviceToDevice, ctx->stream));
     return SP_OK;
@@ -734,6 +742,8 @@
     *n_out = 0;
     if (n == 0) return SP_OK;
     SP_HIP(ctx, hipSetDevice(ctx->device));
+    const int rcj = sp_fetch_join(ctx);
+    if (rcj) return rcj;
     const int64_t n_buckets = (n + (1LL << SP_OVF_SHIFT) - 1) >> SP_OVF_SHIFT;
     int rc = sp_buf_ensure(ctx, ctx->b_ovfw, (cap + 1) * 8 + (3 * n_buckets + 1) * 4 + 256);
     if (rc) return rc;
@@ -765,6 +775,8 @@
     *sum = *n_dump = 0;
     if (n == 0) return SP_OK;
     SP_HIP(ctx, hipSetDevice(ctx->device));
+    const int rcj = sp_fetch_join(ctx);
+    if (rcj) return rcj;
     void *scr = nullptr;
     int rc = sp_scratch(ctx, 256, &scr);
     if (rc) return rc;
@@ -801,6 +813,8 @@
         return sp_fail(ctx, SP_EINVAL, "sp_dump: bad arguments");
     if (!ctx->counted) return sp_fail(ctx, SP_EINVAL, "sp_dump: call sp_count first");
     SP_HIP(ctx, hipSetDevice(ctx->device));
+    const int rcj = sp_fetch_join(ctx);
+    if (rcj) return rcj;
     sp_chrom &c = ctx->chroms[(size_t)chrom];
     *n = c.n_dump;
     if (cap < c.n_dump) return sp_fail(ctx, SP_EINVAL, "sp_dump: capacity %lld < %lld", (long long)cap,
diff --git a/subphaser_amd/csrc/sp_ctx.hip b/subphaser_amd/csrc/sp_ctx.hip
--- a/subphaser_amd/csrc/sp_ctx.hip
+++ b/subphaser_amd/csrc/sp_ctx.hip
@@ -57,6 +57,22 @@
     b.cap = 0;
 }
 
+int sp_fetch_join(sp_ctx *ctx) {
+    if (!ctx || !ctx->rows_pending) return SP_OK;
+    SP_HIP(ctx, hipStreamWaitEvent(ctx->stream, ctx->rows_event, 0));
+    for (auto &ln : ctx->lanes)
+        if (ln.stream) SP_HIP(ctx, hipStreamWaitEvent(ln.stream, ctx->rows_event, 0));
+    ctx->rows_pending = false;
+    return SP_OK;
+}
+
+int sp_fetch_drain(sp_ctx *ctx) {
+    if (!ctx || !ctx->copy_stream) return SP_OK;
+    SP_HIP(ctx, hipStreamSynchronize(ctx->copy_stream));
+    ctx->rows_pending = ctx->sent_pending = false;
+    return SP_OK;
+}
+
 void sp_prof_begin(sp_ctx *ctx, const char *name) {
     if (!ctx->prof) return;
     sp_prof_entry e;
@@ -73,6 +89,7 @@
 void sp_prof_flush(sp_ctx *ctx) {
     if (ctx->prof_pending.empty()) return;
     hipStreamSynchronize(ctx->stream);
+    if (ctx->copy_stream) hipStreamSynchronize(ctx->copy_stream);
     for (auto &e : ctx->prof_pending) {
         float ms = 0.f;
         hipEventElapsedTime(&ms, e.e0, e.e1);
@@ -140,6 +157,7 @@
 int sp_ctx_destroy(sp_ctx *ctx) {
     if (!ctx) return SP_OK;
     hipSetDevice(ctx->device);
+    if (ctx->copy_stream) hipStreamSynchronize(ctx->copy_stream);
     hipStreamSynchronize(ctx->stream);
     sp_prof_flush(ctx);
     for (auto &c : ctx->chroms) free_chrom(c);
@@ -192,17 +210,22 @@
     sp_buf_free(ctx->b_kp);
     sp_buf_free(ctx->b_hc);
     sp_buf_free(ctx->b_win);
+    sp_buf_free(ctx->b_ftabs);
     if (ctx->copy_stream) {
-        hipStreamSynchronize(ctx->copy_stream);
         hipStreamDestroy(ctx->copy_stream);
         hipEventDestroy(ctx->copy_event);
     }
+    if (ctx->rows_event) hipEventDestroy(ctx->rows_event);
+    if (ctx->sent_event) hipEventDestroy(ctx->sent_event);
     if (ctx->own_stream) hipStreamDestroy(ctx->stream);
     delete ctx;
     return SP_OK;
 }
 
 int sp_sync(sp_ctx *ctx) {
+    if (!ctx) return SP_EINVAL;
+    int rcj = sp_fetch_join(ctx);
+    if (rcj) return rcj;
     SP_HIP(ctx, hipStreamSynchronize(ctx->stream));
     return SP_OK;
 }
@@ -212,6 +235,8 @@
 int sp_genome_reset(sp_ctx *ctx, int n_chrom) {
     if (!ctx || n_chrom < 0) return sp_fail(ctx, SP_EINVAL, "sp_genome_reset: bad arguments");
     SP_HIP(ctx, hipSetDevice(ctx->device));
+    int rcj = sp_fetch_join(ctx);
+    if (rcj) return rcj;
     SP_HIP(ctx, hipStreamSynchronize(ctx->stream));
     if ((size_t)n_chrom == ctx->chroms.size()) {
         for (auto &c : ctx->chroms) {
@@ -349,6 +374,8 @@
         return sp_fail(ctx, SP_EINVAL, "sp_genome_add_device: bad arguments (chrom=%d len=%lld)", chrom,
                        (long long)len);
     SP_HIP(ctx, hipSetDevice(ctx->device));
+    int rcj = sp_fetch_join(ctx);
+    if (rcj) return rcj;
     return genome_add_impl(ctx, chrom, d_ascii, len);
 }
 
@@ -357,6 +384,8 @@
         return sp_fail(ctx, SP_EINVAL, "sp_genome_add: bad arguments (chrom=%d len=%lld)", chrom,
                        (long long)len);
     SP_HIP(ctx, hipSetDevice(ctx->device));
+    int rcj = sp_fetch_join(ctx);
+    if (rcj) return rcj;
     uint8_t *d = nullptr;
     SP_HIP(ctx, hipMalloc(&d, (size_t)(len > 0 ? len : 1)));
     hipError_t e = hipMemcpyAsync(d, ascii, (size_t)len, hipMemcpyHostToDevice, ctx->stream);
@@ -382,6 +411,8 @@
     if (len != c.len) return sp_fail(ctx, SP_EINVAL, "sp_genome_unpack: len mismatch");
     if (len == 0) return SP_OK;
     SP_HIP(ctx, hipSetDevice(ctx->device));
+    int rcj = sp_fetch_join(ctx);
+    if (rcj) return rcj;
     uint8_t *d = nullptr;
     SP_HIP(ctx, hipMalloc(&d, (size_t)len));
     int64_t blocks = (len + 255) / 256;
@@ -431,6 +462,8 @@
 }
 int sp_host_free(sp_ctx *ctx, void *h_ptr) {
     if (!ctx) return SP_EINVAL;
+    int rcj = sp_fetch_drain(ctx);
+    if (rcj) return rcj;
     SP_HIP(ctx, hipHostFree(h_ptr));
     return SP_OK;
 }
@@ -442,6 +475,8 @@
 }
 int sp_host_unregister(sp_ctx *ctx, void *h_ptr) {
     if (!ctx || !h_ptr) return SP_EINVAL;
+    int rcj = sp_fetch_drain(ctx);
+    if (rcj) return rcj;
     SP_HIP(ctx, hipHostUnregister(h_ptr));
     return SP_OK;
 }
@@ -453,18 +488,24 @@
 }
 int sp_dev_free(sp_ctx *ctx, void *d_ptr) {
     if (!ctx) return SP_EINVAL;
+    int rcj = sp_fetch_join(ctx);
+    if (rcj) return rcj;
     SP_HIP(ctx, hipStreamSynchronize(ctx->stream));
     SP_HIP(ctx, hipFree(d_ptr));
     return SP_OK;
 }
 int sp_dev_copy_to_host(sp_ctx *ctx, void *dst, const void *d_src, int64_t bytes) {
     if (!ctx || !dst || !d_src || bytes < 0) return sp_fail(ctx, SP_EINVAL, "sp_dev_copy_to_host: bad arguments");
+    int rcj = sp_fetch_join(ctx);
+    if (rcj) return rcj;
     SP_HIP(ctx, hipMemcpyAsync(dst, d_src, (size_t)bytes, hipMemcpyDeviceToHost, ctx->stream));
     SP_HIP(ctx, hipStreamSynchronize(ctx->stream));
     return SP_OK;
 }
 int sp_dev_copy_from_host(sp_ctx *ctx, void *d_dst, const void *src, int64_t bytes) {
     if (!ctx || !d_dst || !src || bytes < 0) return sp_fail(ctx, SP_EINVAL, "sp_dev_copy_from_host: bad arguments");
+    int rcj = sp_fetch_join(ctx);
+    if (rcj) return rcj;
     SP_HIP(ctx, hipMemcpyAsync(d_dst, src, (size_t)bytes, hipMemcpyHostToDevice, ctx->stream));
     SP_HIP(ctx, hipStreamSynchronize(ctx->stream));
     return SP_OK;
diff --git a/subphaser_amd/csrc/sp_filter.hip b/subphaser_amd/csrc/sp_filter.hip
--- a/subphaser_amd/csrc/sp_filter.hip
+++ b/subphaser_amd/csrc/sp_filter.hip
@@ -394,7 +394,7 @@
 }
 
 __global__ void __launch_bounds__(256)
-k3_slow(const sp_tabref *__restrict__ tabs, sp_filter_params P, unsigned long long n_entries,
+k3_slow(const sp_tabref *__restrict__ tabs, sp_filter_params P,
         const int32_t *__restrict__ set_off, const int32_t *__restrict__ unit_off,
         const int32_t *__restrict__ unit_chrom, const double *__restrict__ unit_den,
         unsigned long long *__restrict__ bm_row, unsigned long long *__restrict__ bm_hist,
@@ -403,6 +403,8 @@
     extern __shared__ uint32_t res[];
     const int R = P.R, EW = 1 + (R + 3) / 4, lane = threadIdx.x & 63, wave = threadIdx.x >> 6;
     uint32_t *mine = res + (size_t)wave * R;
+    unsigned long long n_entries = *P.gq_n;
+    if (n_entries > P.gq_cap) n_entries = P.gq_cap;
     sp_fsets F;
     F.n_sets = P.n_sets;
     F.n_multi = P.n_multi;
@@ -531,9 +533,9 @@
 static int upload_tabs(sp_ctx *ctx, const sp_tabref **d_tabs, double **d_len) {
     const size_t C = (size_t)filter_C(ctx);
     size_t bytes = C * sizeof(sp_tabref) + C * sizeof(double);
-    void *scr = nullptr;
-    int rc = sp_scratch(ctx, (int64_t)bytes + 4096, &scr);
+    int rc = sp_buf_ensure(ctx, ctx->b_ftabs, (int64_t)bytes + 4096);
     if (rc) return rc;
+    void *scr = ctx->b_ftabs.p;
     std::vector<sp_tabref> h(C);
     std::vector<double> hl(C);
     for (size_t i = 0; i < C; i++) {
@@ -600,7 +602,11 @@
         return sp_fail(ctx, SP_EINVAL, "sp_filter: bad arguments");
     if (!ctx->counted && !ctx->fv_on && !ctx->sv_on) return sp_fail(ctx, SP_EINVAL, "sp_filter: call sp_count first");
     SP_HIP(ctx, hipSetDevice(ctx->device));
-    if (ctx->copy_stream) SP_HIP(ctx, hipStreamSynchronize(ctx->copy_stream));
+    {
+        const int rcj = sp_fetch_join(ctx);
+        if (rcj) return rcj;
+    }
+    if (ctx->copy_stream && (ctx->sparse_mode || ctx->list_mode)) SP_HIP(ctx, hipStreamSynchronize(ctx->copy_stream));
     const int C = filter_C(ctx);
     if (min_freq > max_freq)
         return sp_fail(ctx, SP_ESTATE, "`min_freq` (%g) should be lower than `max_freq` (%g)", min_freq,
@@ -651,6 +657,7 @@
     const int64_t ngroups = (nslots + 63) / 64;
     ctx->filtered = false;
     if (!ctx->d_flag_row || ctx->n_fblocks != nblk) {
+        SP_HIP(ctx, hipStreamSynchronize(ctx->stream));
         free_filter_buffers(ctx);
         SP_HIP(ctx, hipMalloc(&ctx->d_flag_row, (size_t)ngroups * 8));
         SP_HIP(ctx, hipMalloc(&ctx->d_flag_hist, (size_t)ngroups * 8));
@@ -793,17 +800,11 @@
     else K3_LAUNCH(true, 0);
 #undef K3_LAUNCH
     {
-        unsigned long long hq = 0;
-        SP_HIP(ctx, hipMemcpyAsync(&hq, P.gq_n, 8, hipMemcpyDeviceToHost, ctx->stream));
-        SP_HIP(ctx, hipStreamSynchronize(ctx->stream));
-        if (hq > P.gq_cap) hq = P.gq_cap;
-        if (hq > 0) {
-            unsigned long long nb = (hq + 3) / 4;
-            if (nb > (unsigned long long)ctx->n_cu * 32) nb = (unsigned long long)ctx->n_cu * 32;
-            SP_LAUNCH(ctx, "k3_slow", k3_slow, dim3((unsigned)nb), dim3(256), (size_t)P.R * 16, (const sp_tabref *)d_tabs, P, hq,
-                      d_set, d_uo, d_uc, d_den, (unsigned long long *)ctx->d_flag_row, (unsigned long long *)ctx->d_flag_hist,
-                      (unsigned long long *)ctx->d_blk_row, (unsigned long long *)ctx->d_blk_hist, d_nuni, swar ? 0 : 1);
-        }
+        unsigned long long nb = (P.gq_cap + 3) / 4;
+        if (nb > (unsigned long long)ctx->n_cu * 32) nb = (unsigned long long)ctx->n_cu * 32;
+        SP_LAUNCH(ctx, "k3_slow", k3_slow, dim3((unsigned)nb), dim3(256), (size_t)P.R * 16, (const sp_tabref *)d_tabs, P,
+                  d_set, d_uo, d_uc, d_den, (unsigned long long *)ctx->d_flag_row, (unsigned long long *)ctx->d_flag_hist,
+                  (unsigned long long *)ctx->d_blk_row, (unsigned long long *)ctx->d_blk_hist, d_nuni, swar ? 0 : 1);
     }
     unsigned long long *d_tot = d_nuni + 1;
     SP_LAUNCH(ctx, "scan_excl_u64", scan_excl_u64, dim3(1), dim3(1024), 0,
@@ -811,12 +812,12 @@
     SP_LAUNCH(ctx, "scan_excl_u64", scan_excl_u64, dim3(1), dim3(1024), 0,
               (unsigned long long *)ctx->d_blk_hist, nblk, d_tot + 1);
     unsigned long long h[3] = {0, 0, 0};
-    SP_HIP(ctx, hipMemcpyAsync(h, d_tot, 16, hipMemcpyDeviceToHost, ctx->stream));
-    SP_HIP(ctx, hipMemcpyAsync(h + 2, d_nuni, 8, hipMemcpyDeviceToHost, ctx->stream));
+    SP_HIP(ctx, hipMemcpyAsync(h, d_nuni, 24, hipMemcpyDeviceToHost, ctx->stream));
     SP_HIP(ctx, hipStreamSynchronize(ctx->stream));
-    ctx->n_rows = (int64_t)h[0];
-    ctx->n_hist = (int64_t)h[1];
-    ctx->n_union = (int64_t)h[2];
+    ctx->n_union = (int64_t)h[0];
+    ctx->n_rows = (int64_t)h[1];
+    ctx->n_hist = (int64_t)h[2];
+    ctx->fq_cap = (int64_t)P.gq_cap;
     ctx->filtered = true;
     if (n_union) *n_union = ctx->n_union;
     if (n_rows) *n_rows = ctx->n_rows;
@@ -828,14 +829,20 @@
                        uint64_t *tot, int64_t cap, bool async = false) {
     if (!ctx->filtered) return sp_fail(ctx, SP_EINVAL, "call sp_filter first");
     SP_HIP(ctx, hipSetDevice(ctx->device));
+    int rc = sp_fetch_join(ctx);
+    if (rc) return rc;
     const int64_t M = hist ? ctx->n_hist : ctx->n_rows;
     if (cap < M) return sp_fail(ctx, SP_EINVAL, "capacity %lld < %lld rows", (long long)cap, (long long)M);
     if (M == 0) return SP_OK;
     if (ctx->sparse_mode || ctx->list_mode) return sp_sparse_fetch(ctx, hist, keys, counts, freqs, tot, async);
+    if (ctx->sent_pending) {
+        SP_HIP(ctx, hipStreamWaitEvent(ctx->stream, ctx->sent_event, 0));
+        ctx->sent_pending = false;
+    }
     const int C = filter_C(ctx);
     const sp_tabref *d_tabs = nullptr;
     double *d_len = nullptr;
-    int rc = upload_tabs(ctx, &d_tabs, &d_len);
+    rc = upload_tabs(ctx, &d_tabs, &d_len);
     if (rc) return rc;
     unsigned long long *d_keys = nullptr, *d_tot = nullptr;
     uint32_t *d_counts = nullptr;
@@ -856,27 +863,41 @@
     rc = sp_buf_ensure(ctx, ctx->b_slots, M * 4 + 64);
     if (rc) return rc;
     uint32_t *d_slots = (uint32_t *)ctx->b_slots.p;
-    SP_LAUNCH(ctx, "k3_emit_slots", k3_emit_slots, dim3((unsigned)ctx->n_fblocks), dim3(F_BLOCK), 0, filter_nslots(ctx),
-              (const unsigned long long *)(hist ? ctx->d_flag_hist : ctx->d_flag_row),
-              (const unsigned long long *)(hist ? ctx->d_blk_hist : ctx->d_blk_row), d_slots);
-    SP_LAUNCH(ctx, hist ? "k3_emit_hist" : "k3_emit", k3_emit, dim3((unsigned)((M + 255) / 256)), dim3(256), 0, d_tabs, C,
-              (uint32_t)ctx->lower, M, filter_base(ctx), kp, (const uint32_t *)d_slots, (const double *)d_len, d_keys,
-              d_counts, d_freqs, d_tot);
     hipStream_t cs = ctx->stream;
     if (async) {
         if (!ctx->copy_stream) {
             SP_HIP(ctx, hipStreamCreateWithFlags(&ctx->copy_stream, hipStreamNonBlocking));
             SP_HIP(ctx, hipEventCreateWithFlags(&ctx->copy_event, hipEventDisableTiming));
         }
+        if (!ctx->rows_event) SP_HIP(ctx, hipEventCreateWithFlags(&ctx->rows_event, hipEventDisableTiming));
+        if (!ctx->sent_event) SP_HIP(ctx, hipEventCreateWithFlags(&ctx->sent_event, hipEventDisableTiming));
         SP_HIP(ctx, hipEventRecord(ctx->copy_event, ctx->stream));
         SP_HIP(ctx, hipStreamWaitEvent(ctx->copy_stream, ctx->copy_event, 0));
         cs = ctx->copy_stream;
+    }
+    {
+        sp_ctx::lane_scope on(ctx, async ? cs : (hipStream_t) nullptr);
+        SP_LAUNCH(ctx, "k3_emit_slots", k3_emit_slots, dim3((unsigned)ctx->n_fblocks), dim3(F_BLOCK), 0, filter_nslots(ctx),
+                  (const unsigned long long *)(hist ? ctx->d_flag_hist : ctx->d_flag_row),
+                  (const unsigned long long *)(hist ? ctx->d_blk_hist : ctx->d_blk_row), d_slots);
+        SP_LAUNCH(ctx, hist ? "k3_emit_hist" : "k3_emit", k3_emit, dim3((unsigned)((M + 255) / 256)), dim3(256), 0, d_tabs, C,
+                  (uint32_t)ctx->lower, M, filter_base(ctx), kp, (const uint32_t *)d_slots, (const double *)d_len, d_keys,
+                  d_counts, d_freqs, d_tot);
+    }
+    if (async) {
+        SP_HIP(ctx, hipEventRecord(ctx->rows_event, cs));
+        ctx->rows_pending = true;
     }
     if (keys) SP_HIP(ctx, hipMemcpyAsync(keys, d_keys, (size_t)M * 8, hipMemcpyDeviceToHost, cs));
     if (tot) SP_HIP(ctx, hipMemcpyAsync(tot, d_tot, (size_t)M * 8, hipMemcpyDeviceToHost, cs));
     if (counts) SP_HIP(ctx, hipMemcpyAsync(counts, d_counts, (size_t)M * C * 4, hipMemcpyDeviceToHost, cs));
     if (freqs) SP_HIP(ctx, hipMemcpyAsync(freqs, d_freqs, (size_t)M * C * 8, hipMemcpyDeviceToHost, cs));
-    if (!async) SP_HIP(ctx, hipStreamSynchronize(ctx->stream));
+    if (async) {
+        SP_HIP(ctx, hipEventRecord(ctx->sent_event, cs));
+        ctx->sent_pending = true;
+    } else {
+        SP_HIP(ctx, hipStreamSynchronize(ctx->stream));
+    }
     return SP_OK;
 }
 
@@ -893,14 +914,15 @@
 
 int sp_filter_fetch_wait(sp_ctx *ctx) {
     if (!ctx) return SP_EINVAL;
-    if (ctx->copy_stream) SP_HIP(ctx, hipStreamSynchronize(ctx->copy_stream));
-    return SP_OK;
+    return sp_fetch_drain(ctx);
 }
 
 int sp_filter_fetch_device(sp_ctx *ctx, void *d_keys, void *d_counts, void *d_tot, int64_t cap_rows) {
     if (!ctx) return SP_EINVAL;
     if (!ctx->filtered) return sp_fail(ctx, SP_EINVAL, "call sp_filter first");
     SP_HIP(ctx, hipSetDevice(ctx->device));
+    int rc = sp_fetch_join(ctx);
+    if (rc) return rc;
     const int64_t M = ctx->n_rows;
     if (cap_rows < M) return sp_fail(ctx, SP_EINVAL, "capacity %lld < %lld rows", (long long)cap_rows, (long long)M);
     if (M == 0) return SP_OK;
@@ -914,7 +936,7 @@
     }
     const sp_tabref *d_tabs = nullptr;
     double *d_len = nullptr;
-    int rc = upload_tabs(ctx, &d_tabs, &d_len);
+    rc = upload_tabs(ctx, &d_tabs, &d_len);
     if (rc) return rc;
     const sp_kparams kp = sp_make_kparams(ctx->k);
     rc = sp_buf_ensure(ctx, ctx->b_slots, M * 4 + 64);
@@ -929,6 +951,19 @@
     return SP_OK;
 }
 
+int sp_filter_queue_stats(sp_ctx *ctx, int64_t *pushed, int64_t *cap) {
+    if (!ctx || !pushed || !cap) return sp_fail(ctx, SP_EINVAL, "sp_filter_queue_stats: bad arguments");
+    if (!ctx->filtered || ctx->sparse_mode || ctx->list_mode)
+        return sp_fail(ctx, SP_EINVAL, "sp_filter_queue_stats: call sp_filter on byte tables (k <= 15) first");
+    unsigned long long h = 0;
+    SP_HIP(ctx, hipSetDevice(ctx->device));
+    SP_HIP(ctx, hipMemcpyAsync(&h, ctx->b_fq.p, 8, hipMemcpyDeviceToHost, ctx->stream));
+    SP_HIP(ctx, hipStreamSynchronize(ctx->stream));
+    *pushed = (int64_t)h;
+    *cap = ctx->fq_cap;
+    return SP_OK;
+}
+
 int sp_filter_hist(sp_ctx *ctx, uint64_t *tot, int64_t cap) {
     if (!ctx || !tot) return sp_fail(ctx, SP_EINVAL, "sp_filter_hist: bad arguments");
     return emit_common(ctx, true, nullptr, nullptr, nullptr, tot, cap);
diff --git a/subphaser_amd/csrc/sp_hclust.hip b/subphaser_amd/csrc/sp_hclust.hip
--- a/subphaser_amd/csrc/sp_hclust.hip
+++ b/subphaser_amd/csrc/sp_hclust.hip
@@ -174,6 +174,10 @@
             return sp_fail(ctx, SP_EINVAL, "sp_hclust_complete: coordinate %d of point %lld is not finite", (int)(i % (size_t)D),
                            (long long)(i / (size_t)D));
     SP_HIP(ctx, hipSetDevice(ctx->device));
+    {
+        const int rcj_ = sp_fetch_join(ctx);
+        if (rcj_) return rcj_;
+    }
     auto layout = [&](sp_carve &cv, double *&d_pts, double *&d_dist, double *&d_merges, int *&d_size, int *&d_chain, long long *&d_status) {
         d_pts = cv.take<double>(n_pts);
         d_dist = cv.take<double>((size_t)P * (size_t)P);
diff --git a/subphaser_amd/csrc/sp_kboot.hip b/subphaser_amd/csrc/sp_kboot.hip
--- a/subphaser_amd/csrc/sp_kboot.hip
+++ b/subphaser_amd/csrc/sp_kboot.hip
@@ -106,6 +106,10 @@
                            (long long)cols[i], (long long)(i / (size_t)n), (long long)M);
     if (R == 0) return SP_OK;
     SP_HIP(ctx, hipSetDevice(ctx->device));
+    {
+        const int rcj_ = sp_fetch_join(ctx);
+        if (rcj_) return rcj_;
+    }
     const bool on_device = sp_on_device(ctx, z);
     sp_carve sizes;
     auto layout = [&](sp_carve &cv, long long *&d_cols, int *&d_lab, int *&d_it, double *&d_gram) {
diff --git a/subphaser_amd/csrc/sp_kmertest.h b/subphaser_amd/csrc/sp_kmertest.h
--- a/subphaser_amd/csrc/sp_kmertest.h
+++ b/subphaser_amd/csrc/sp_kmertest.h
@@ -42,6 +42,10 @@
 int sp_kt_begin(sp_kt_call &k, bool with_stat, Extra &&extra) {
     sp_ctx *ctx = k.ctx;
     SP_HIP(ctx, hipSetDevice(ctx->device));
+    {
+        const int rcj_ = sp_fetch_join(ctx);
+        if (rcj_) return rcj_;
+    }
     const sp_kt_shape shape{k.M, k.C, k.n_groups, (size_t)k.group_off[k.n_groups], sp_on_device(ctx, k.counts), with_stat};
     sp_carve sizes;
     const size_t need = sp_kt_layout(sizes, shape, k.d, extra);
diff --git a/subphaser_amd/csrc/sp_kpca.hip b/subphaser_amd/csrc/sp_kpca.hip
--- a/subphaser_amd/csrc/sp_kpca.hip
+++ b/subphaser_amd/csrc/sp_kpca.hip
@@ -263,6 +263,10 @@
     if (rc) return rc;
     if (!gram || !n_bad) return sp_fail(ctx, SP_EINVAL, "sp_kmer_pca_gram: bad arguments");
     SP_HIP(ctx, hipSetDevice(ctx->device));
+    {
+        const int rcj_ = sp_fetch_join(ctx);
+        if (rcj_) return rcj_;
+    }
     const int64_t n_chunks = sp_kp_chunks(M), P = sp_kp_tri(C - 1, C - 1) + 1;
     const int n_tiles = (C + SP_KP_T - 1) / SP_KP_T, n_tpairs = n_tiles * (n_tiles + 1) / 2;
     auto layout = [&](sp_carve &cv, double *&d_len, double *&d_stats, double *&d_part, double *&d_gram, unsigned long long *&d_bad) {
@@ -313,6 +317,10 @@
     if (n_comp < 1 || n_comp > SP_KP_MAXCOMP)
         return sp_fail(ctx, SP_EINVAL, "sp_kmer_pca_signs: %d components (1..%d)", n_comp, SP_KP_MAXCOMP);
     SP_HIP(ctx, hipSetDevice(ctx->device));
+    {
+        const int rcj_ = sp_fetch_join(ctx);
+        if (rcj_) return rcj_;
+    }
     const int64_t n_blocks = (M + SP_KP_THREADS - 1) / SP_KP_THREADS;
     auto layout = [&](sp_carve &cv, double *&d_len, double *&d_stats, double *&d_U, long long *&d_crow, double *&d_cval,
                       long long *&d_rows, double *&d_vals, unsigned long long *&d_bad) {
diff --git a/subphaser_amd/csrc/sp_sparse.hip b/subphaser_amd/csrc/sp_sparse.hip
--- a/subphaser_amd/csrc/sp_sparse.hip
+++ b/subphaser_amd/csrc/sp_sparse.hip
@@ -1115,6 +1115,10 @@
     if (!ctx || !keys || !n_out || n_samples < 1 || chrom < 0 || chrom >= (int)ctx->sparse.size())
         return sp_fail(ctx, SP_EINVAL, "sp_sparse_sample: bad arguments");
     SP_HIP(ctx, hipSetDevice(ctx->device));
+    {
+        const int rcj_ = sp_fetch_join(ctx);
+        if (rcj_) return rcj_;
+    }
     const sp_sparse_chrom &o = ctx->sparse[(size_t)chrom];
     const int64_t stride = o.n / n_samples;
     if (stride < 1) {
@@ -1134,6 +1138,10 @@
         chrom >= (int)ctx->sparse.size())
         return sp_fail(ctx, SP_EINVAL, "sp_sparse_split: bad arguments");
     SP_HIP(ctx, hipSetDevice(ctx->device));
+    {
+        const int rcj_ = sp_fetch_join(ctx);
+        if (rcj_) return rcj_;
+    }
     const sp_sparse_chrom &o = ctx->sparse[(size_t)chrom];
     bounds[0] = 0;
     bounds[n_split + 1] = o.n;
@@ -1159,6 +1167,10 @@
     if (count == 0) return SP_OK;
     if (!d_keys || !d_counts) return sp_fail(ctx, SP_EINVAL, "sp_sparse_export: NULL destination");
     SP_HIP(ctx, hipSetDevice(ctx->device));
+    {
+        const int rcj_ = sp_fetch_join(ctx);
+        if (rcj_) return rcj_;
+    }
     SP_HIP(ctx, hipMemcpyAsync(d_keys, o.d_keys + first, (size_t)count * 8, hipMemcpyDeviceToDevice, ctx->stream));
     SP_HIP(ctx, hipMemcpyAsync(d_counts, o.d_cnts + first, (size_t)count * 4, hipMemcpyDeviceToDevice, ctx->stream));
     return SP_OK;
diff --git a/subphaser_amd/csrc/sp_synth.hip b/subphaser_amd/csrc/sp_synth.hip
--- a/subphaser_amd/csrc/sp_synth.hip
+++ b/subphaser_amd/csrc/sp_synth.hip
@@ -86,6 +86,10 @@
         return sp_fail(ctx, SP_EINVAL, "sp_synth_chrom_range: bad arguments");
     if (n == 0) return SP_OK;
     SP_HIP(ctx, hipSetDevice(ctx->device));
+    {
+        const int rcj_ = sp_fetch_join(ctx);
+        if (rcj_) return rcj_;
+    }
     sp_synth_params P;
     P.len = len;
     P.start = start;
```

After: 159.8, median of 6. No clear change (+0.8%).
